# dgrzech/sobfu

Measured on AMD Instinct MI355X. Metric: solver iterations/sec on 256^3 voxel grid, higher is better.
Workload: dtype f32

## Files before the change

include/sobfu_amd/sobfu.hpp:

```cpp
#pragma once

#include <hip/hip_runtime_api.h>
#include <hip/hip_vector_types.h>

#include <chrono>
#include <cmath>
#include <cstdio>
#include <cstdlib>
#include <cstring>
#include <iostream>
#include <memory>
#include <stdexcept>
#include <algorithm>
#include <string>
#include <vector>

#include "sobfu_hip.h"

#ifndef SOBFU_AMD_HAVE_OPENCV
namespace cv {
template <class T, int N>
struct Vec {
    T val[N];
    Vec() { for (int i = 0; i < N; ++i) val[i] = T(); }
// ... 310 lines not shown
    image.create(normals.rows(), normals.cols());
    sobfuSafeCall(sobfu_hip_render_normals((const float*) normals.ptr(), (int) normals.step(), normals.rows(), normals.cols(), (uint8_t*) image.ptr(),
                                           (int) image.step(), nullptr));
}

inline void depthBilateralFilter(const Depth& in, Depth& out, int kernel_size, float sigma_spatial, float sigma_depth) {
    out.create(in.rows(), in.cols());
    sobfuSafeCall(sobfu_hip_bilateral_filter(in.ptr(), (int) in.step(), out.ptr(), (int) out.step(), in.rows(), in.cols(),
                                             kernel_size, sigma_spatial, sigma_depth, nullptr));
}
inline void depthTruncation(Depth& depth, float threshold) {
    sobfuSafeCall(sobfu_hip_truncate_depth(depth.ptr(), (int) depth.step(), depth.rows(), depth.cols(), threshold, nullptr));
}
inline void computeDists(const Depth& depth, Dists& dists, const Intr& intr) {
    dists.create(depth.rows(), depth.cols());
    sobfuSafeCall(sobfu_hip_compute_dists(depth.ptr(), (int) depth.step(), dists.ptr(), (int) dists.step(), depth.rows(),
                                          depth.cols(), intr.fx, intr.fy, intr.cx, intr.cy, nullptr));
}

inline void depthBuildPyramid(const Depth& depth, Depth& pyramid, float sigma_depth) {
    pyramid.create(depth.rows() / 2, depth.cols() / 2);
    sobfuSafeCall(sobfu_hip_depth_pyramid(depth.ptr(), (int) depth.step(), depth.rows(), depth.cols(), pyramid.ptr(), (int) pyramid.step(),
                                          sigma_depth, nullptr));
}
inline void computeNormalsAndMaskDepth(const Intr& intr, Depth& depth, Normals& normals) {
    normals.create(depth.rows(), depth.cols());
    sobfuSafeCall(sobfu_hip_compute_normals_mask_depth(depth.ptr(), (int) depth.step(), depth.rows(), depth.cols(), intr.fx, intr.fy, intr.cx, intr.cy,
                                                       (float*) normals.ptr(), (int) normals.step(), nullptr));
}
inline void computePointNormals(const Intr& intr, const Depth& depth, Cloud& points, Normals& normals) {
    points.create(depth.rows(), depth.cols());
    normals.create(depth.rows(), depth.cols());
    sobfuSafeCall(sobfu_hip_compute_point_normals(depth.ptr(), (int) depth.step(), depth.rows(), depth.cols(), intr.fx, intr.fy, intr.cx, intr.cy,
                                                  (float*) points.ptr(), (int) points.step(), (float*) normals.ptr(), (int) normals.step(), nullptr));
}
inline void resizeDepthNormals(const Depth& depth, const Normals& normals, Depth& depth_out, Normals& normals_out) {
    depth_out.create(depth.rows() / 2, depth.cols() / 2);
    normals_out.create(depth.rows() / 2, depth.cols() / 2);
    sobfuSafeCall(sobfu_hip_resize_depth_normals(depth.ptr(), (int) depth.step(), (const float*) normals.ptr(), (int) normals.step(), depth.rows(),
                                                 depth.cols(), depth_out.ptr(), (int) depth_out.step(), (float*) normals_out.ptr(),
                                                 (int) normals_out.step(), nullptr));
}
inline void resizePointsNormals(const Cloud& points, const Normals& normals, Cloud& points_out, Normals& normals_out) {
    points_out.create(points.rows() / 2, points.cols() / 2);
    normals_out.create(points.rows() / 2, points.cols() / 2);
    sobfuSafeCall(sobfu_hip_resize_points_normals((const float*) points.ptr(), (int) points.step(), (const float*) normals.ptr(), (int) normals.step(),
                                                  points.rows(), points.cols(), (float*) points_out.ptr(), (int) points_out.step(),
                                                  (float*) normals_out.ptr(), (int) normals_out.step(), nullptr));
}

struct Frame {
    bool use_points = false;
    std::vector<Depth> depth_pyr;
    std::vector<Cloud> points_pyr;
    std::vector<Normals> normals_pyr;
};

class ProjectiveICP {
public:
    enum { MAX_PYRAMID_LEVELS = 4 };
    typedef std::vector<Depth> DepthPyr;
    typedef std::vector<Cloud> PointsPyr;
    typedef std::vector<Normals> NormalsPyr;

    ProjectiveICP() : angle_thres_(20.f * 0.017453293f), dist_thres_(0.1f) {
        setIterationsNum(std::vector<int>{10, 5, 4, 0});
        workspace_.create(sobfu_hip_icp_workspace_bytes() + 16 * sizeof(float) + 4 * sizeof(int));
    }
    virtual ~ProjectiveICP() {}
    float getDistThreshold() const { return dist_thres_; }
    void setDistThreshold(float distance) { dist_thres_ = distance; }
    float getAngleThreshold() const { return angle_thres_; }
    void setAngleThreshold(float angle) { angle_thres_ = angle; }
    void setIterationsNum(const std::vector<int>& iters) {
        iters_.assign(MAX_PYRAMID_LEVELS, 0);
        for (size_t i = 0; i < iters.size() && i < (size_t) MAX_PYRAMID_LEVELS; ++i) iters_[i] = iters[i];
    }
    int getUsedLevelsNum() const {
        int i = MAX_PYRAMID_LEVELS - 1;
        for (; i >= 0 && !iters_[i]; --i) {}
        return i + 1;
    }
    virtual bool estimateTransform(Affine3f& affine, const Intr& intr, const Frame& curr, const Frame& prev) {
        if (curr.use_points) return estimateTransform(affine, intr, curr.points_pyr, curr.normals_pyr, prev.points_pyr, prev.normals_pyr);
        return estimateTransform(affine, intr, curr.depth_pyr, curr.normals_pyr, prev.depth_pyr, prev.normals_pyr);
    }
    virtual bool estimateTransform(Affine3f& affine, const Intr& intr, const DepthPyr& dcurr, const NormalsPyr ncurr, const DepthPyr dprev,
                                   const NormalsPyr nprev) {
        return run(affine, intr, 1, [&](int l) {
            return sobfu_hip_icp_level{dcurr[l].ptr(), (int) dcurr[l].step(), (const float*) ncurr[l].ptr(), (int) ncurr[l].step(), dprev[l].ptr(),
                                       (int) dprev[l].step(), (const float*) nprev[l].ptr(), (int) nprev[l].step(), nprev[l].rows(), nprev[l].cols()};
        }, std::min(std::min(dcurr.size(), ncurr.size()), std::min(dprev.size(), nprev.size())));
    }
    virtual bool estimateTransform(Affine3f& affine, const Intr& intr, const PointsPyr& vcurr, const NormalsPyr ncurr, const PointsPyr vprev,
                                   const NormalsPyr nprev) {
        return run(affine, intr, 0, [&](int l) {
            return sobfu_hip_icp_level{vcurr[l].ptr(), (int) vcurr[l].step(), (const float*) ncurr[l].ptr(), (int) ncurr[l].step(), vprev[l].ptr(),
                                       (int) vprev[l].step(), (const float*) nprev[l].ptr(), (int) nprev[l].step(), nprev[l].rows(), nprev[l].cols()};
        }, std::min(std::min(vcurr.size(), ncurr.size()), std::min(vprev.size(), nprev.size())));
    }
    int lastFailedLevel() const { return status_ ? (status_ >> 8) & 0xFF : -1; }
    int lastFailedIteration() const { return status_ ? status_ & 0xFF : -1; }

private:
    template <class F>
    bool run(Affine3f& affine, const Intr& intr, int depth_mode, F level, size_t available) {
        const int n = getUsedLevelsNum();
        affine = Affine3f::Identity();
        if (n < 1 || available < (size_t) n) error("ProjectiveICP: fewer pyramid levels than iterations need", __FILE__, __LINE__);
        sobfu_hip_icp_level lv[MAX_PYRAMID_LEVELS];
        for (int l = 0; l < n; ++l) lv[l] = level(l);
        char* ws = workspace_.ptr<char>();
        const size_t wsb = sobfu_hip_icp_workspace_bytes();
        float* d_pose = (float*) (ws + wsb);
        int* d_status = (int*) (ws + wsb + 16 * sizeof(float));
        sobfuSafeCall(sobfu_hip_icp_estimate(lv, n, iters_.data(), depth_mode, intr.fx, intr.fy, intr.cx, intr.cy, dist_thres_, angle_thres_, ws, wsb,
                                             d_pose, d_status, nullptr, nullptr));
        float P[16];
        sobfuSafeCall(hipMemcpy(P, d_pose, sizeof P, hipMemcpyDeviceToHost));
        sobfuSafeCall(hipMemcpy(&status_, d_status, sizeof status_, hipMemcpyDeviceToHost));
        if (status_ != 0) return false;
        for (int i = 0; i < 3; ++i) {
            for (int j = 0; j < 3; ++j) affine.R[3 * i + j] = P[4 * i + j];
            affine.t[i] = P[4 * i + 3];
        }
        return true;
    }
    std::vector<int> iters_;
    float angle_thres_;
    float dist_thres_;
    DeviceMemory workspace_;
    int status_ = 0;
};
}

namespace device {
typedef int3 Vec3i;
typedef float3 Vec3f;
struct Mat3f { float3 data[3]; };
struct Aff3f { Mat3f R; Vec3f t; };
struct Projector {
    float2 f, c;
    Projector() {}
    Projector(float fx, float fy, float cx, float cy) { f.x = fx; f.y = fy; c.x = cx; c.y = cy; }
};
struct TsdfVolume {
    float2* const data;
    const int3 dims;
    const float3 voxel_size;
    const float trunc_dist, eta, max_weight;
    TsdfVolume(float2* d, int3 dm, float3 vs, float trunc, float eta_, float maxw)
        : data(d), dims(dm), voxel_size(vs), trunc_dist(trunc), eta(eta_), max_weight(maxw) {}
};
inline void clear_volume(TsdfVolume& v) { sobfuSafeCall(sobfu_hip_clear_volume((float*) v.data, v.dims.x, v.dims.y, v.dims.z, nullptr)); }
inline void integrate(TsdfVolume& g, TsdfVolume& n) {
    sobfuSafeCall(sobfu_hip_integrate_fuse((float*) g.data, (const float*) n.data, g.dims.x, g.dims.y, g.dims.z, g.max_weight, nullptr));
    sobfuSafeCall(hipDeviceSynchronize());
}
inline void integrate(const cuda::Dists& dists, TsdfVolume& v, const Aff3f& a, const Projector& p) {
    float R[9] = {a.R.data[0].x, a.R.data[0].y, a.R.data[0].z, a.R.data[1].x, a.R.data[1].y, a.R.data[1].z,
                  a.R.data[2].x, a.R.data[2].y, a.R.data[2].z};
    float t[3] = {a.t.x, a.t.y, a.t.z}, vs[3] = {v.voxel_size.x, v.voxel_size.y, v.voxel_size.z};
    sobfuSafeCall(sobfu_hip_integrate_depth(dists.ptr(), (int) dists.step(), dists.rows(), dists.cols(), (float*) v.data, v.dims.x,
                                            v.dims.y, v.dims.z, vs, v.trunc_dist, v.eta, R, t, p.f.x, p.f.y, p.c.x, p.c.y, nullptr));
    sobfuSafeCall(hipDeviceSynchronize());
}
#define SOBFU_AMD_VS(v) float vs[3] = {(v).voxel_size.x, (v).voxel_size.y, (v).voxel_size.z}
inline void init_sphere(TsdfVolume& v, const float3& c, const float& r) {
    SOBFU_AMD_VS(v); float cc[3] = {c.x, c.y, c.z};
    sobfuSafeCall(sobfu_hip_init_sphere((float*) v.data, v.dims.x, v.dims.y, v.dims.z, vs, v.trunc_dist, v.eta, cc, r, nullptr));
    sobfuSafeCall(hipDeviceSynchronize());
}
inline void init_box(TsdfVolume& v, const float3& b) {
    SOBFU_AMD_VS(v); float bb[3] = {b.x, b.y, b.z};
    sobfuSafeCall(sobfu_hip_init_box((float*) v.data, v.dims.x, v.dims.y, v.dims.z, vs, v.trunc_dist, bb, nullptr));
    sobfuSafeCall(hipDeviceSynchronize());
}
inline void init_ellipsoid(TsdfVolume& v, const float3& r) {
    SOBFU_AMD_VS(v); float rr[3] = {r.x, r.y, r.z};
    sobfuSafeCall(sobfu_hip_init_ellipsoid((float*) v.data, v.dims.x, v.dims.y, v.dims.z, vs, v.trunc_dist, rr, nullptr));
    sobfuSafeCall(hipDeviceSynchronize());
}
inline void init_plane(TsdfVolume& v, const float& z) {
    SOBFU_AMD_VS(v);
    sobfuSafeCall(sobfu_hip_init_plane((float*) v.data, v.dims.x, v.dims.y, v.dims.z, vs, v.trunc_dist, z, nullptr));
    sobfuSafeCall(hipDeviceSynchronize());
}
inline void init_torus(TsdfVolume& v, const float2& t) {
    SOBFU_AMD_VS(v); float tt[2] = {t.x, t.y};
    sobfuSafeCall(sobfu_hip_init_torus((float*) v.data, v.dims.x, v.dims.y, v.dims.z, vs, v.trunc_dist, tt, nullptr));
    sobfuSafeCall(hipDeviceSynchronize());
}
#undef SOBFU_AMD_VS
}

template <class D, class S> inline D device_cast(const S& s);
template <> inline int3 device_cast<int3, cv::Vec3i>(const cv::Vec3i& v) { int3 r; r.x = v[0]; r.y = v[1]; r.z = v[2]; return r; }
template <> inline float3 device_cast<float3, cv::Vec3f>(const cv::Vec3f& v) { float3 r; r.x = v[0]; r.y = v[1]; r.z = v[2]; return r; }
template <> inline device::Aff3f device_cast<device::Aff3f, cv::Affine3f>(const cv::Affine3f& a) {
    device::Aff3f r;
    for (int i = 0; i < 3; ++i) { r.R.data[i].x = a.R[3 * i]; r.R.data[i].y = a.R[3 * i + 1]; r.R.data[i].z = a.R[3 * i + 2]; }
    r.t.x = a.t[0]; r.t.y = a.t[1]; r.t.z = a.t[2];
    return r;
}

namespace cuda {
class TsdfVolume {
public:
    explicit TsdfVolume(const Params& p)
        : trunc_dist_(p.tsdf_trunc_dist), eta_(p.eta), max_weight_(p.tsdf_max_weight), dims_(p.volume_dims), size_(p.volume_size),
          pose_(p.volume_pose), gradient_delta_factor_(p.gradient_delta_factor), raycast_step_factor_(0.f) { create(dims_); }
    virtual ~TsdfVolume() {}
    void create(const Vec3i& dims) {
        dims_ = dims;
        data_.create((size_t) dims_[0] * dims_[1] * dims_[2] * 2 * sizeof(float));
        clear();
    }
    Vec3i getDims() const { return dims_; }
    Vec3f getVoxelSize() const { return Vec3f(size_[0] / dims_[0], size_[1] / dims_[1], size_[2] / dims_[2]); }
    const CudaData data() const { return data_; }
    CudaData data() { return data_; }
    Vec3f getSize() const { return size_; }
    void setSize(const Vec3f& s) { size_ = s; }
    float getTruncDist() const { return trunc_dist_; }
    void setTruncDist(float& d) { trunc_dist_ = d; }
    float getEta() const { return eta_; }
    void setEta(float& e) { eta_ = e; }
    float getMaxWeight() const { return max_weight_; }
    void setMaxWeight(float& w) { max_weight_ = w; }
    Affine3f getPose() const { return pose_; }
    void setPose(const Affine3f& p) { pose_ = p; }
    float getGradientDeltaFactor() const { return gradient_delta_factor_; }
    void setGradientDeltaFactor(float& f) { gradient_delta_factor_ = f; }
    float getRaycastStepFactor() const { return raycast_step_factor_; }
    void setRaycastStepFactor(float& f) { raycast_step_factor_ = f; }
    virtual void clear() { device::TsdfVolume v = pod(); device::clear_volume(v); }
    void swap(CudaData& d) { data_.swap(d); }
    virtual void applyAffine(const Affine3f& a) { pose_ = a * pose_; }
    virtual void integrate(const TsdfVolume& phi_n_psi) {
        device::TsdfVolume g = pod();
        device::TsdfVolume n((float2*) phi_n_psi.data_.ptr<float2>(), g.dims, g.voxel_size, trunc_dist_, eta_, max_weight_);
        device::integrate(g, n);
    }
    virtual void integrate(const Dists& dists, const Affine3f& camera_pose, const Intr& intr) {
        Affine3f vol2cam = camera_pose.inv() * pose_;
        device::TsdfVolume v = pod();
        device::integrate(dists, v, device_cast<device::Aff3f>(vol2cam), device::Projector(intr.fx, intr.fy, intr.cx, intr.cy));
    }
    virtual void raycast(const Affine3f& camera_pose, const Intr& intr, Cloud& points, Normals& normals) {
        const Affine3f vol2cam = camera_pose.inv() * pose_;
        const Vec3f vs = getVoxelSize();
        normals.create(points.rows(), points.cols());
        sobfuSafeCall(sobfu_hip_raycast(data_.ptr<float>(), dims_[0], dims_[1], dims_[2], vs[0], vs[1], vs[2], trunc_dist_, vol2cam.R, vol2cam.t,
                                        intr.fx, intr.fy, intr.cx, intr.cy, points.rows(), points.cols(),
                                        raycast_step_factor_ > 0.f ? raycast_step_factor_ : 0.75f, (float*) points.ptr(), (int) points.step(),
                                        (float*) normals.ptr(), (int) normals.step(), nullptr));
    }
    virtual void initBox(const float3& b) { device::TsdfVolume v = pod(); device::init_box(v, b); }
    virtual void initEllipsoid(const float3& r) { device::TsdfVolume v = pod(); device::init_ellipsoid(v, r); }
    virtual void initPlane(const float& z) { device::TsdfVolume v = pod(); device::init_plane(v, z); }
    virtual void initSphere(const float3& c, const float& r) { device::TsdfVolume v = pod(); device::init_sphere(v, c, r); }
    virtual void initTorus(const float2& t) { device::TsdfVolume v = pod(); device::init_torus(v, t); }
    device::TsdfVolume pod() {
        return device::TsdfVolume(data_.ptr<float2>(), device_cast<int3>(dims_), device_cast<float3>(getVoxelSize()), trunc_dist_, eta_, max_weight_);
    }

private:
    CudaData data_;
    float trunc_dist_, eta_, max_weight_;
    Vec3i dims_;
    Vec3f size_;
    Affine3f pose_;
    float gradient_delta_factor_, raycast_step_factor_;
};

inline int colour_weight_cap(float tsdf_max_weight) { return !(tsdf_max_weight >= 1.f) ? 1 : tsdf_max_weight >= 255.f ? 255 : (int) tsdf_max_weight; }
class ColourVolume {
public:
    explicit ColourVolume(const Vec3i& dims) { create(dims); }
    void create(const Vec3i& dims) {
        dims_ = dims;
        data_.create((size_t) dims_[0] * dims_[1] * dims_[2]);
        clear();
    }
    void clear() { sobfuSafeCall(hipMemsetAsync(data_.ptr(), 0, data_.sizeBytes(), nullptr)); }
    Vec3i getDims() const { return dims_; }
    DeviceArray<RGB>& data() { return data_; }
    const DeviceArray<RGB>& data() const { return data_; }
    void integrate(const Image& image, const TsdfVolume& tsdf, const float* d_psi, const Affine3f& camera_pose, const Intr& intr) {
        const Affine3f vol2cam = camera_pose.inv() * tsdf.getPose();
        const Vec3f vs = tsdf.getVoxelSize();
        const float v[3] = {vs[0], vs[1], vs[2]};
        sobfuSafeCall(sobfu_hip_integrate_colour((const uint8_t*) image.ptr(), (int) image.step(), image.rows(), image.cols(),
                                                 tsdf.data().ptr<float>(), d_psi, (uint8_t*) data_.ptr(), dims_[0], dims_[1], dims_[2], v,
                                                 vol2cam.R, vol2cam.t, intr.fx, intr.fy, intr.cx, intr.cy, colour_weight_cap(tsdf.getMaxWeight()),
                                                 nullptr));
    }
    void apply(const float* d_psi_inv, ColourVolume& out) const {
        out.create(dims_);
        sobfuSafeCall(sobfu_hip_apply_colour((const uint8_t*) data_.ptr(), (uint8_t*) out.data_.ptr(), d_psi_inv, dims_[0], dims_[1], dims_[2], nullptr));
    }
    void sample(const Cloud& points, const Normals& normals, const Affine3f& vol2cam, const Vec3f& voxel_size, Image& out) const {
        out.create(points.rows(), points.cols());
        const float v[3] = {voxel_size[0], voxel_size[1], voxel_size[2]};
        sobfuSafeCall(sobfu_hip_sample_colour((const uint8_t*) data_.ptr(), dims_[0], dims_[1], dims_[2], v, vol2cam.R, vol2cam.t, 0,
                                              (const float*) points.ptr(), (int) points.step(), (const float*) normals.ptr(), (int) normals.step(),
                                              points.rows(), points.cols(), (uint8_t*) out.ptr(), (int) out.step(), nullptr));
    }
    void sample_vertices(const DeviceArray<Point>& vertices, const Affine3f& mc_pose, const Vec3f& voxel_size, std::vector<RGB>& out) const {
        out.clear();
        const size_t n = vertices.size();
        if (n == 0) return;
        DeviceArray<RGB> d(n);
        const float v[3] = {voxel_size[0], voxel_size[1], voxel_size[2]};
        sobfuSafeCall(sobfu_hip_sample_colour((const uint8_t*) data_.ptr(), dims_[0], dims_[1], dims_[2], v, mc_pose.R, mc_pose.t, 1,
                                              (const float*) vertices.ptr(), (int) (n * sizeof(Point)), nullptr, 0, 1, (int) n, (uint8_t*) d.ptr(),
                                              (int) (n * sizeof(RGB)), nullptr));
        d.download(out);
    }

private:
    DeviceArray<RGB> data_;
    Vec3i dims_;
};

inline void renderImage(const Cloud& points, const Normals& normals, const Image& colours, const Vec3f& light_pose, Image& image) {
    image.create(normals.rows(), normals.cols());
    sobfuSafeCall(sobfu_hip_render_colour((const float*) points.ptr(), (int) points.step(), (const float*) normals.ptr(), (int) normals.step(),
                                          (const uint8_t*) colours.ptr(), (int) colours.step(), normals.rows(), normals.cols(), light_pose[0],
                                          light_pose[1], light_pose[2], (uint8_t*) image.ptr(), (int) image.step(), nullptr));
}
}

namespace device {
typedef float4 PointType;
inline void bindTextures(const int*, const int*, const int*) {}
inline void unbindTextures() {}
inline int getOccupiedVoxels(const TsdfVolume& v, cuda::DeviceArray2D<int>& occupied_voxels, cuda::DeviceArray<unsigned char>* scratch = nullptr) {
    int n = 0;
    if (scratch && scratch->size() < sobfu_hip_mc_workspace_bytes(v.dims.x, v.dims.y, v.dims.z))
        scratch->create(sobfu_hip_mc_workspace_bytes(v.dims.x, v.dims.y, v.dims.z));
    sobfuSafeCall(sobfu_hip_mc_occupied_voxels(nullptr, (const float*) v.data, v.dims.x, v.dims.y, v.dims.z, occupied_voxels.ptr(),
                                               (int) (occupied_voxels.step() / sizeof(int)), occupied_voxels.cols(), &n,
                                               scratch ? scratch->ptr() : nullptr, scratch ? scratch->size() : 0));
    return n;
}
inline int computeOffsetsAndTotalVertices(cuda::DeviceArray2D<int>& occupied_voxels, int active_voxels, cuda::DeviceArray<unsigned char>* scratch = nullptr) {
    int total = 0;
    sobfuSafeCall(sobfu_hip_mc_offsets(nullptr, occupied_voxels.ptr(), (int) (occupied_voxels.step() / sizeof(int)), active_voxels, &total,
                                       scratch ? scratch->ptr() : nullptr, scratch ? scratch->size() : 0));
    return total;
}
inline void generateTriangles(const TsdfVolume& v, const cuda::DeviceArray2D<int>& occupied_voxels, int active_voxels, const float3& volume_size,
                              const Aff3f& pose, cuda::DeviceArray<PointType>& out_vertices, cuda::DeviceArray<PointType>& out_normals) {
    const float R[9] = {pose.R.data[0].x, pose.R.data[0].y, pose.R.data[0].z, pose.R.data[1].x, pose.R.data[1].y, pose.R.data[1].z,
                        pose.R.data[2].x, pose.R.data[2].y, pose.R.data[2].z};
    const float t[3] = {pose.t.x, pose.t.y, pose.t.z};
    sobfuSafeCall(sobfu_hip_mc_generate_triangles(nullptr, (const float*) v.data, v.dims.x, v.dims.y, v.dims.z, occupied_voxels.ptr(),
                                                  (int) (occupied_voxels.step() / sizeof(int)), active_voxels, volume_size.x, volume_size.y,
                                                  volume_size.z, R, t, (float*) out_vertices.ptr(), (float*) out_normals.ptr(),
                                                  (int) std::min(out_vertices.size(), out_normals.size())));
    sobfuSafeCall(hipDeviceSynchronize());
}
}

}

namespace sobfu_amd {
struct IndexedMesh {
    std::vector<float4> vertices, normals;
    std::vector<int> faces;
    std::vector<kfusion::RGB> colours;
    size_t triangles() const { return faces.size() / 3; }
    bool empty() const { return faces.empty(); }
};
}

namespace kfusion {
namespace cuda {
class MarchingCubes {
public:
    enum { POINTS_PER_TRIANGLE = 3, DEFAULT_TRIANGLES_BUFFER_SIZE = 2 * 1000 * 1000 * POINTS_PER_TRIANGLE };
    typedef std::shared_ptr<MarchingCubes> Ptr;
    MarchingCubes() : pose(Affine3f::Identity()) {}
    void setPose(const Affine3f& pose_) { pose = pose_; }
    Surface run(const TsdfVolume& volume, DeviceArray<Point>& vertices_buffer, DeviceArray<Normal>& normals_buffer) {
        if (vertices_buffer.empty()) vertices_buffer.create(DEFAULT_TRIANGLES_BUFFER_SIZE);
        if (normals_buffer.empty()) normals_buffer.create(DEFAULT_TRIANGLES_BUFFER_SIZE);
        occupied_voxels_buffer_.create(3, (int) (vertices_buffer.size() / 3));
        device::TsdfVolume vol = const_cast<TsdfVolume&>(volume).pod();
        const int active_voxels = device::getOccupiedVoxels(vol, occupied_voxels_buffer_, &scan_scratch_);
        std::cout << "no. of active voxels: " << active_voxels << std::endl;
        if (!active_voxels) return Surface();
        int total_vertices = device::computeOffsetsAndTotalVertices(occupied_voxels_buffer_, active_voxels, &scan_scratch_);
        const int cap = (int) (std::min(vertices_buffer.size(), normals_buffer.size()) / 3 * 3);
        if (total_vertices > cap) total_vertices = cap;
        device::generateTriangles(vol, occupied_voxels_buffer_, active_voxels, device_cast<float3>(volume.getSize()),
                                  device_cast<device::Aff3f>(pose), vertices_buffer, normals_buffer);
        Surface s;
        s.vertices = DeviceArray<Point>(vertices_buffer.ptr(), (size_t) total_vertices);
        s.normals  = DeviceArray<Normal>(normals_buffer.ptr(), (size_t) total_vertices);
        return s;
    }

    sobfu_amd::IndexedMesh run_indexed(const TsdfVolume& volume) {
        const Vec3i d = volume.getDims();
        const size_t ws = sobfu_hip_mc_indexed_workspace_bytes(d[0], d[1], d[2]);
        if (indexed_scratch_.size() < ws) indexed_scratch_.create(ws);
        const float* vol = volume.data().ptr<float>();
        int active = 0, nv = 0, nt = 0;
        sobfuSafeCall(sobfu_hip_mc_indexed_count(nullptr, vol, d[0], d[1], d[2], indexed_scratch_.ptr(), indexed_scratch_.size(), &active, &nv, &nt));
        std::cout << "no. of active voxels: " << active << std::endl;
        sobfu_amd::IndexedMesh m;
        indexed_vertices_.release();
        if (nt == 0) return m;
        indexed_vertices_.create(nv);
        indexed_normals_.create(nv);
        indexed_faces_.create(3 * (size_t) nt);
        const Vec3f sz = volume.getSize();
        sobfuSafeCall(sobfu_hip_mc_indexed_generate(nullptr, vol, d[0], d[1], d[2], sz[0], sz[1], sz[2], pose.R, pose.t, indexed_scratch_.ptr(),
                                                    indexed_scratch_.size(), (float*) indexed_vertices_.ptr(), (float*) indexed_normals_.ptr(), nv,
// ... 136 lines not shown
inline void convolution_depth(float4* dst, float4* src, int w, int h, int d) { sobfuSafeCall(sobfu_hip_convolution_depth((float*) dst, (const float*) src, conv_taps(), w, h, d, nullptr)); }
inline void calculate_potential_gradient(kfusion::device::TsdfVolume& pnp, kfusion::device::TsdfVolume& pg, TsdfGradient& g, Laplacian& L,
                                         PotentialGradient& nU, float w_reg) {
    sobfuSafeCall(sobfu_hip_potential_gradient((const float*) pnp.data, (const float*) pg.data, (const float*) g.data, (const float*) L.data,
                                               (float*) nU.data, w_reg, pnp.dims.x, pnp.dims.y, pnp.dims.z, nullptr));
}
inline void update_psi(DeformationField& psi, PotentialGradient& nUS, float4* updates, float alpha) {
    sobfuSafeCall(sobfu_hip_update_psi((float*) psi.data, (const float*) nUS.data, (float*) updates, alpha, psi.dims.x, psi.dims.y, psi.dims.z, nullptr));
}

struct Reductor {
    Reductor(int3 dims_, float vsz_, float trunc_dist_) : dims(dims_), vsz(vsz_), trunc_dist(trunc_dist_) {
        no_voxels = dims.x * dims.y * dims.z;
        sobfuSafeCall(sobfu_hip_reduce_config(no_voxels, &blocks, &threads));
        sobfuSafeCall(hipMalloc(&scratch, (size_t) blocks * 8));
        sobfuSafeCall(hipMalloc((void**) &updates, (size_t) no_voxels * sizeof(float4)));
    }
    ~Reductor() { (void) hipFree(scratch); (void) hipFree(updates); }
    Reductor(const Reductor&) = delete;
    Reductor& operator=(const Reductor&) = delete;
    float data_energy(float2* phi_global, float2* phi_n) {
        float e;
        sobfuSafeCall(sobfu_hip_data_energy((const float*) phi_global, (const float*) phi_n, no_voxels, scratch, &e, nullptr));
        return e;
    }
    float reg_energy_sobolev(Mat4f* J) {
        float e;
        sobfuSafeCall(sobfu_hip_reg_energy_sobolev((const float*) J, no_voxels, scratch, &e, nullptr));
        return e;
    }
    float2 max_update_norm() {
        float o[2];
        sobfuSafeCall(sobfu_hip_max_update_norm((const float*) updates, no_voxels, scratch, o, nullptr));
        float2 r; r.x = o[0]; r.y = o[1];
        return r;
    }
    int3 dims;
    float vsz, trunc_dist;
    int no_voxels, blocks, threads;
    float4* updates;
    void* scratch;
};
}

namespace cuda {
class VectorField {
public:
    explicit VectorField(cv::Vec3i d) : dims(d) {
        data.create((size_t) dims[0] * dims[1] * dims[2] * sizeof(float4));
        clear();
    }
    virtual ~VectorField() {}
    cv::Vec3i get_dims() const { return dims; }
    kfusion::cuda::CudaData get_data() { return data; }
    const kfusion::cuda::CudaData get_data() const { return data; }
    void set_data(kfusion::cuda::CudaData& d) { data = d; }
    void clear() { device::VectorField f(data.ptr<float4>(), kfusion::device_cast<int3>(dims)); device::clear(f); }
    void print() {
        const size_t X = (size_t) dims[0], Y = (size_t) dims[1], Z = (size_t) dims[2];
        std::vector<float4> h(X * Y * Z);
        data.download(h.data());
        std::cout << "--- FIELD ---" << std::endl;
        for (size_t i = 0; i < X; ++i)
            for (size_t j = 0; j < Y; ++j)
                for (size_t k = 0; k < Z; ++k) {
                    const float4& v = h[i + X * (j + Y * k)];
                    if (std::fabs(v.x) > 1e-5f || std::fabs(v.y) > 1e-5f || std::fabs(v.z) > 1e-5f)
                        std::cout << "(x,y,z)=(" << i << ", " << j << ", " << k << "), (u,v,w)=(" << v.x << ", " << v.y << "," << v.z << ")"
                                  << std::endl;
                }
    }
    int get_no_nans() {
        size_t n = (size_t) dims[0] * dims[1] * dims[2];
        std::unique_ptr<float4[]> h(new float4[n]);
        data.download(h.get());
        int c = 0;
        for (size_t i = 0; i < n; ++i) c += (h[i].x != h[i].x || h[i].y != h[i].y || h[i].z != h[i].z);
        return c;
    }

protected:
    kfusion::cuda::CudaData data;
    cv::Vec3i dims;
};
typedef VectorField TsdfGradient;
typedef VectorField Laplacian;
typedef VectorField PotentialGradient;

class DeformationField : public VectorField {
public:
    explicit DeformationField(cv::Vec3i d) : VectorField(d) { clear(); }
    void clear() { device::DeformationField p(data.ptr<float4>(), kfusion::device_cast<int3>(dims)); device::init_identity(p); }
    void apply(const cv::Ptr<kfusion::cuda::TsdfVolume> phi, cv::Ptr<kfusion::cuda::TsdfVolume> phi_psi) {
        kfusion::device::TsdfVolume a = phi->pod(), b = phi_psi->pod();
        device::DeformationField p(data.ptr<float4>(), a.dims);
        device::apply(a, b, p);
        kfusion::cuda::waitAllDefaultStream();
    }
    void get_inverse(DeformationField& psi_inv) {
        int3 d = kfusion::device_cast<int3>(dims);
        device::DeformationField a(data.ptr<float4>(), d), b(psi_inv.data.ptr<float4>(), d);
        device::estimate_inverse(a, b);
    }
};

class Jacobian {
public:
    explicit Jacobian(cv::Vec3i d) : dims(d) {
        data.create((size_t) dims[0] * dims[1] * dims[2] * sizeof(Mat4f));
        clear();
    }
    kfusion::cuda::CudaData get_data() { return data; }
    void clear() { device::Jacobian J(data.ptr<Mat4f>(), kfusion::device_cast<int3>(dims)); device::clear(J); }

private:
    kfusion::cuda::CudaData data;
    cv::Vec3i dims;
};

struct SpatialGradients {
    explicit SpatialGradients(cv::Vec3i d)
        : nabla_phi_n(new TsdfGradient(d)), nabla_phi_n_o_psi(new TsdfGradient(d)), J(new Jacobian(d)), J_inv(new Jacobian(d)),
          L(new Laplacian(d)), L_o_psi_inv(new Laplacian(d)), nabla_U(new PotentialGradient(d)), nabla_U_S(new PotentialGradient(d)) {}
    ~SpatialGradients() {
        delete nabla_phi_n; delete nabla_phi_n_o_psi; delete J; delete J_inv; delete L; delete L_o_psi_inv; delete nabla_U; delete nabla_U_S;
    }
    SpatialGradients(const SpatialGradients&) = delete;
    SpatialGradients& operator=(const SpatialGradients&) = delete;
    TsdfGradient *nabla_phi_n, *nabla_phi_n_o_psi;
    Jacobian *J, *J_inv;
    Laplacian *L, *L_o_psi_inv;
    PotentialGradient *nabla_U, *nabla_U_S;
};

class Solver {
public:
    explicit Solver(Params& p) : h_(nullptr) {
        sobfu_hip_solver_params sp;
        sp.verbosity = p.verbosity; sp.max_iter = p.max_iter; sp.s = p.s; sp.max_update_norm = p.max_update_norm;
        sp.lambda = p.lambda; sp.alpha = p.alpha; sp.w_reg = p.w_reg;
        sobfuSafeCall(sobfu_hip_solver_create(&h_, p.volume_dims[0], p.volume_dims[1], p.volume_dims[2], &sp));
    }
    ~Solver() { sobfu_hip_solver_destroy(h_); }
    Solver(const Solver&) = delete;
    Solver& operator=(const Solver&) = delete;
    void estimate_psi(const cv::Ptr<kfusion::cuda::TsdfVolume> phi_global, cv::Ptr<kfusion::cuda::TsdfVolume> phi_global_psi_inv,
                      const cv::Ptr<kfusion::cuda::TsdfVolume> phi_n, cv::Ptr<kfusion::cuda::TsdfVolume> phi_n_psi,
                      std::shared_ptr<DeformationField> psi, std::shared_ptr<DeformationField> psi_inv) {
        sobfuSafeCall(sobfu_hip_solver_estimate_psi(h_, phi_global->data().ptr<float>(), phi_global_psi_inv->data().ptr<float>(),
                                                    phi_n->data().ptr<float>(), phi_n_psi->data().ptr<float>(),
                                                    psi->get_data().ptr<float>(), psi_inv->get_data().ptr<float>(), &last_report,
                                                    nullptr, nullptr));
    }
    sobfu_hip_solver* handle() { return h_; }
    sobfu_hip_solver_report last_report{};

private:
    sobfu_hip_solver* h_;
};
}
}

#include <fstream>
#include <map>
#include <sstream>

namespace sobfu_amd {

inline bool read_params_ini(const std::string& path, Params& p, std::map<std::string, std::string>* raw = nullptr, std::string* why = nullptr) {
    std::ifstream f(path);
    if (!f) {
        if (why) *why = "cannot open " + path;
        return false;
    }
    std::map<std::string, std::string> kv;
    std::string line;
    while (std::getline(f, line)) {
        size_t h = line.find('#');
        if (h != std::string::npos) line.erase(h);
        size_t e = line.find('=');
        if (e == std::string::npos) continue;
        auto trim = [](std::string s) {
            size_t a = s.find_first_not_of(" \t\r\n"), b = s.find_last_not_of(" \t\r\n");
            return a == std::string::npos ? std::string() : s.substr(a, b - a + 1);
        };
        kv[trim(line.substr(0, e))] = trim(line.substr(e + 1));
    }
    auto F = [&](const char* k, float& v) { auto it = kv.find(k); if (it != kv.end()) v = std::strtof(it->second.c_str(), nullptr); };
    auto I = [&](const char* k, int& v) { auto it = kv.find(k); if (it != kv.end()) v = (int) std::strtol(it->second.c_str(), nullptr, 10); };
    I("VOL_DIMS_X", p.volume_dims[0]); I("VOL_DIMS_Y", p.volume_dims[1]); I("VOL_DIMS_Z", p.volume_dims[2]);
    F("VOL_SIZE_X", p.volume_size[0]); F("VOL_SIZE_Y", p.volume_size[1]); F("VOL_SIZE_Z", p.volume_size[2]);
    F("TSDF_MAX_WEIGHT", p.tsdf_max_weight);
    F("GRADIENT_DELTA_FACTOR", p.gradient_delta_factor);
    F("INTR_FX", p.intr.fx); F("INTR_FY", p.intr.fy); F("INTR_CX", p.intr.cx); F("INTR_CY", p.intr.cy);
    F("TRUNC_DEPTH", p.icp_truncate_depth_dist);
    F("BILATERAL_SIGMA_DEPTH", p.bilateral_sigma_depth); F("BILATERAL_SIGMA_SPATIAL", p.bilateral_sigma_spatial);
    I("BILATERAL_KERNEL_SIZE", p.bilateral_kernel_size);
    I("START_FRAME", p.start_frame); I("MAX_ITER", p.max_iter);
    F("MAX_UPDATE_NORM", p.max_update_norm);
    I("S", p.s); F("LAMBDA", p.lambda); F("ALPHA", p.alpha); F("W_REG", p.w_reg);
    {
        int track = p.track_camera ? 1 : 0;
        I("TRACK_CAMERA", track);
        p.track_camera = track != 0;
        F("ICP_DIST_THRES", p.icp_dist_thres);
        auto it = kv.find("ICP_ANGLE_THRES");
        if (it != kv.end()) p.icp_angle_thres = std::strtof(it->second.c_str(), nullptr) * 0.017453293f;
        it = kv.find("ICP_ITERS");
        if (it != kv.end()) {
            std::vector<int> iters;
            std::stringstream ss(it->second);
            std::string tok;
            while (std::getline(ss, tok, ',')) iters.push_back((int) std::strtol(tok.c_str(), nullptr, 10));
            iters.resize(4, 0);
            p.icp_iter_num = iters;
        }
    }
    float trunc_vox = 0.f, eta_vox = 0.f, tz = 0.f;
    for (const char* k : {"TSDF_TRUNC_DIST", "ETA", "VOL_POSE_T_Z"})
        if (!kv.count(k)) {
            if (why) *why = std::string("required key ") + k + " is missing from " + path;
            return false;
        }
    F("TSDF_TRUNC_DIST", trunc_vox); F("ETA", eta_vox); F("VOL_POSE_T_Z", tz);
    for (int i = 0; i < 3; ++i)
        if (p.volume_dims[i] <= 0 || !(p.volume_size[i] > 0.f)) {
            if (why) *why = "VOL_DIMS_* / VOL_SIZE_* must be positive in " + path;
            return false;
        }
    if (!(trunc_vox > 0.f)) {
        if (why) *why = "TSDF_TRUNC_DIST must be positive in " + path;
        return false;
    }
    p.tsdf_trunc_dist = trunc_vox * p.voxel_sizes()[0];
    p.eta             = eta_vox * p.voxel_sizes()[0];
    p.volume_pose     = cv::Affine3f().translate(cv::Vec3f(-p.volume_size[0] / 2.f, -p.volume_size[1] / 2.f, tz));
    if (raw) *raw = kv;
    return true;
}
}

namespace sobfu_amd {
struct MeshFit {
    size_t vertices = 0, valid = 0;
    double mean_abs = 0, rms = 0, max = 0;
};
inline void warp_mesh(IndexedMesh& m, const sobfu::cuda::DeformationField& psi, const Params& p,
                      kfusion::cuda::DeviceArray<kfusion::cuda::Point>* d_vertices = nullptr, kfusion::cuda::DeviceArray<kfusion::cuda::Normal>* d_normals = nullptr) {
    const size_t n = m.vertices.size();
    if (n == 0) return;
    kfusion::cuda::DeviceArray<kfusion::cuda::Point> dv;
    kfusion::cuda::DeviceArray<kfusion::cuda::Normal> dn;
    const bool normals = m.normals.size() == n;
    if (d_vertices && d_vertices->size() == n && (!normals || (d_normals && d_normals->size() == n))) {
        dv = *d_vertices;
        if (normals) dn = *d_normals;
    } else {
        dv.upload(m.vertices);
        if (normals) dn.upload(m.normals);
    }
    const cv::Vec3i d = psi.get_dims();
    const cv::Vec3f vs = p.voxel_sizes();
    const float v[3] = {vs[0], vs[1], vs[2]};
    sobfuSafeCall(sobfu_hip_warp_points(psi.get_data().ptr<float>(), d[0], d[1], d[2], v, p.volume_pose.R, p.volume_pose.t, 1, (const float*) dv.ptr(),
                                        normals ? (const float*) dn.ptr() : nullptr, (int) n, (float*) dv.ptr(), normals ? (float*) dn.ptr() : nullptr,
                                        nullptr));
    dv.download(m.vertices);
    if (normals) dn.download(m.normals);
}
inline MeshFit mesh_fit(const IndexedMesh& m, const kfusion::cuda::TsdfVolume& vol, const Params& p, std::vector<float>* samples = nullptr) {
    MeshFit f;
    const size_t n = f.vertices = m.vertices.size();
    std::vector<float> h;
    if (n > 0) {
        kfusion::cuda::DeviceArray<kfusion::cuda::Point> dv;
        kfusion::cuda::DeviceArray<float> out(n);
        dv.upload(m.vertices);
        const cv::Vec3i d = vol.getDims();
        const cv::Vec3f vs = vol.getVoxelSize();
        const float v[3] = {vs[0], vs[1], vs[2]};
        sobfuSafeCall(sobfu_hip_sample_tsdf(vol.data().ptr<float>(), d[0], d[1], d[2], v, p.volume_pose.R, p.volume_pose.t, 1, (const float*) dv.ptr(), (int) n,
                                            out.ptr(), nullptr));
        out.download(h);
    }
    double s1 = 0, s2 = 0;
    for (float x : h) {
        if (x != x) continue;
        const double a = std::fabs((double) x) * (double) vol.getTruncDist();
        ++f.valid, s1 += a, s2 += a * a, f.max = std::max(f.max, a);
    }
    if (f.valid) f.mean_abs = s1 / (double) f.valid, f.rms = std::sqrt(s2 / (double) f.valid);
    if (samples) samples->swap(h);
    return f;
}
}

#include "evaluate.hpp"
#include "warp_stats.hpp"

#ifndef SOBFU_AMD_NO_SOBFUSION
class SobFusion {
public:
    explicit SobFusion(const Params& p) : frame_counter_(0), params(p), camera_pose_(cv::Affine3f::Identity()) {
        dists_.create(params.rows, params.cols);
        mc = std::make_shared<kfusion::cuda::MarchingCubes>();
        mc->setPose(params.volume_pose);
        poses_.reserve(4096);
    }
    Params& getParams() { return params; }
    const std::vector<cv::Affine3f>& getPoses() const { return poses_; }
    cv::Affine3f getCameraPose() const { return camera_pose_; }
    bool operator()(const kfusion::cuda::Depth& depth, const kfusion::cuda::Image& image = kfusion::cuda::Image()) {
        const bool coloured = !image.empty();
        if (coloured && (image.rows() != depth.rows() || image.cols() != depth.cols()))
            kfusion::cuda::error("colour frame and depth frame differ in size", __FILE__, __LINE__);
        std::printf("--- FRAME NO. %d ---\n", frame_counter_);
        kfusion::cuda::depthBilateralFilter(depth, filtered_, params.bilateral_kernel_size, params.bilateral_sigma_spatial,
                                            params.bilateral_sigma_depth);
        kfusion::cuda::depthTruncation(filtered_, params.icp_truncate_depth_dist);
        kfusion::cuda::computeDists(filtered_, dists_, params.intr);
        if (params.track_camera) track();
        poses_.push_back(camera_pose_);
        return frame(image, [&](kfusion::cuda::TsdfVolume& v, bool fresh) {
            if (!fresh) v.clear();
            v.integrate(dists_, camera_pose_, params.intr);
        });
    }
    bool integrate_mesh(const sobfu_amd::IndexedMesh& mesh, const cv::Affine3f& mesh2cam = sobfu_amd::mesh_frame(), bool allow_open = false,
                        std::string* why = nullptr, int* open_rows = nullptr, int sign = sobfu_amd::kSignParity) {
        cv::Ptr<kfusion::cuda::TsdfVolume> target = frame_counter_ == 0 ? cv::Ptr<kfusion::cuda::TsdfVolume>(new kfusion::cuda::TsdfVolume(params)) : phi_n;
        int open = 0;
        if (!sobfu_amd::mesh_to_tsdf(mesh, mesh2cam, camera_pose_.inv() * params.volume_pose, *target, &open, why, 0.f, SOBFU_MESH_DISTANCE_AUTO, sign)) return false;
        if (open_rows) *open_rows = open;
        if (sign != sobfu_amd::kSignWinding && open > 0 && !allow_open) {
            if (why) *why = "the mesh is not closed: " + std::to_string(open) + " rows of the volume cross it an odd number of times";
            return false;
        }
        std::printf("--- FRAME NO. %d ---\n", frame_counter_);
        poses_.push_back(camera_pose_);
        return frame(kfusion::cuda::Image(), [](kfusion::cuda::TsdfVolume&, bool) {}, target);
    }
    std::shared_ptr<kfusion::cuda::ColourVolume> get_colour_global_psi_inv() {
        if (!colour_global) return nullptr;
        if (!colour_global_psi_inv) colour_global_psi_inv = std::make_shared<kfusion::cuda::ColourVolume>(params.volume_dims);
        colour_global->apply(psi_inv->get_data().ptr<float>(), *colour_global_psi_inv);
        return colour_global_psi_inv;
    }
    std::shared_ptr<sobfu::cuda::DeformationField> getDeformationField() { return psi; }
    sobfu_amd::TriangleMesh get_phi_global_mesh() { return get_mesh(phi_global, colour_global.get()); }
    sobfu_amd::TriangleMesh get_phi_global_psi_inv_mesh() { return get_mesh(phi_global_psi_inv, get_colour_global_psi_inv().get()); }
    sobfu_amd::TriangleMesh get_phi_n_mesh() { return get_mesh(phi_n); }
    sobfu_amd::TriangleMesh get_phi_n_psi_mesh() { return get_mesh(phi_n_psi); }
    sobfu_amd::TriangleMesh get_mesh(cv::Ptr<kfusion::cuda::TsdfVolume> vol, const kfusion::cuda::ColourVolume* colour = nullptr) {
        kfusion::cuda::DeviceArray<kfusion::cuda::Point> vertices_buffer;
        kfusion::cuda::DeviceArray<kfusion::cuda::Normal> normals_buffer;
        kfusion::cuda::Surface model = mc->run(*vol, vertices_buffer, normals_buffer);
        kfusion::cuda::waitAllDefaultStream();
        sobfu_amd::TriangleMesh m = convert_to_mesh(model.vertices);
        if (colour) colour->sample_vertices(model.vertices, params.volume_pose, vol->getVoxelSize(), m.colours);
        return m;
    }
    sobfu_amd::IndexedMesh get_phi_global_indexed_mesh() { return get_indexed_mesh(phi_global, colour_global.get()); }
    sobfu_amd::IndexedMesh get_phi_global_psi_inv_indexed_mesh() { return get_indexed_mesh(phi_global_psi_inv, get_colour_global_psi_inv().get()); }
    sobfu_amd::IndexedMesh get_phi_n_indexed_mesh() { return get_indexed_mesh(phi_n); }
    sobfu_amd::IndexedMesh get_phi_n_psi_indexed_mesh() { return get_indexed_mesh(phi_n_psi); }
    sobfu_amd::IndexedMesh get_indexed_mesh(cv::Ptr<kfusion::cuda::TsdfVolume> vol, const kfusion::cuda::ColourVolume* colour = nullptr) {
        sobfu_amd::IndexedMesh m = mc->run_indexed(*vol);
        if (colour && !m.empty()) colour->sample_vertices(mc->last_indexed_vertices(), params.volume_pose, vol->getVoxelSize(), m.colours);
        return m;
    }
    sobfu_amd::IndexedMesh get_phi_global_warped_indexed_mesh() {
        sobfu_amd::IndexedMesh m = get_indexed_mesh(phi_global, colour_global.get());
        if (!m.empty() && psi) sobfu_amd::warp_mesh(m, *psi, params, &mc->last_indexed_vertices(), &mc->last_indexed_normals());
        return m;
    }
    sobfu_amd::IndexedMesh warp_to_live(sobfu_amd::IndexedMesh m) {
        if (psi) sobfu_amd::warp_mesh(m, *psi, params);
        return m;
    }
    sobfu_amd::MeshFit fit_to_live(const sobfu_amd::IndexedMesh& m, std::vector<float>* samples = nullptr) {
        if (!phi_n) kfusion::cuda::error("fit_to_live needs a second frame", __FILE__, __LINE__);
        return sobfu_amd::mesh_fit(m, *phi_n, params, samples);
    }
    bool evaluate_canonical(const sobfu_amd::IndexedMesh& gt, float max_dist, sobfu_amd::MeshComparison& out, sobfu_amd::IndexedMesh* model = nullptr,
                            std::vector<float>* d_model = nullptr, std::string* why = nullptr, sobfu_amd::AlignRequest* align = nullptr, bool with_signs = false,
                            int sign = sobfu_amd::kSignParity, const sobfu_amd::ScoreRequest* score = nullptr, sobfu_amd::MeshScore* scored = nullptr) {
        sobfu_amd::IndexedMesh m = get_phi_global_indexed_mesh();
        const bool scoring = score && scored;
        bool ok;
        if (align) {
            sobfu_amd::IndexedMesh posed = gt;
            ok = sobfu_amd::align_meshes(m.vertices, gt, align->pose, align->info, align->iters, max_dist, align->dof, 0.f, 0.f, why);
            if (ok) {
                sobfu_amd::transform_points(posed.vertices, align->pose);
                ok = sobfu_amd::compare_meshes(m, posed, max_dist, out, d_model, nullptr, why, nullptr, with_signs, sign);
            }
            if (ok && scoring) ok = sobfu_amd::f_score(m, posed, *score, max_dist, *scored, why);
        } else {
            ok = sobfu_amd::compare_meshes(m, gt, max_dist, out, d_model, nullptr, why, nullptr, with_signs, sign);
            if (ok && scoring) ok = sobfu_amd::f_score(m, gt, *score, max_dist, *scored, why);
        }
        if (model) *model = std::move(m);
        return ok;
    }
    bool evaluate_live(const sobfu_amd::IndexedMesh& gt, float max_dist, sobfu_amd::MeshComparison& out, sobfu_amd::IndexedMesh* model = nullptr,
                       std::vector<float>* d_model = nullptr, std::string* why = nullptr, sobfu_amd::TriangleGrid* gt_grid = nullptr, bool with_signs = false,
                       int sign = sobfu_amd::kSignParity, const sobfu_amd::ScoreRequest* score = nullptr, sobfu_amd::MeshScore* scored = nullptr) {
        sobfu_amd::IndexedMesh m = get_phi_global_warped_indexed_mesh();
        bool ok = sobfu_amd::compare_meshes(m, gt, max_dist, out, d_model, nullptr, why, gt_grid, with_signs, sign);
        if (ok && score && scored) ok = sobfu_amd::f_score(m, gt, *score, max_dist, *scored, why, gt_grid);
        if (model) *model = std::move(m);
        return ok;
    }
    bool warp_stats(float band, sobfu_amd::WarpStats& out, std::vector<float>* det = nullptr, std::vector<float>* res = nullptr,
                    const std::vector<float>& edges = {0.f, 0.25f, 0.5f, 1.f, 2.f, 4.f}, float res_tol = -1.f) {
        if (!solved_) return false;
        const cv::Vec3i d = psi->get_dims();
        const cv::Vec3f vs = params.voxel_sizes();
        const int dims[3] = {d[0], d[1], d[2]};
        const float v[3] = {vs[0], vs[1], vs[2]};
        const float tol = res_tol >= 0.f ? res_tol : (float) (0.1 * (double) std::min(v[0], std::min(v[1], v[2])));
        out = sobfu_amd::warp_stats(psi->get_data().ptr<float>(), psi_inv->get_data().ptr<float>(), phi_global->data().ptr<float>(),
                                    phi_global_psi_inv->data().ptr<float>(), dims, v, band, edges, tol, det, res);
        return true;
    }
    static sobfu_amd::TriangleMesh convert_to_mesh(const kfusion::cuda::DeviceArray<kfusion::cuda::Point>& triangles) {
        sobfu_amd::TriangleMesh m;
        if (!triangles.empty()) triangles.download(m.vertices);
        return m;
    }
    std::shared_ptr<kfusion::cuda::MarchingCubes> mc;

    cv::Ptr<kfusion::cuda::TsdfVolume> phi_global, phi_global_psi_inv, phi_n, phi_n_psi;
    std::shared_ptr<sobfu::cuda::DeformationField> psi, psi_inv;
    std::shared_ptr<sobfu::cuda::Solver> solver;
    std::shared_ptr<kfusion::cuda::ColourVolume> colour_global, colour_global_psi_inv;

private:
    template <class Integrate>
    bool frame(const kfusion::cuda::Image& image, Integrate&& integrate, cv::Ptr<kfusion::cuda::TsdfVolume> ready = cv::Ptr<kfusion::cuda::TsdfVolume>()) {
        const bool coloured = !image.empty();
        if (frame_counter_ == 0) {
            phi_global = ready ? ready : cv::Ptr<kfusion::cuda::TsdfVolume>(new kfusion::cuda::TsdfVolume(params));
            integrate(*phi_global, true);
            if (coloured) integrate_colour(image, *phi_global, nullptr);
            phi_global_psi_inv = cv::Ptr<kfusion::cuda::TsdfVolume>(new kfusion::cuda::TsdfVolume(params));
            phi_n              = cv::Ptr<kfusion::cuda::TsdfVolume>(new kfusion::cuda::TsdfVolume(params));
            phi_n_psi          = cv::Ptr<kfusion::cuda::TsdfVolume>(new kfusion::cuda::TsdfVolume(params));
            psi     = std::make_shared<sobfu::cuda::DeformationField>(params.volume_dims);
            psi_inv = std::make_shared<sobfu::cuda::DeformationField>(params.volume_dims);
            solver  = std::make_shared<sobfu::cuda::Solver>(params);
            return ++frame_counter_, true;
        }
        integrate(*phi_n, false);
        if (frame_counter_ < params.start_frame) {
            if (coloured) integrate_colour(image, *phi_n, nullptr);
            phi_global->integrate(*phi_n);
            return ++frame_counter_, true;
        }
        solver->estimate_psi(phi_global, phi_global_psi_inv, phi_n, phi_n_psi, psi, psi_inv);
        solved_ = true;
        if (coloured) integrate_colour(image, *phi_n_psi, psi->get_data().ptr<float>());
        phi_global->integrate(*phi_n_psi);
        return ++frame_counter_, true;
    }
    void integrate_colour(const kfusion::cuda::Image& image, const kfusion::cuda::TsdfVolume& tsdf, const float* d_psi) {
        if (!colour_global) colour_global = std::make_shared<kfusion::cuda::ColourVolume>(params.volume_dims);
        colour_global->integrate(image, tsdf, d_psi, camera_pose_, params.intr);
    }
    void track() {
        kfusion::cuda::ProjectiveICP probe;
        probe.setIterationsNum(params.icp_iter_num);
        const int levels = std::max(1, probe.getUsedLevelsNum());
        curr_.use_points = prev_.use_points = true;
        curr_.depth_pyr.resize(levels), curr_.points_pyr.resize(levels), curr_.normals_pyr.resize(levels);
        curr_.depth_pyr[0] = filtered_;
        for (int l = 1; l < levels; ++l) kfusion::cuda::depthBuildPyramid(curr_.depth_pyr[l - 1], curr_.depth_pyr[l], params.bilateral_sigma_depth);
        for (int l = 0; l < levels; ++l) kfusion::cuda::computePointNormals(params.intr(l), curr_.depth_pyr[l], curr_.points_pyr[l], curr_.normals_pyr[l]);
        if (frame_counter_ > 0) {
            if (!icp_) icp_ = std::make_shared<kfusion::cuda::ProjectiveICP>();
            icp_->setIterationsNum(params.icp_iter_num);
            icp_->setDistThreshold(params.icp_dist_thres);
            icp_->setAngleThreshold(params.icp_angle_thres);
            cv::Affine3f aff;
            if (icp_->estimateTransform(aff, params.intr, curr_, prev_)) camera_pose_ = camera_pose_ * aff;
            else std::printf("camera tracking failed on frame %d (level %d, iteration %d): keeping the previous pose\n", frame_counter_,
                             icp_->lastFailedLevel(), icp_->lastFailedIteration());
        }
        std::swap(curr_, prev_);
    }
    int frame_counter_;
    bool solved_ = false;
    Params params;
    cv::Affine3f camera_pose_;
    std::vector<cv::Affine3f> poses_;
    kfusion::cuda::Frame curr_, prev_;
    std::shared_ptr<kfusion::cuda::ProjectiveICP> icp_;
    kfusion::cuda::Depth filtered_;
    kfusion::cuda::Dists dists_;
};
#endif
```

include/sobfu_hip.h:

```cpp
#ifndef SOBFU_HIP_H
#define SOBFU_HIP_H

#include <stddef.h>
#include <stdint.h>

#if defined(__GNUC__)
#pragma GCC visibility push(default)
#endif
#ifdef __cplusplus
extern "C" {
#endif

#define SOBFU_HIP_ABI_VERSION 3

#define SOBFU_E_BADARG (-1)
#define SOBFU_E_FILTER (-2)
#define SOBFU_E_UNSUPPORTED (-3)

int sobfu_hip_abi_version(void);
const char* sobfu_hip_error_string(int code);

int sobfu_hip_clear_volume(float* d_vol, int X, int Y, int Z, void* stream);
int sobfu_hip_integrate_depth(const float* d_dists, int dists_step_bytes, int rows, int cols, float* d_vol, int X,
                              int Y, int Z, const float voxel_size[3], float trunc_dist, float eta,
                              const float R[9], const float t[3], float fx, float fy, float cx, float cy,
                              void* stream);
int sobfu_hip_integrate_fuse(float* d_phi_global, const float* d_phi_n_psi, int X, int Y, int Z, float max_weight,
                             void* stream);
int sobfu_hip_init_sphere(float* d_vol, int X, int Y, int Z, const float voxel_size[3], float trunc_dist, float eta,
                          const float centre[3], float radius, void* stream);
int sobfu_hip_init_box(float* d_vol, int X, int Y, int Z, const float voxel_size[3], float trunc_dist,
                       const float b[3], void* stream);
int sobfu_hip_init_ellipsoid(float* d_vol, int X, int Y, int Z, const float voxel_size[3], float trunc_dist,
                             const float r[3], void* stream);
int sobfu_hip_init_plane(float* d_vol, int X, int Y, int Z, const float voxel_size[3], float trunc_dist, float z,
                         void* stream);
int sobfu_hip_init_torus(float* d_vol, int X, int Y, int Z, const float voxel_size[3], float trunc_dist,
                         const float t[2], void* stream);

int sobfu_hip_bilateral_filter(const uint16_t* d_src, int src_step_bytes, uint16_t* d_dst, int dst_step_bytes,
                               int rows, int cols, int kernel_size, float sigma_spatial, float sigma_depth,
                               void* stream);
int sobfu_hip_truncate_depth(uint16_t* d_depth, int step_bytes, int rows, int cols, float max_dist_m, void* stream);
int sobfu_hip_compute_dists(const uint16_t* d_depth, int depth_step_bytes, float* d_dists, int dists_step_bytes,
                            int rows, int cols, float fx, float fy, float cx, float cy, void* stream);

int sobfu_hip_clear_field(float* d_field, int X, int Y, int Z, void* stream);
int sobfu_hip_init_identity(float* d_psi, int X, int Y, int Z, void* stream);
int sobfu_hip_apply(const float* d_phi, float* d_phi_warped, const float* d_psi, int X, int Y, int Z, void* stream);
int sobfu_hip_estimate_inverse(const float* d_psi, float* d_psi_inv, int X, int Y, int Z, int n_sweeps,
                               void* stream);
int sobfu_hip_inverse_and_warp(const float* d_psi, float* d_psi_inv, const float* d_phi, float* d_phi_warped, int X, int Y, int Z,
                               int n_sweeps, void* stream);
int sobfu_hip_tsdf_gradient(const float* d_vol, float* d_grad, int X, int Y, int Z, void* stream);
int sobfu_hip_laplacian(const float* d_psi, float* d_L, int X, int Y, int Z, void* stream);
int sobfu_hip_jacobian(const float* d_psi, float* d_J, int X, int Y, int Z, int mode, void* stream);
int sobfu_hip_clear_jacobian(float* d_J, int X, int Y, int Z, void* stream);

int sobfu_hip_sobolev_filter(int s, float lambda, float* out);
int sobfu_hip_potential_gradient(const float* d_phi_n_psi, const float* d_phi_global, const float* d_grad,
                                 const float* d_L, float* d_nabla_U, float w_reg, int X, int Y, int Z, void* stream);
int sobfu_hip_convolution_rows(float* d_dst, const float* d_src, const float taps[7], int w, int h, int d,
                               void* stream);
int sobfu_hip_convolution_columns(float* d_dst, const float* d_src, const float taps[7], int w, int h, int d,
                                  void* stream);
int sobfu_hip_convolution_depth(float* d_dst, const float* d_src, const float taps[7], int w, int h, int d,
                                void* stream);
int sobfu_hip_update_psi(float* d_psi, const float* d_nabla_U_S, float* d_updates, float alpha, int X, int Y, int Z,
                         void* stream);

int sobfu_hip_reduce_config(int n, int* blocks, int* threads);
int sobfu_hip_data_energy(const float* d_phi_global, const float* d_phi_n, int n, void* d_scratch, float* out,
                          void* stream);
int sobfu_hip_reg_energy_sobolev(const float* d_J, int n, void* d_scratch, float* out, void* stream);
int sobfu_hip_max_update_norm(const float* d_updates, int n, void* d_scratch, float out[2], void* stream);
int sobfu_hip_reg_energy_sobolev_from_psi(const float* d_psi, int X, int Y, int Z, void* d_scratch, float* out,
                                          void* stream);

int sobfu_hip_fused_potential_gradient(const float* d_phi_n_psi, const float* d_phi_global, const float* d_psi,
                                       float* d_nabla_U, float w_reg, int X, int Y, int Z, void* stream);
int sobfu_hip_fused_smooth_update_apply(const float* d_nabla_U, float* d_psi, const float* d_phi_n,
                                        float* d_phi_n_psi, float* d_updates, uint32_t* d_max_sq_slots,
                                        const float taps[7], float alpha, int X, int Y, int Z, void* stream);

int sobfu_hip_pack_vec3(const float* d_src4, float* d_dst3, size_t n, void* stream);
int sobfu_hip_unpack_vec3(const float* d_src3, float* d_dst4, size_t n, void* stream);
int sobfu_hip_extract_tsdf(const float* d_src2, float* d_dst1, size_t n, void* stream);

int sobfu_hip_tile3_init_identity(float* d_psi, int Lx, int Ly, int Lz, int xb, int yb, int zb, void* stream);
int sobfu_hip_tile3_apply(const float* d_phi, int Xg, int Yg, int Zg, float* d_phi_warped, const float* d_psi, int Lx, int Ly, int Lz,
                          void* stream);
int sobfu_hip_tile3_estimate_inverse(const float* d_psi, int Xg, int Yg, int Zg, float* d_psi_inv, int Lx, int Ly, int Lz, int xb, int yb,
                                     int zb, int n_sweeps, void* stream);
int sobfu_hip_tile3_estimate_inverse_window(const float* d_psi_win, const int win[6], int Xg, int Yg, int Zg, float* d_psi_inv, int Lx, int Ly, int Lz,
                                            int xb, int yb, int zb, const int box[6], int n_sweeps, int* d_violation, void* stream);
int sobfu_hip_tile3_apply_window(const float* d_phi_win, const int win[6], int Xg, int Yg, int Zg, float* d_phi_warped, const float* d_psi, int Lx,
                                 int Ly, int Lz, const int box[6], int* d_violation, void* stream);
int sobfu_hip_tile3_max_displacement(const float* d_psi, int Lx, int Ly, int Lz, int xb, int yb, int zb, const int box[6], uint32_t* d_max_bits,
                                     void* stream);
int sobfu_hip_tile3_integrate_depth(const float* d_dists, int dists_step_bytes, int rows, int cols, float* d_vol_local, int Lx, int Ly,
                                    int Lz, int xb, int yb, int zb, const float voxel_size[3], float trunc_dist, float eta,
                                    const float R[9], const float t[3], float fx, float fy, float cx, float cy, void* stream);
int sobfu_hip_tile3_potential_gradient(const float* d_phi_n_psi, const float* d_phi_global, const float* d_psi, float* d_nabla_U,
                                       float w_reg, int Lx, int Ly, int Lz, const int box[6], int thin,
                                       const uint32_t* d_prev_slots, float max_update_norm, int compact, void* stream);
int sobfu_hip_tile3_smooth_update_apply(const float* d_nabla_U, float* d_psi, const float* d_phi_n, float* d_phi_n_psi, float* d_updates,
                                        uint32_t* d_max_sq_slots, const float taps[7], float alpha, int Lx, int Ly, int Lz, int Xg,
                                        int Yg, int Zg, const int own[6], const int box[6], int thin,
                                        const uint32_t* d_prev_slots, float max_update_norm, int compact, void* stream);
int sobfu_hip_tile3_apply_tsdf_only(const float* d_phi1, int Xg, int Yg, int Zg, float* d_out1, const float* d_psi3, int Lx, int Ly, int Lz,
                                    void* stream);
int sobfu_hip_tile3_pack(const float* d_field3, int Lx, int Ly, int Lz, float* d_buf, const int* boxes, int n_boxes, void* stream);
int sobfu_hip_tile3_unpack(float* d_field3, int Lx, int Ly, int Lz, const float* d_buf, const int* boxes, int n_boxes, void* stream);

typedef struct sobfu_hip_solver sobfu_hip_solver;

typedef struct {
    int verbosity;
    int max_iter;
    int s;
    float max_update_norm;
    float lambda;
    float alpha;
    float w_reg;
} sobfu_hip_solver_params;

typedef struct {
    int iterations;
    int converged;
    float last_max_update_norm;
    float last_max_update_index;
    float last_e_data, last_e_reg;
} sobfu_hip_solver_report;

int sobfu_hip_solver_create(sobfu_hip_solver** out, int X, int Y, int Z, const sobfu_hip_solver_params* params);
int sobfu_hip_solver_destroy(sobfu_hip_solver* s);
int sobfu_hip_solver_set_params(sobfu_hip_solver* s, const sobfu_hip_solver_params* params);
size_t sobfu_hip_solver_workspace_bytes(const sobfu_hip_solver* s);
int sobfu_hip_solver_estimate_psi(sobfu_hip_solver* s, const float* d_phi_global, float* d_phi_global_psi_inv,
                                  const float* d_phi_n, float* d_phi_n_psi, float* d_psi, float* d_psi_inv,
                                  sobfu_hip_solver_report* report, float* per_iter_max_norm, void* stream);
int sobfu_hip_solver_iterate(sobfu_hip_solver* s, const float* d_phi_global, const float* d_phi_n,
                             float* d_phi_n_psi, float* d_psi, int n_iters, sobfu_hip_solver_report* report,
                             float* per_iter_max_norm, void* stream);
int sobfu_hip_solver_begin(sobfu_hip_solver* s, const float* d_phi_global, const float* d_phi_n, float* d_phi_n_psi,
                           float* d_psi, int max_iters, void* stream);
int sobfu_hip_solver_step(sobfu_hip_solver* s, int n_iters, void* stream);
int sobfu_hip_solver_end(sobfu_hip_solver* s, sobfu_hip_solver_report* report, float* per_iter_max_norm, void* stream);
float* sobfu_hip_solver_updates(sobfu_hip_solver* s);
int sobfu_hip_solver_keep_updates(sobfu_hip_solver* s, int keep);
int sobfu_hip_solver_set_compact(sobfu_hip_solver* s, int enable);
int sobfu_hip_solver_set_profiling(sobfu_hip_solver* s, int stride);
int sobfu_hip_solver_get_profile(sobfu_hip_solver* s, float* ms_pass_a, float* ms_pass_b, int* launches, int reset);
typedef void (*sobfu_hip_log_fn)(const char* line, void* user);
int sobfu_hip_solver_set_logger(sobfu_hip_solver* s, sobfu_hip_log_fn fn, void* user);

size_t sobfu_hip_mc_workspace_bytes(int X, int Y, int Z);
int sobfu_hip_mc_occupied_voxels(void* stream, const float* d_vol, int X, int Y, int Z, int* d_occupied, int stride, int max_size,
                                 int* h_count, void* d_workspace, size_t workspace_bytes);
int sobfu_hip_mc_offsets(void* stream, int* d_occupied, int stride, int count, int* h_total_vertices, void* d_workspace,
                         size_t workspace_bytes);
int sobfu_hip_mc_generate_triangles(void* stream, const float* d_vol, int X, int Y, int Z, const int* d_occupied, int stride, int count,
                                    float size_x, float size_y, float size_z, const float R[9], const float t[3], float* d_vertices,
                                    float* d_normals, int max_vertices);
size_t sobfu_hip_mc_indexed_workspace_bytes(int X, int Y, int Z);
int sobfu_hip_mc_indexed_count(void* stream, const float* d_vol, int X, int Y, int Z, void* d_workspace, size_t workspace_bytes,
                               int* h_active_cells, int* h_vertices, int* h_triangles);
int sobfu_hip_mc_indexed_generate(void* stream, const float* d_vol, int X, int Y, int Z, float size_x, float size_y, float size_z,
                                  const float R[9], const float t[3], void* d_workspace, size_t workspace_bytes, float* d_vertices,
                                  float* d_normals, int max_vertices, int* d_faces, int max_triangles);

int sobfu_hip_raycast(const float* d_vol, int X, int Y, int Z, float vsx, float vsy, float vsz, float trunc, const float R[9],
                      const float t[3], float fx, float fy, float cx, float cy, int rows, int cols, float step_factor, float* d_points,
                      int points_step, float* d_normals, int normals_step, void* stream);
int sobfu_hip_render_image(const float* d_points, int points_step, const float* d_normals, int normals_step, int rows, int cols,
                           float lx, float ly, float lz, uint8_t* d_image, int image_step, void* stream);
int sobfu_hip_render_normals(const float* d_normals, int normals_step, int rows, int cols, uint8_t* d_image, int image_step,
                             void* stream);

int sobfu_hip_integrate_colour(const uint8_t* d_image, int image_step, int rows, int cols, const float* d_tsdf, const float* d_psi,
                               uint8_t* d_colour, int X, int Y, int Z, const float voxel_size[3], const float R[9], const float t[3],
                               float fx, float fy, float cx, float cy, int cap, void* stream);
int sobfu_hip_apply_colour(const uint8_t* d_colour, uint8_t* d_colour_warped, const float* d_psi_inv, int X, int Y, int Z, void* stream);
int sobfu_hip_sample_colour(const uint8_t* d_colour, int X, int Y, int Z, const float voxel_size[3], const float R[9], const float t[3],
                            int mc_vertices, const float* d_points, int points_step, const float* d_normals, int normals_step, int rows,
                            int cols, uint8_t* d_out, int out_step, void* stream);
int sobfu_hip_render_colour(const float* d_points, int points_step, const float* d_normals, int normals_step, const uint8_t* d_colour_image,
                            int colour_step, int rows, int cols, float lx, float ly, float lz, uint8_t* d_image, int image_step,
                            void* stream);

int sobfu_hip_warp_points(const float* d_psi, int X, int Y, int Z, const float voxel_size[3], const float R[9], const float t[3],
                          int mc_vertices, const float* d_points, const float* d_normals, int n, float* d_points_out, float* d_normals_out,
                          void* stream);
int sobfu_hip_sample_tsdf(const float* d_vol, int X, int Y, int Z, const float voxel_size[3], const float R[9], const float t[3],
                          int mc_vertices, const float* d_points, int n, float* d_out, void* stream);

int sobfu_hip_depth_pyramid(const uint16_t* d_src, int src_step, int rows, int cols, uint16_t* d_dst, int dst_step, float sigma_depth,
                            void* stream);
int sobfu_hip_compute_point_normals(const uint16_t* d_depth, int depth_step, int rows, int cols, float fx, float fy, float cx, float cy,
                                    float* d_points, int points_step, float* d_normals, int normals_step, void* stream);
int sobfu_hip_compute_normals_mask_depth(uint16_t* d_depth, int depth_step, int rows, int cols, float fx, float fy, float cx, float cy,
                                         float* d_normals, int normals_step, void* stream);
int sobfu_hip_resize_depth_normals(const uint16_t* d_depth, int depth_step, const float* d_normals, int normals_step, int rows, int cols,
                                   uint16_t* d_depth_out, int depth_out_step, float* d_normals_out, int normals_out_step, void* stream);
int sobfu_hip_resize_points_normals(const float* d_points, int points_step, const float* d_normals, int normals_step, int rows, int cols,
                                    float* d_points_out, int points_out_step, float* d_normals_out, int normals_out_step, void* stream);
typedef struct {
    const void* curr;
    int curr_step;
    const float* ncurr;
    int ncurr_step;
    const void* prev;
    int prev_step;
    const float* nprev;
    int nprev_step;
    int rows, cols;
} sobfu_hip_icp_level;
size_t sobfu_hip_icp_workspace_bytes(void);
int sobfu_hip_icp_step(const sobfu_hip_icp_level* level, int level_index, int depth_mode, float fx, float fy, float cx, float cy,
                       float dist_thres, float angle_thres, const float* d_aff, void* d_workspace, size_t workspace_bytes,
                       double* d_sums, uint8_t* d_codes, int codes_step, void* stream);
int sobfu_hip_icp_estimate(const sobfu_hip_icp_level* levels, int n_levels, const int iters[4], int depth_mode, float fx, float fy, float cx,
                           float cy, float dist_thres, float angle_thres, void* d_workspace, size_t workspace_bytes, float* d_pose,
                           int* d_status, float* d_trace, void* stream);

#define SOBFU_E_RCCL (-4)
typedef struct sobfu_hip_tiled sobfu_hip_tiled;
int sobfu_hip_tiled_load_rccl(const char* librccl_path);
int sobfu_hip_tiled_unique_id(char out[128]);
int sobfu_hip_tiled_create(sobfu_hip_tiled** out, int X, int Y, int Z, int world, int rank, const char unique_id[128],
                           const sobfu_hip_solver_params* params);
int sobfu_hip_tiled_destroy(sobfu_hip_tiled* t);
int sobfu_hip_tiled_create3(sobfu_hip_tiled** out, int X, int Y, int Z, int Px, int Py, int Pz, int rank, const char unique_id[128],
                            const sobfu_hip_solver_params* params);
int sobfu_hip_tiled_layout3(const sobfu_hip_tiled* t, int out[24]);
int sobfu_hip_tiled_layout(const sobfu_hip_tiled* t, int* z0, int* z1, int* lo, int* hi, int* Lz, int* zbase);
int sobfu_hip_tiled_iterate(sobfu_hip_tiled* t, const float* d_phi_global_local, const float* d_phi_n_full,
                            float* d_phi_n_psi_local, float* d_psi_local, int n_iters, sobfu_hip_solver_report* report,
                            float* per_iter_max_norm, void* stream);
int sobfu_hip_tiled_begin(sobfu_hip_tiled* t, const float* d_phi_global_local, const float* d_phi_n_full, float* d_phi_n_psi_local,
                          float* d_psi_local, int max_iters, void* stream);
int sobfu_hip_tiled_step(sobfu_hip_tiled* t, int n_iters, void* stream);
int sobfu_hip_tiled_end(sobfu_hip_tiled* t, sobfu_hip_solver_report* report, float* per_iter_max_norm, void* stream);
int sobfu_hip_tiled_add_reduce_comm(sobfu_hip_tiled* t, const char unique_id[128]);
int sobfu_hip_tiled_set_schedule(sobfu_hip_tiled* t, int schedule);
double sobfu_hip_tiled_last_enqueue_us(const sobfu_hip_tiled* t);
typedef struct {
    int peer;
    size_t send_off, recv_off, count;
} sobfu_hip_tiled_msg;
int sobfu_hip_tiled_messages(const sobfu_hip_tiled* t, sobfu_hip_tiled_msg* msgs, int* send_boxes, int* recv_boxes, int max_msgs);
int sobfu_hip_tiled_messages_inplace(const sobfu_hip_tiled* t, sobfu_hip_tiled_msg* msgs, int max_msgs, int* n_packed);
int sobfu_hip_tiled_set_profiling(sobfu_hip_tiled* t, int stride, int max_samples);
int sobfu_hip_tiled_get_profile(sobfu_hip_tiled* t, float ms[3], int* samples, int reset);
typedef int (*sobfu_hip_tiled_exchange_fn)(void* ctx, int rank, const float* d_send, float* d_recv, const sobfu_hip_tiled_msg* msgs,
                                           int n_msgs, void* stream);
typedef int (*sobfu_hip_tiled_allreduce_fn)(void* ctx, int rank, uint32_t* d_buf, size_t n, void* stream);
int sobfu_hip_tiled_set_transport(sobfu_hip_tiled* t, sobfu_hip_tiled_exchange_fn exchange, sobfu_hip_tiled_allreduce_fn allreduce_max,
                                  void* ctx);
#define SOBFU_E_TIMEOUT (-5)
typedef struct {
    void* arena;
    size_t nabla_u_off[2];
    size_t rows_off;
    void* flags;
} sobfu_hip_tiled_exports;
int sobfu_hip_tiled_exports_get(const sobfu_hip_tiled* t, sobfu_hip_tiled_exports* out);
int sobfu_hip_tiled_connect(sobfu_hip_tiled* t, int n_peers, const int* peer_ranks, const sobfu_hip_tiled_exports* peers);
int sobfu_hip_ipc_export(const void* d_ptr, char handle[64]);
int sobfu_hip_ipc_open(const char handle[64], void** d_ptr);
int sobfu_hip_ipc_close(void* d_ptr);
int sobfu_hip_tiled_status(sobfu_hip_tiled* t, int* missing_peer);
int sobfu_hip_tiled_max_iterations(const sobfu_hip_tiled* t);
int sobfu_hip_p2p_info(int device, int peer_device, int out[4]);
int sobfu_hip_tiled_wait_stats(sobfu_hip_tiled* t, double* wait_us, int* waits, int reset);
int sobfu_hip_tiled_pingpong(sobfu_hip_tiled* t, int rank_a, int rank_b, int reps, void* stream);
int sobfu_hip_tiled_probe_push(sobfu_hip_tiled* t, int reps, void* stream);
int sobfu_hip_tiled_set_wait(sobfu_hip_tiled* t, int wait);
int sobfu_hip_tiled_step_phase(sobfu_hip_tiled* t, int phase, void* stream);
int sobfu_hip_tiled_exchange(sobfu_hip_tiled* t, float* d_field3, int planes, void* stream);
int sobfu_hip_tiled_self_sendrecv(sobfu_hip_tiled* t, const float* d_src, float* d_dst, size_t n, void* stream);
int sobfu_hip_tiled_allreduce_max_u32(sobfu_hip_tiled* t, uint32_t* d_buf, size_t n, void* stream);

int sobfu_hip_mesh_grid_plan(const float bbox[6], int n_triangles, float cell, float origin[3], float* h, int dims[3]);
size_t sobfu_hip_mesh_grid_workspace_bytes(const int dims[3], int max_refs);
int sobfu_hip_mesh_grid_build(const float* d_vertices, int n_vertices, const int* d_faces, int n_triangles, const float origin[3], float h,
                              const int dims[3], void* d_workspace, size_t workspace_bytes, int max_refs, int* h_refs, void* stream);
#define SOBFU_MESH_DISTANCE_AUTO 0
#define SOBFU_MESH_DISTANCE_GRID 1
#define SOBFU_MESH_DISTANCE_BRUTE 2
int sobfu_hip_mesh_distance(void* d_workspace, size_t workspace_bytes, const float* d_vertices, int n_vertices, const int* d_faces,
                            int n_triangles, const float origin[3], float h, const int dims[3], const float* d_points, int n, float max_dist,
                            int mode, int ring_cap, float* d_dist, int* d_tri, float* d_closest, int* d_unresolved, void* stream);
int sobfu_hip_mesh_distance_unresolved(const void* d_workspace, int* h_count, void* stream);

size_t sobfu_hip_mesh_align_workspace_bytes(int n);
int sobfu_hip_mesh_align_step(void* d_grid_workspace, size_t grid_workspace_bytes, const float* d_vertices, int n_vertices, const int* d_faces,
                              int n_triangles, const float origin[3], float h, const int dims[3], const float* d_points, int n, float max_dist, int mode,
                              int ring_cap, const float* d_pose, void* d_workspace, size_t workspace_bytes, double* d_sums, void* stream);
int sobfu_hip_mesh_align_estimate(void* d_grid_workspace, size_t grid_workspace_bytes, const float* d_vertices, int n_vertices, const int* d_faces,
                                  int n_triangles, const float origin[3], float h, const int dims[3], const float* d_points, int n, float max_dist,
                                  int mode, int ring_cap, int iters, int dof, float eps_rot, float eps_trans, void* d_workspace, size_t workspace_bytes,
                                  float* d_pose, int* d_status, float* d_trace, void* stream);

// ... 99 lines not shown
```

sobfu_amd/csrc/solver_capi.hip:

```cpp
#include <algorithm>
#include <cmath>
#include <cstdio>
#include <cstdlib>
#include <cstring>
#include <string>
#include <vector>

#include "sobfu_device.hpp"
#include "sobfu_hip.h"
#include "sobfu_host.hpp"
#include "sobfu_launch.hpp"


namespace {

using sobfu_hip::DevicePtr;
using sobfu_hip::EventPtr;
using sobfu_hip::kSlots;
using sobfu_hip::slots_to_norm;
constexpr int kCheckEvery = 32;
constexpr int kMaxRunAhead = 96;

}

struct sobfu_hip_solver {
    int X = 0, Y = 0, Z = 0;
    size_t N = 0;
    sobfu_hip_solver_params p{};
    float taps[7]{};
    DevicePtr<float> nabla_U;
    DevicePtr<float> updates;
    DevicePtr<float> c_psi;
    DevicePtr<float> c_f;
    DevicePtr<float> c_g;
    DevicePtr<float> c_n;
    bool compact = true;
    DevicePtr<uint32_t> slots;
    sobfu_hip::PinnedPtr<uint32_t> h_rows;
    int h_rows_iters   = 0;
    EventPtr ev_chk;
    DevicePtr<void> red_scratch;
    int slots_iters    = 0;
    bool keep_updates  = false;
    sobfu_hip_log_fn log_fn = nullptr;
    void* log_user          = nullptr;
    bool log_set            = false;
    size_t bytes            = 0;
    int prof_stride = 0;
    std::vector<EventPtr> events;
    double ms_a = 0, ms_b = 0;
    int prof_launches = 0, prof_pending = 0;
    struct Session {
        bool active = false, compact = false;
        const float *pg = nullptr, *pn = nullptr;
        float *pnp = nullptr, *psi = nullptr;
        const float *it_pnp = nullptr, *it_pg = nullptr, *it_pn = nullptr;
        float *it_psi = nullptr, *it_out = nullptr, *upd = nullptr;
        int cap = 0;
        int launched = 0;
        int checked = 0, fl_to = 0;
        bool in_flight = false;
        int done = 0;
        bool converged = false;
        float last_norm = 0.f;
        bool inline_log = false;
        bool warp = false;
    } q;

    void log(const std::string& line) const {
        if (log_set) {
            if (log_fn) log_fn(line.c_str(), log_user);
        } else {
            std::printf("%s\n", line.c_str());
        }
    }
};

namespace {

std::string fmt_g(float v) {
    char b[64];
    std::snprintf(b, sizeof b, "%g", (double) v);
    return b;
}

int ensure_slots(sobfu_hip_solver* s, int iters) {
    if (iters <= s->slots_iters) return 0;
    if (s->slots) s->bytes -= (size_t) (s->slots_iters + 1) * kSlots * 4;
    s->slots_iters = 0;
    SOBFU_HIP_TRY(sobfu_hip::device_alloc(s->slots, (size_t) (iters + 1) * kSlots * 4));
    s->slots_iters = iters;
    s->bytes += (size_t) (iters + 1) * kSlots * 4;
    return 0;
}

int ensure_poll(sobfu_hip_solver* s, int iters) {
    if (!s->ev_chk) SOBFU_HIP_TRY(sobfu_hip::event_create(s->ev_chk, hipEventDisableTiming));
    if (iters <= s->h_rows_iters) return 0;
    s->h_rows.reset();
    s->h_rows_iters = 0;
    void* h = nullptr;
    SOBFU_HIP_TRY(hipHostMalloc(&h, (size_t) iters * kSlots * 4, hipHostMallocDefault));
    s->h_rows.reset((uint32_t*) h);
    s->h_rows_iters = iters;
    return 0;
}

int ensure_compact(sobfu_hip_solver* s) {
    if (s->c_psi) return 0;
    SOBFU_HIP_TRY(sobfu_hip::device_alloc(s->c_psi, s->N * 12));
    SOBFU_HIP_TRY(sobfu_hip::device_alloc(s->c_f, s->N * 4));
    SOBFU_HIP_TRY(sobfu_hip::device_alloc(s->c_g, s->N * 4));
    SOBFU_HIP_TRY(sobfu_hip::device_alloc(s->c_n, s->N * 4));
    s->bytes += s->N * 24;
    return 0;
}

int ensure_updates(sobfu_hip_solver* s) {
    if (s->updates) return 0;
    SOBFU_HIP_TRY(sobfu_hip::device_alloc(s->updates, s->N * 16));
    s->bytes += s->N * 16;
    return 0;
}

int set_params(sobfu_hip_solver* s, const sobfu_hip_solver_params* p) {
    SOBFU_CHECK_ARGS(p && p->max_iter >= 0);
    if (p->s < 7 || p->s > 16) return p->s < 7 ? SOBFU_E_UNSUPPORTED : SOBFU_E_FILTER;
    float h[16];
    SOBFU_TRY(sobfu_hip_sobolev_filter(p->s, p->lambda, h));
    for (int i = 0; i < 7; ++i) s->taps[i] = h[i];
    s->p = *p;
    return 0;
}

int ensure_events(sobfu_hip_solver* s, size_t n) {
    while (s->events.size() < n) {
        EventPtr e;
        SOBFU_HIP_TRY(sobfu_hip::event_create(e, hipEventDefault));
        s->events.push_back(std::move(e));
    }
    return 0;
}

int session_begin_impl(sobfu_hip_solver* s, const float* pg, const float* pn, float* pnp, float* psi, int cap, hipStream_t st) {
    sobfu_hip_solver::Session& q = s->q;
    const int X = s->X, Y = s->Y, Z = s->Z;
    q = sobfu_hip_solver::Session{};
    q.pg = pg; q.pn = pn; q.pnp = pnp; q.psi = psi;
    q.cap = cap;
    q.compact = s->compact && cap > 0;
    q.last_norm = NAN;
    if (!q.compact) SOBFU_TRY(sobfu_hip_apply(pn, pnp, psi, X, Y, Z, st));
    if (cap <= 0) return 0;
    SOBFU_TRY(ensure_slots(s, cap));
    SOBFU_HIP_TRY(hipMemsetAsync(s->slots.get(), 0, (size_t) (cap + 1) * kSlots * 4, st));
    if (s->keep_updates) {
        SOBFU_TRY(ensure_updates(s));
        q.upd = s->updates.get();
    }
    q.it_pnp = pnp; q.it_pg = pg; q.it_pn = pn; q.it_psi = psi; q.it_out = pnp;
    if (q.compact) {
        SOBFU_TRY(ensure_compact(s));
        SOBFU_TRY(sobfu_hip::launch_compact_enter(psi, pg, pn, s->c_psi.get(), s->c_g.get(), s->c_n.get(), s->c_f.get(), X, Y, Z, st));
        q.it_pnp = s->c_f.get(); q.it_pg = s->c_g.get(); q.it_pn = s->c_n.get(); q.it_psi = s->c_psi.get(); q.it_out = s->c_f.get();
        q.warp = s->p.verbosity == 0 && !q.upd && sobfu_hip::loop_warps_in_pass_a(X, Y, Z);
    }
    if (s->p.max_update_norm >= 0.f) SOBFU_TRY(ensure_poll(s, cap));
    if (s->prof_stride > 0) SOBFU_TRY(ensure_events(s, (size_t) 3 * (cap / s->prof_stride + 1)));
    return 0;
}
int session_begin(sobfu_hip_solver* s, const float* pg, const float* pn, float* pnp, float* psi, int cap, hipStream_t st) {
    if (s->q.active) return SOBFU_E_BADARG;
    const int rc = session_begin_impl(s, pg, pn, pnp, psi, cap, st);
    s->q.active = rc == 0;
    return rc;
}

void session_examine(sobfu_hip_solver* s, int upto, float* per_iter) {
    sobfu_hip_solver::Session& q = s->q;
    for (int k = q.checked; k < upto && !q.converged; ++k) {
        const float v = slots_to_norm(s->h_rows.get() + (size_t) k * kSlots);
        if (per_iter) per_iter[k] = v;
        q.last_norm = v;
        q.done = k + 1;
        if (v <= s->p.max_update_norm) q.converged = true;
    }
    q.checked = upto;
}

int session_enqueue(sobfu_hip_solver* s, int n, bool poll, float* per_iter, hipStream_t st) {
    sobfu_hip_solver::Session& q = s->q;
    if (!q.active || n < 0 || q.launched + n > q.cap) return SOBFU_E_BADARG;
    const int X = s->X, Y = s->Y, Z = s->Z;
    const sobfu_hip_solver_params& p = s->p;
    const bool can_converge = p.max_update_norm >= 0.f;
    const int last = q.launched + n;
    sobfu_hip::PassALaunch A;
    sobfu_hip::set_whole_grid(A, X, Y, Z);
    A.pnp = q.warp ? q.it_pn : q.it_pnp; A.pg = q.it_pg; A.psi = q.it_psi; A.nU = s->nabla_U.get(); A.w_reg = p.w_reg;
    A.max_update_norm = p.max_update_norm;
    A.compact = q.compact;
    A.warp    = q.warp;
    sobfu_hip::PassBLaunch B;
    sobfu_hip::set_whole_grid(B, X, Y, Z);
    B.nU = s->nabla_U.get(); B.psi = q.it_psi; B.phi_n = q.it_pn; B.pnp = q.it_out; B.updates = q.upd; B.taps = s->taps; B.alpha = p.alpha;
    B.max_update_norm = p.max_update_norm;
    B.compact = q.compact;
    B.warp    = q.warp;
    for (int it = q.launched + 1; it <= last && !q.converged; ++it) {
        const uint32_t* prev = (it > 1) ? s->slots.get() + (size_t) (it - 1) * kSlots : nullptr;
        uint32_t* cur        = s->slots.get() + (size_t) it * kSlots;
        const bool ev = s->prof_stride > 0 && (it % s->prof_stride == 0) && (size_t) 3 * (s->prof_pending + 1) <= s->events.size();
        const int e0  = 3 * s->prof_pending;
        if (ev) SOBFU_HIP_TRY(hipEventRecord(s->events[e0].get(), st));
        A.prev_slots = B.prev_slots = prev;
        B.slots = cur;
        SOBFU_TRY(sobfu_hip::launch_pass_a(A, st));
        if (ev) SOBFU_HIP_TRY(hipEventRecord(s->events[e0 + 1].get(), st));
        SOBFU_TRY(sobfu_hip::launch_pass_b(B, st));
        if (ev) {
            SOBFU_HIP_TRY(hipEventRecord(s->events[e0 + 2].get(), st));
            s->prof_pending += 1;
        }
        q.launched = it;
        if (can_converge && poll) {
            if (!q.in_flight && (it % kCheckEvery == 0 || it == last)) {
                SOBFU_HIP_TRY(hipMemcpyAsync(s->h_rows.get() + (size_t) q.checked * kSlots, s->slots.get() + (size_t) (q.checked + 1) * kSlots,
                                             (size_t) (it - q.checked) * kSlots * 4, hipMemcpyDeviceToHost, st));
                SOBFU_HIP_TRY(hipEventRecord(s->ev_chk.get(), st));
                q.in_flight = true;
                q.fl_to     = it;
            }
            if (q.in_flight) {
                const bool must_wait = it - q.checked >= kMaxRunAhead;
                hipError_t e = must_wait ? hipEventSynchronize(s->ev_chk.get()) : hipEventQuery(s->ev_chk.get());
                if (e == hipSuccess) {
                    session_examine(s, q.fl_to, per_iter);
                    q.in_flight = false;
                } else if (e != hipErrorNotReady) {
                    return (int) e;
                }
            }
        }
    }
    return 0;
}

int session_drain(sobfu_hip_solver* s, float* per_iter, hipStream_t st) {
    sobfu_hip_solver::Session& q = s->q;
    if (q.launched == 0) return 0;
    if (s->p.max_update_norm >= 0.f) {
        if (q.in_flight) {
            SOBFU_HIP_TRY(hipEventSynchronize(s->ev_chk.get()));
            session_examine(s, q.fl_to, per_iter);
            q.in_flight = false;
        }
        if (!q.converged && q.checked < q.launched) {
            SOBFU_HIP_TRY(hipMemcpyAsync(s->h_rows.get() + (size_t) q.checked * kSlots, s->slots.get() + (size_t) (q.checked + 1) * kSlots,
                                         (size_t) (q.launched - q.checked) * kSlots * 4, hipMemcpyDeviceToHost, st));
            SOBFU_HIP_TRY(hipStreamSynchronize(st));
            session_examine(s, q.launched, per_iter);
        }
    } else {
        std::vector<uint32_t> hs((size_t) q.launched * kSlots);
        SOBFU_HIP_TRY(hipMemcpyAsync(hs.data(), s->slots.get() + kSlots, hs.size() * 4, hipMemcpyDeviceToHost, st));
        SOBFU_HIP_TRY(hipStreamSynchronize(st));
        for (int k = 0; k < q.launched; ++k) {
            const float v = slots_to_norm(hs.data() + (size_t) k * kSlots);
            if (per_iter) per_iter[k] = v;
            q.last_norm = v;
        }
        q.done = q.launched;
    }
    return 0;
}

int session_end(sobfu_hip_solver* s, sobfu_hip_solver_report* rep, float* per_iter, hipStream_t st) {
    sobfu_hip_solver::Session& q = s->q;
    if (!q.active) return SOBFU_E_BADARG;
    sobfu_hip_solver_report r{};
    r.last_max_update_norm = NAN;
    r.last_max_update_index = NAN;
    r.last_e_data = r.last_e_reg = NAN;
    SOBFU_TRY(session_drain(s, per_iter, st));
    if (q.compact) SOBFU_TRY(sobfu_hip::launch_compact_leave(s->c_psi.get(), q.pn, q.psi, q.pnp, s->X, s->Y, s->Z, st));
    for (int it = 1; it <= q.done && !q.inline_log; ++it)
        if (it == 1 || it % 50 == 0) s->log("iter. no. " + std::to_string(it));
    if (q.converged) s->log("SOLVER CONVERGED AFTER " + std::to_string(q.done) + " ITERATIONS");
    else if (q.cap > 0 && q.done == q.cap) s->log("SOLVER REACHED MAX. NO. OF ITERATIONS WITHOUT CONVERGING");
    r.iterations = q.done;
    r.converged  = q.converged ? 1 : 0;
    r.last_max_update_norm = q.last_norm;
    q.active = false;
    SOBFU_HIP_TRY(hipStreamSynchronize(st));
    if (rep) *rep = r;
    return 0;
}

int run_verbose(sobfu_hip_solver* s, const float* pg, const float* pn, float* pnp, float* psi, int max_iter,
                sobfu_hip_solver_report* rep, float* per_iter, hipStream_t st) {
    const int X = s->X, Y = s->Y, Z = s->Z;
    const sobfu_hip_solver_params& p = s->p;
    auto reports = [&](int it) { return p.verbosity == 2 || (p.verbosity == 1 && (it == 1 || it % 50 == 0 || it == max_iter)); };
    SOBFU_TRY(ensure_updates(s));
    SOBFU_TRY(session_begin(s, pg, pn, pnp, psi, max_iter, st));
    sobfu_hip_solver::Session& q = s->q;
    q.upd = s->updates.get();
    q.inline_log = p.verbosity <= 2;
    float e_data = NAN, e_reg = NAN, arg = NAN;
    auto fail = [&](int rc) {
        q.active = false;
        return rc;
    };
#define SOBFU_VTRY(expr)                    \
    do {                                    \
        const int rc_ = (int) (expr);       \
        if (rc_ != 0) return fail(rc_);     \
    } while (0)
    sobfu_hip::PassALaunch A;
    sobfu_hip::set_whole_grid(A, X, Y, Z);
    A.pnp = q.it_pnp; A.pg = q.it_pg; A.psi = q.it_psi; A.nU = s->nabla_U.get(); A.w_reg = p.w_reg;
    A.compact = q.compact;
    sobfu_hip::PassBLaunch B;
    sobfu_hip::set_whole_grid(B, X, Y, Z);
    B.nU = s->nabla_U.get(); B.psi = q.it_psi; B.phi_n = q.it_pn; B.pnp = q.it_out; B.updates = s->updates.get(); B.taps = s->taps; B.alpha = p.alpha;
    B.compact = q.compact;
    for (int it = 1; it <= max_iter && !q.converged;) {
        if (!reports(it)) {
            int to = it;
            while (to + 1 <= max_iter && !reports(to + 1)) ++to;
            SOBFU_VTRY(session_enqueue(s, to - it + 1, true, per_iter, st));
            if (p.max_update_norm >= 0.f) SOBFU_VTRY(session_drain(s, per_iter, st));
            it = to + 1;
            continue;
        }
        if (it == 1 || it % 50 == 0) s->log("iter. no. " + std::to_string(it));
        if (q.compact) {
            SOBFU_VTRY(sobfu_hip::data_energy_tsdf(q.it_pg, q.it_pnp, (int) s->N, s->red_scratch.get(), &e_data, st));
            SOBFU_VTRY(sobfu_hip::reg_energy_from_psi3(q.it_psi, X, Y, Z, s->red_scratch.get(), &e_reg, st));
        } else {
            SOBFU_VTRY(sobfu_hip_data_energy(pg, pnp, (int) s->N, s->red_scratch.get(), &e_data, st));
            SOBFU_VTRY(sobfu_hip_reg_energy_sobolev_from_psi(psi, X, Y, Z, s->red_scratch.get(), &e_reg, st));
        }
        const float e = e_data + p.w_reg * e_reg;
        s->log("data energy + w_reg * reg energy = " + fmt_g(e_data) + " + " + fmt_g(p.w_reg) + " * " + fmt_g(e_reg) + " = " + fmt_g(e));
        uint32_t* cur = s->slots.get() + (size_t) it * kSlots;
        B.slots = cur;
        SOBFU_VTRY(sobfu_hip::launch_pass_a(A, st));
        SOBFU_VTRY(sobfu_hip::launch_pass_b(B, st));
        float mx[2];
        SOBFU_VTRY(sobfu_hip_max_update_norm(s->updates.get(), (int) s->N, s->red_scratch.get(), mx, st));
        if (per_iter) per_iter[it - 1] = mx[0];
        arg = mx[1];
        q.launched = q.checked = q.done = it;
        q.last_norm = mx[0];
        {
            int ix = (int) (mx[1] / (float) (X * Y));
            int iy = (int) ((mx[1] - (float) (ix * X * Y)) / (float) X);
            int iz = (int) (mx[1] - (float) (X * (iy + Y * ix)));
            s->log("max. update norm " + fmt_g(mx[0]) + " at voxel (" + std::to_string(iz) + ", " + std::to_string(iy) + ", " + std::to_string(ix) + ")");
        }
        if (mx[0] <= p.max_update_norm) q.converged = true;
        ++it;
    }
#undef SOBFU_VTRY
    const bool last_reported = q.done > 0 && reports(q.done);
    sobfu_hip_solver_report r{};
    SOBFU_TRY(session_end(s, &r, per_iter, st));
    r.last_e_data = e_data;
    r.last_e_reg  = e_reg;
    r.last_max_update_index = last_reported ? arg : NAN;
    if (rep) *rep = r;
    return 0;
}

int run_loop(sobfu_hip_solver* s, const float* pg, const float* pn, float* pnp, float* psi, int max_iter,
             sobfu_hip_solver_report* rep, float* per_iter, hipStream_t st) {
    if (s->q.active) return SOBFU_E_BADARG;
    if (s->p.verbosity > 0 && max_iter > 0) return run_verbose(s, pg, pn, pnp, psi, max_iter, rep, per_iter, st);
    SOBFU_TRY(session_begin(s, pg, pn, pnp, psi, max_iter, st));
    int rc = session_enqueue(s, max_iter, true, per_iter, st);
    if (rc != 0) {
        s->q.active = false;
        return rc;
    }
    return session_end(s, rep, per_iter, st);
}

}

extern "C" {

int sobfu_hip_abi_version(void) { return SOBFU_HIP_ABI_VERSION; }

const char* sobfu_hip_error_string(int code) {
    switch (code) {
        case 0: return "success";
        case SOBFU_E_BADARG: return "sobfu_hip: bad argument";
        case SOBFU_E_FILTER: return "sobfu_hip: (s, lambda) not in the Sobolev filter table";
        case SOBFU_E_UNSUPPORTED: return "sobfu_hip: unsupported configuration";
        case SOBFU_E_RCCL: return "sobfu_hip: RCCL not loaded or an RCCL call failed (see stderr)";
        case SOBFU_E_TIMEOUT: return "sobfu_hip: a peer rank did not answer within the deadline (see stderr); the tiled handle is dead";
        default: return code > 0 ? hipGetErrorString((hipError_t) code) : "sobfu_hip: unknown error";
    }
}

int sobfu_hip_sobolev_filter(int s, float lambda, float* h) {
    SOBFU_CHECK_ARGS(h);
    bool ok = false;
    if (s == 3 && lambda == 0.1f) { h[0] = 0.06537f; h[1] = 0.99572f; h[2] = h[0]; ok = true; }
    if (s == 7) {
        if (lambda == 0.05f) { h[0] = 0.00006f; h[1] = 0.00015f; h[2] = 0.03917f; h[3] = 0.99846f; ok = true; }
        if (lambda == 0.1f) { h[0] = 0.00030f; h[1] = 0.00441f; h[2] = 0.06571f; h[3] = 0.99565f; ok = true; }
        if (lambda == 0.2f) { h[0] = 0.00120f; h[1] = 0.01094f; h[2] = 0.10204f; h[3] = 0.98941f; ok = true; }
        if (lambda == 0.4f) { h[0] = 0.00169f; h[1] = 0.01312f; h[2] = 0.10927f; h[3] = 0.98781f; ok = true; }
        if (ok) { h[4] = h[2]; h[5] = h[1]; h[6] = h[0]; }
    }
    if (s == 9) {
        if (lambda == 0.05f) { h[0] = 0.000003f; h[1] = 0.00006f; h[2] = 0.00155f; h[3] = 0.03917f; h[4] = 0.99846f; ok = true; }
        if (lambda == 0.1f) { h[0] = 0.00002f; h[1] = 0.00030f; h[2] = 0.00441f; h[3] = 0.06571f; h[4] = 0.99565f; ok = true; }
        if (ok) { h[5] = h[3]; h[6] = h[2]; h[7] = h[1]; h[8] = h[0]; }
    }
    if (s == 11 && lambda == 0.1f) {
        h[0] = 0.0000015f; h[1] = 0.00002f; h[2] = 0.00030f; h[3] = 0.00441f; h[4] = 0.06571f; h[5] = 0.99565f;
        h[6] = h[4]; h[7] = h[3]; h[8] = h[2]; h[9] = h[1]; h[10] = h[0];
        ok = true;
    }
    if (!ok) return SOBFU_E_FILTER;
    volatile float sum = 0.f;
    for (int i = 0; i < s; ++i) sum = sum + h[i];
    for (int i = 0; i < s; ++i) h[i] = h[i] / sum;
    return 0;
}

int sobfu_hip_solver_create(sobfu_hip_solver** out, int X, int Y, int Z, const sobfu_hip_solver_params* params) {
    SOBFU_CHECK_ARGS(out && params && X > 1 && Y > 1 && Z > 1);
    if ((size_t) X * Y * Z > (size_t) 0x7fffffff) return SOBFU_E_UNSUPPORTED;
    std::unique_ptr<sobfu_hip_solver> s(new sobfu_hip_solver());
    s->X = X; s->Y = Y; s->Z = Z;
    s->N = (size_t) X * Y * Z;
    if (const char* e = getenv("SOBFU_COMPACT")) s->compact = atoi(e) != 0;
    SOBFU_TRY(set_params(s.get(), params));
    SOBFU_HIP_TRY(sobfu_hip::device_alloc(s->nabla_U, s->N * 16));
    SOBFU_HIP_TRY(sobfu_hip::device_alloc(s->red_scratch, 65536 * 8));
    s->bytes = s->N * 16 + 65536 * 8;
    SOBFU_TRY(ensure_slots(s.get(), params->max_iter > 0 ? params->max_iter : 1));
    if (s->compact) SOBFU_TRY(ensure_compact(s.get()));
    if (params->verbosity > 0) SOBFU_TRY(ensure_updates(s.get()));
    *out = s.release();
    return 0;
}

int sobfu_hip_solver_destroy(sobfu_hip_solver* s) {
    if (s) delete s;
    return 0;
}

int sobfu_hip_solver_set_params(sobfu_hip_solver* s, const sobfu_hip_solver_params* params) {
    SOBFU_CHECK_ARGS(s);
    return set_params(s, params);
}

size_t sobfu_hip_solver_workspace_bytes(const sobfu_hip_solver* s) { return s ? s->bytes : 0; }

float* sobfu_hip_solver_updates(sobfu_hip_solver* s) {
    if (!s) return nullptr;
    if (ensure_updates(s) != 0) return nullptr;
    return s->updates.get();
}

int sobfu_hip_solver_keep_updates(sobfu_hip_solver* s, int keep) {
    SOBFU_CHECK_ARGS(s);
    s->keep_updates = keep != 0;
    return 0;
}

int sobfu_hip_solver_set_logger(sobfu_hip_solver* s, sobfu_hip_log_fn fn, void* user) {
    SOBFU_CHECK_ARGS(s);
    s->log_fn   = fn;
    s->log_user = user;
    s->log_set  = true;
    return 0;
}

int sobfu_hip_solver_set_compact(sobfu_hip_solver* s, int enable) {
    SOBFU_CHECK_ARGS(s);
    s->compact = enable != 0;
    return 0;
}

int sobfu_hip_solver_set_profiling(sobfu_hip_solver* s, int stride) {
    SOBFU_CHECK_ARGS(s && stride >= 0);
    s->prof_stride = stride;
    const int cap = s->q.active ? s->q.cap : (s->p.max_iter > 0 ? s->p.max_iter : 1);
    if (stride > 0) SOBFU_TRY(ensure_events(s, (size_t) 3 * (cap / stride + 1)));
    return 0;
}

int sobfu_hip_solver_get_profile(sobfu_hip_solver* s, float* ms_pass_a, float* ms_pass_b, int* launches, int reset) {
    SOBFU_CHECK_ARGS(s);
    for (int it = 1; it <= s->prof_pending; ++it) {
        float a = 0, b = 0;
        SOBFU_HIP_TRY(hipEventElapsedTime(&a, s->events[3 * (it - 1)].get(), s->events[3 * (it - 1) + 1].get()));
        SOBFU_HIP_TRY(hipEventElapsedTime(&b, s->events[3 * (it - 1) + 1].get(), s->events[3 * (it - 1) + 2].get()));
        s->ms_a += a;
        s->ms_b += b;
        s->prof_launches += 1;
    }
    s->prof_pending = 0;
    if (ms_pass_a) *ms_pass_a = (float) s->ms_a;
    if (ms_pass_b) *ms_pass_b = (float) s->ms_b;
    if (launches) *launches = s->prof_launches;
    if (reset) {
        s->ms_a = s->ms_b = 0;
        s->prof_launches = 0;
    }
    return 0;
}

int sobfu_hip_solver_iterate(sobfu_hip_solver* s, const float* d_phi_global, const float* d_phi_n, float* d_phi_n_psi,
                             float* d_psi, int n_iters, sobfu_hip_solver_report* report, float* per_iter_max_norm,
                             void* stream) {
    SOBFU_CHECK_ARGS(s && d_phi_global && d_phi_n && d_phi_n_psi && d_psi && n_iters >= 0);
    SOBFU_TRY(run_loop(s, d_phi_global, d_phi_n, d_phi_n_psi, d_psi, n_iters, report, per_iter_max_norm, (hipStream_t) stream));
    return (int) hipStreamSynchronize((hipStream_t) stream);
}

int sobfu_hip_solver_begin(sobfu_hip_solver* s, const float* d_phi_global, const float* d_phi_n, float* d_phi_n_psi, float* d_psi,
                           int max_iters, void* stream) {
    SOBFU_CHECK_ARGS(s && d_phi_global && d_phi_n && d_phi_n_psi && d_psi && max_iters >= 0);
    if (s->p.verbosity > 0) return SOBFU_E_UNSUPPORTED;
    return session_begin(s, d_phi_global, d_phi_n, d_phi_n_psi, d_psi, max_iters, (hipStream_t) stream);
}

int sobfu_hip_solver_step(sobfu_hip_solver* s, int n_iters, void* stream) {
    SOBFU_CHECK_ARGS(s && n_iters >= 0);
    return session_enqueue(s, n_iters, false, nullptr, (hipStream_t) stream);
}

int sobfu_hip_solver_end(sobfu_hip_solver* s, sobfu_hip_solver_report* report, float* per_iter_max_norm, void* stream) {
    SOBFU_CHECK_ARGS(s);
    return session_end(s, report, per_iter_max_norm, (hipStream_t) stream);
}

int sobfu_hip_solver_estimate_psi(sobfu_hip_solver* s, const float* d_phi_global, float* d_phi_global_psi_inv,
                                  const float* d_phi_n, float* d_phi_n_psi, float* d_psi, float* d_psi_inv,
                                  sobfu_hip_solver_report* report, float* per_iter_max_norm, void* stream) {
    SOBFU_CHECK_ARGS(s && d_phi_global && d_phi_global_psi_inv && d_phi_n && d_phi_n_psi && d_psi && d_psi_inv);
    hipStream_t st = (hipStream_t) stream;
    SOBFU_TRY(run_loop(s, d_phi_global, d_phi_n, d_phi_n_psi, d_psi, s->p.max_iter, report, per_iter_max_norm, st));
    SOBFU_TRY(sobfu_hip_inverse_and_warp(d_psi, d_psi_inv, d_phi_global, d_phi_global_psi_inv, s->X, s->Y, s->Z, 48, st));
    return (int) hipStreamSynchronize(st);
}

}
```

sobfu_amd/csrc/tsdf_kernels.hip:

```cpp
#include "sobfu_frame.hpp"
#include "sobfu_hip.h"
#include "sobfu_host.hpp"

using namespace sobfu_hip;

namespace {

constexpr int kZC = 16;

struct IntegrateArgs {
    const float* dists;
    int step, rows, cols;
    float2* vol;
    Dims d;
    float vsx, vsy, vsz, trunc, eta;
    float R[9], t[3];
    float fx, fy, cx, cy;
    int zbase;
    int xbase, ybase;
};

__global__ void __launch_bounds__(256) integrate_depth_kernel(IntegrateArgs a) {
    int x = blockIdx.x * kBX + threadIdx.x, y = blockIdx.y * kBY + threadIdx.y;
    if (x >= a.d.x || y >= a.d.y) return;
    int z0 = blockIdx.z * kZC;
    float vcx = (x + a.xbase) * a.vsx + a.vsx / 2.f, vcy = (y + a.ybase) * a.vsy + a.vsy / 2.f, vcz = a.vsz / 2.f;
    float camx = dot3(a.R + 0, vcx, vcy, vcz) + a.t[0];
    float camy = dot3(a.R + 3, vcx, vcy, vcz) + a.t[1];
    float camz = dot3(a.R + 6, vcx, vcy, vcz) + a.t[2];
    const float sx = a.R[2] * a.vsz, sy = a.R[5] * a.vsz, sz = a.R[8] * a.vsz;
    for (int i = 0; i < z0 + a.zbase; ++i) camx += sx, camy += sy, camz += sz;
    int z1 = min(z0 + kZC, a.d.z);
    for (int z = z0; z < z1; ++z, camx += sx, camy += sy, camz += sz) {
        float coox = __builtin_fmaf(a.fx, camx / camz, a.cx), cooy = __builtin_fmaf(a.fy, camy / camz, a.cy);
        if (coox < 0 || cooy < 0 || coox >= (float) a.cols || cooy >= (float) a.rows) continue;
        if (!(camz > 0)) continue;
        if (!(coox == coox) || !(cooy == cooy)) continue;
        int px = (int) floorf(coox), py = (int) floorf(cooy);
        float Dp = row_ptr(a.dists, a.step, py)[px];
        if (Dp <= 0.f) continue;
        float psdf   = Dp - camz;
        float weight = (psdf > -a.eta) ? 1.f : 0.f;
        a.vol[vidx(a.d, x, y, z)] = pack_tsdf(psdf, a.trunc, weight);
    }
}

__global__ void __launch_bounds__(256) integrate_fuse_kernel(float2* __restrict__ g, const float2* __restrict__ n,
                                                             size_t N, float max_weight) {
    size_t i = ((size_t) blockIdx.x * blockDim.x + threadIdx.x) * 2;
    if (i >= N) return;
    auto one = [&](float2 t, float2 p, bool& w) -> float2 {
        w = !(t.y == 0.f || (t.y == 1.f && (t.x == 0.f || t.x == -1.f)));
        return make_float2(__builtin_fmaf(p.y, p.x, t.x) / (p.y + 1.f), fminf(p.y + 1.f, max_weight));
    };
    if (i + 1 < N) {
        float4 t = *(const float4*) (n + i), p = *(const float4*) (g + i);
        bool w0, w1;
        float2 o0 = one(make_float2(t.x, t.y), make_float2(p.x, p.y), w0);
        float2 o1 = one(make_float2(t.z, t.w), make_float2(p.z, p.w), w1);
        if (w0 && w1) *(float4*) (g + i) = make_float4(o0.x, o0.y, o1.x, o1.y);
        else if (w0) g[i] = o0;
        else if (w1) g[i + 1] = o1;
    } else {
        bool w0;
        float2 o0 = one(n[i], g[i], w0);
        if (w0) g[i] = o0;
    }
}

enum Prim { SPHERE, BOX, ELLIPSOID, PLANE, TORUS };
struct PrimArgs {
    float2* vol;
    Dims d;
    float vsx, vsy, vsz, trunc, eta;
    float p[3];
    float r;
};

SOBFU_DEV float norm3_fma(float x, float y, float z) {
    float a[3] = {x, y, z};
    return __builtin_sqrtf(dot3(a, x, y, z));
}

template <int P>
__global__ void __launch_bounds__(256) init_prim_kernel(PrimArgs a) {
    int x = blockIdx.x * kBX + threadIdx.x, y = blockIdx.y * kBY + threadIdx.y;
    if (x >= a.d.x || y >= a.d.y) return;
    int z0 = blockIdx.z * kZC;
    float vx = x * a.vsx + a.vsx / 2.f, vy = y * a.vsy + a.vsy / 2.f, vz = a.vsz / 2.f;
    if (P == BOX || P == ELLIPSOID || P == TORUS) {
        vx = vx - a.d.x / 2.f * a.vsx;
        vy = vy - a.d.y / 2.f * a.vsy;
        vz = vz - a.d.z / 2.f * a.vsz;
    }
    for (int i = 0; i < z0; ++i) vz += a.vsz;
    int z1 = min(z0 + kZC, a.d.z);
    for (int z = z0; z < z1; ++z, vz += a.vsz) {
        float sdf, w = 1.f;
        if (P == SPHERE) {
            float dx = vx - a.p[0], dy = vy - a.p[1], dz = vz - a.p[2];
            sdf = __builtin_sqrtf(dx * dx + dy * dy + dz * dz) - a.r;
            w   = (sdf > -a.eta) ? 1.f : 0.f;
        } else if (P == BOX) {
            float dx = fabsf(vx) - a.p[0], dy = fabsf(vy) - a.p[1], dz = fabsf(vz) - a.p[2];
            sdf = fminf(fmaxf(dx, fmaxf(dy, dz)), 0.f) + norm3_fma(fmaxf(dx, 0.f), fmaxf(dy, 0.f), fmaxf(dz, 0.f));
        } else if (P == ELLIPSOID) {
            float k0 = norm3_fma(vx / a.p[0], vy / a.p[1], vz / a.p[2]);
            float k1 = norm3_fma(vx / (a.p[0] * a.p[0]), vy / (a.p[1] * a.p[1]), vz / (a.p[2] * a.p[2]));
            sdf      = k0 * (k0 - 1.f) / k1;
        } else if (P == PLANE) {
            sdf = vz - a.p[0];
        } else {
            float qx = __builtin_sqrtf(vx * vx + vz * vz) - a.p[0];
            sdf      = __builtin_sqrtf(qx * qx + vy * vy) - a.p[1];
        }
        a.vol[vidx(a.d, x, y, z)] = pack_tsdf(sdf, a.trunc, w);
    }
}

__global__ void __launch_bounds__(256) bilateral_kernel(const uint16_t* src, int sstep, uint16_t* dst, int dstep,
                                                        int rows, int cols, int ksz, float sss, float sds) {
    int x = blockIdx.x * blockDim.x + threadIdx.x, y = blockIdx.y * blockDim.y + threadIdx.y;
    if (x >= cols || y >= rows) return;
    int value = row_ptr(src, sstep, y)[x];
    int tx = min(x - ksz / 2 + ksz, cols - 1), ty = min(y - ksz / 2 + ksz, rows - 1);
    float sum1 = 0, sum2 = 0;
    for (int cy = max(y - ksz / 2, 0); cy < ty; ++cy)
        for (int cx = max(x - ksz / 2, 0); cx < tx; ++cx) {
            int depth    = row_ptr(src, sstep, cy)[cx];
            float space2 = (float) ((x - cx) * (x - cx) + (y - cy) * (y - cy));
            float color2 = (float) (int) ((unsigned) (value - depth) * (unsigned) (value - depth));
            float weight = expf(-(space2 * sss + color2 * sds));
            sum1 += depth * weight;
            sum2 += weight;
        }
    float q = sum1 / sum2;
    int r   = (q == q) ? (int) rintf(q) : 0;
    row_ptr(dst, dstep, y)[x] = (uint16_t) r;
}

__global__ void truncate_depth_kernel(uint16_t* depth, int step, int rows, int cols, uint16_t max_mm) {
    int x = blockIdx.x * blockDim.x + threadIdx.x, y = blockIdx.y * blockDim.y + threadIdx.y;
    if (x >= cols || y >= rows) return;
    uint16_t* p = row_ptr(depth, step, y) + x;
    if (*p > max_mm) *p = 0;
}

__global__ void compute_dists_kernel(const uint16_t* depth, int dstep, float* dists, int sstep, int rows, int cols,
                                     float fix, float fiy, float cx, float cy) {
    int x = blockIdx.x * blockDim.x + threadIdx.x, y = blockIdx.y * blockDim.y + threadIdx.y;
    if (x >= cols || y >= rows) return;
    float xl = (x - cx) * fix, yl = (y - cy) * fiy;
    float lambda = __builtin_sqrtf(xl * xl + yl * yl + 1);
    int dv       = row_ptr(depth, dstep, y)[x];
    row_ptr(dists, sstep, y)[x] = dv * lambda * 0.001f;
}

inline dim3 chunk_grid(int X, int Y, int Z) { return dim3((X + kBX - 1) / kBX, (Y + kBY - 1) / kBY, (Z + kZC - 1) / kZC); }

template <int P>
int launch_prim(float* d_vol, int X, int Y, int Z, const float vs[3], float trunc, float eta, const float* p, int np,
                float r, void* stream) {
    SOBFU_CHECK_ARGS(d_vol && vs && X > 0 && Y > 0 && Z > 0);
    PrimArgs a{(float2*) d_vol, {X, Y, Z}, vs[0], vs[1], vs[2], trunc, eta, {0, 0, 0}, r};
    for (int i = 0; i < np; ++i) a.p[i] = p[i];
    hipLaunchKernelGGL(init_prim_kernel<P>, chunk_grid(X, Y, Z), voxel_block(), 0, (hipStream_t) stream, a);
    return (int) hipGetLastError();
}

}

extern "C" {

int sobfu_hip_clear_volume(float* d_vol, int X, int Y, int Z, void* stream) {
    SOBFU_CHECK_ARGS(d_vol && X > 0 && Y > 0 && Z > 0);
    return (int) hipMemsetAsync(d_vol, 0, sizeof(float2) * (size_t) X * Y * Z, (hipStream_t) stream);
}

int sobfu_hip_integrate_depth(const float* d_dists, int step, int rows, int cols, float* d_vol, int X, int Y, int Z,
                              const float vs[3], float trunc, float eta, const float R[9], const float t[3], float fx,
                              float fy, float cx, float cy, void* stream) {
    SOBFU_CHECK_ARGS(d_dists && d_vol && vs && R && t && X > 0 && Y > 0 && Z > 0 && rows > 0 && cols > 0 && step >= cols * 4);
    IntegrateArgs a{d_dists, step, rows, cols, (float2*) d_vol, {X, Y, Z}, vs[0], vs[1], vs[2], trunc, eta, {}, {}, fx, fy, cx, cy, 0, 0, 0};
    fill_pose(R, t, a.R, nullptr, a.t);
    hipLaunchKernelGGL(integrate_depth_kernel, chunk_grid(X, Y, Z), voxel_block(), 0, (hipStream_t) stream, a);
    return (int) hipGetLastError();
}

int sobfu_hip_tile3_integrate_depth(const float* d_dists, int step, int rows, int cols, float* d_vol_local, int Lx, int Ly, int Lz, int xb,
                                    int yb, int zb, const float vs[3], float trunc, float eta, const float R[9], const float t[3], float fx,
                                    float fy, float cx, float cy, void* stream) {
    SOBFU_CHECK_ARGS(d_dists && d_vol_local && vs && R && t && Lx > 0 && Ly > 0 && Lz > 0 && xb >= 0 && yb >= 0 && zb >= 0 && rows > 0 &&
                     cols > 0 && step >= cols * 4);
    IntegrateArgs a{d_dists, step, rows, cols, (float2*) d_vol_local, {Lx, Ly, Lz}, vs[0], vs[1], vs[2], trunc, eta, {}, {}, fx, fy, cx, cy, zb, xb, yb};
    fill_pose(R, t, a.R, nullptr, a.t);
    hipLaunchKernelGGL(integrate_depth_kernel, chunk_grid(Lx, Ly, Lz), voxel_block(), 0, (hipStream_t) stream, a);
    return (int) hipGetLastError();
}

int sobfu_hip_integrate_fuse(float* d_phi_global, const float* d_phi_n_psi, int X, int Y, int Z, float max_weight,
                             void* stream) {
    SOBFU_CHECK_ARGS(d_phi_global && d_phi_n_psi && X > 0 && Y > 0 && Z > 0);
    size_t N = (size_t) X * Y * Z, pairs = (N + 1) / 2;
    hipLaunchKernelGGL(integrate_fuse_kernel, dim3((unsigned) ((pairs + 255) / 256)), dim3(256), 0, (hipStream_t) stream,
                       (float2*) d_phi_global, (const float2*) d_phi_n_psi, N, max_weight);
    return (int) hipGetLastError();
}

int sobfu_hip_init_sphere(float* d_vol, int X, int Y, int Z, const float vs[3], float trunc, float eta,
                          const float c[3], float radius, void* stream) {
    SOBFU_CHECK_ARGS(c);
    return launch_prim<SPHERE>(d_vol, X, Y, Z, vs, trunc, eta, c, 3, radius, stream);
}
int sobfu_hip_init_box(float* d_vol, int X, int Y, int Z, const float vs[3], float trunc, const float b[3], void* stream) {
    SOBFU_CHECK_ARGS(b);
    return launch_prim<BOX>(d_vol, X, Y, Z, vs, trunc, 0.f, b, 3, 0.f, stream);
}
int sobfu_hip_init_ellipsoid(float* d_vol, int X, int Y, int Z, const float vs[3], float trunc, const float r[3], void* stream) {
    SOBFU_CHECK_ARGS(r);
    return launch_prim<ELLIPSOID>(d_vol, X, Y, Z, vs, trunc, 0.f, r, 3, 0.f, stream);
}
int sobfu_hip_init_plane(float* d_vol, int X, int Y, int Z, const float vs[3], float trunc, float z, void* stream) {
    return launch_prim<PLANE>(d_vol, X, Y, Z, vs, trunc, 0.f, &z, 1, 0.f, stream);
}
int sobfu_hip_init_torus(float* d_vol, int X, int Y, int Z, const float vs[3], float trunc, const float t[2], void* stream) {
    SOBFU_CHECK_ARGS(t);
    return launch_prim<TORUS>(d_vol, X, Y, Z, vs, trunc, 0.f, t, 2, 0.f, stream);
}

int sobfu_hip_bilateral_filter(const uint16_t* d_src, int sstep, uint16_t* d_dst, int dstep, int rows, int cols, int ksz,
                               float sigma_spatial, float sigma_depth, void* stream) {
    SOBFU_CHECK_ARGS(d_src && d_dst && rows > 0 && cols > 0 && ksz > 0);
    sigma_depth *= 1000;
    hipLaunchKernelGGL(bilateral_kernel, image_grid(rows, cols), dim3(64, 4), 0, (hipStream_t) stream, d_src, sstep, d_dst,
                       dstep, rows, cols, ksz, 0.5f / (sigma_spatial * sigma_spatial), 0.5f / (sigma_depth * sigma_depth));
    return (int) hipGetLastError();
}

int sobfu_hip_truncate_depth(uint16_t* d_depth, int step, int rows, int cols, float max_dist_m, void* stream) {
    SOBFU_CHECK_ARGS(d_depth && rows > 0 && cols > 0);
    hipLaunchKernelGGL(truncate_depth_kernel, image_grid(rows, cols), dim3(64, 4), 0, (hipStream_t) stream, d_depth, step, rows,
                       cols, (uint16_t) (max_dist_m * 1000.f));
    return (int) hipGetLastError();
}

int sobfu_hip_compute_dists(const uint16_t* d_depth, int dstep, float* d_dists, int sstep, int rows, int cols, float fx,
                            float fy, float cx, float cy, void* stream) {
    SOBFU_CHECK_ARGS(d_depth && d_dists && rows > 0 && cols > 0);
    hipLaunchKernelGGL(compute_dists_kernel, image_grid(rows, cols), dim3(64, 4), 0, (hipStream_t) stream, d_depth, dstep,
                       d_dists, sstep, rows, cols, 1.f / fx, 1.f / fy, cx, cy);
    return (int) hipGetLastError();
}

}
```

sobfu_amd/fusion.py:

```python
from __future__ import annotations

import numpy as np

MESH_FRAME = (np.diag([1.0, -1.0, -1.0]).astype(np.float32), np.zeros(3, np.float32))


def affine_mul(a, b):
    a, b = np.asarray(a, np.float32), np.asarray(b, np.float32)
    r = np.eye(4, dtype=np.float32)
    for i in range(3):
        for j in range(3):
            acc = np.float32(0)
            for k in range(3):
                acc = np.float32(acc + a[i, k] * b[k, j])
            r[i, j] = acc
        r[i, 3] = np.float32(np.float32(np.float32(a[i, 0] * b[0, 3]) + np.float32(a[i, 1] * b[1, 3])) + np.float32(a[i, 2] * b[2, 3])) + a[i, 3]
    return r


def affine_inv(a):
    a = np.asarray(a, np.float32)
    r = np.eye(4, dtype=np.float32)
    r[:3, :3] = a[:3, :3].T
    for i in range(3):
        r[i, 3] = -(np.float32(np.float32(r[i, 0] * a[0, 3]) + np.float32(r[i, 1] * a[1, 3])) + np.float32(r[i, 2] * a[2, 3]))
    return r


def transform_points(points, pose):
    p, m = np.asarray(points, np.float32), np.asarray(pose, np.float32).reshape(4, 4)
    out = np.ones((len(p), 4), np.float32)
    for i in range(3):
        out[:, i] = ((m[i, 0] * p[:, 0] + m[i, 1] * p[:, 1]) + m[i, 2] * p[:, 2]) + m[i, 3]
    return out


class SobFusion:

    def __init__(self, params, max_iter=None):
        from . import ops

        self.ops, self.P = ops, params
        self.max_iter = int(params["max_iter"] if max_iter is None else max_iter)
        self.frame = 0
        self.phi_global = self.phi_global_psi_inv = self.phi_n = self.phi_n_psi = self.psi = self.psi_inv = self.solver = None
        self.last_report = None
        self.colour_global = None
        self.image_shape = None
        self.track = bool(params.get("track_camera", False))
        self.pose = np.eye(4, dtype=np.float32)
        self.poses = []
        self.icp = None
        self._prev = None

    def vol2cam(self):
        P = self.P
        if not self.track:
            return P["R"], P["t"]
        vp = np.eye(4, dtype=np.float32)
        vp[:3, :3], vp[:3, 3] = P["R"], P["t"]
        m = affine_mul(affine_inv(self.pose), vp)
        return m[:3, :3], m[:3, 3]

    def _track(self, d):
        ops, P = self.ops, self.P
        if self.icp is None:
            self.icp = ops.ICP(P["icp_dist_thres"], P["icp_angle_thres"], P["icp_iter_num"])
        levels = max(1, self.icp.used_levels())
        depth = [d]
        for _ in range(1, levels):
            depth.append(ops.depth_pyramid(depth[-1], P["bilateral"][2]))
        curr = [ops.point_normals(x, tuple(float(np.float32(np.float32(v) / np.float32(1 << l))) for v in P["intr"])) for l, x in enumerate(depth)]
        prev, self._prev = self._prev, curr
        if prev is None:
            return
        ok, aff = self.icp.estimate(P["intr"], [c[0] for c in curr], [c[1] for c in curr], [p[0] for p in prev], [p[1] for p in prev])
        if ok:
            self.pose = affine_mul(self.pose, aff)
        else:
            level, it = self.icp.failure()
            print(f"camera tracking failed on frame {self.frame} (level {level}, iteration {it}): keeping the previous pose")

    def __call__(self, depth_u16, colour=None):
        ops, P = self.ops, self.P
        if colour is not None and tuple(colour.shape) != tuple(depth_u16.shape) + (4,):
            raise ValueError(f"colour frame {tuple(colour.shape)} does not match the depth frame {tuple(depth_u16.shape)}")
        self.image_shape = tuple(depth_u16.shape)
        vs = tuple(float(v) for v in P["vs"])
        ks, ss, sd = P["bilateral"]
        d = ops.bilateral_filter(depth_u16, ks, ss, sd)
        ops.truncate_depth(d, P["trunc_depth"])
        dists = ops.compute_dists(d, P["intr"])
        if self.track:
            self._track(d)
        self.poses.append(self.pose.copy())
        R, t = self.vol2cam()

        def integrate(vol, fresh):
            if not fresh:
                ops.clear_volume(vol)
            ops.integrate_depth(dists, vol, vs, P["trunc"], P["eta"], R, t, P["intr"])

        return self._frame(integrate, colour)

    def integrate_mesh(self, vertices, faces, pose=MESH_FRAME, allow_open=False, sign="parity"):
        from .mesh_voxelise import mesh_to_tsdf

        ops, P = self.ops, self.P
        R, t = self.vol2cam()
        target = ops.new_volume(P["dims"]) if self.frame == 0 else self.phi_n
        _, open_rows = mesh_to_tsdf(vertices, faces, dict(P, R=R, t=t), pose=pose, out=target, sign=sign)
        if sign != "winding" and int(open_rows) > 0 and not allow_open:
            raise ValueError(f"the mesh is not closed: {int(open_rows)} rows of the volume cross it an odd number of times")
        self.poses.append(self.pose.copy())

        def integrate(vol, fresh):
            if vol is not target:
                vol.copy_(target)

        return self._frame(integrate, None)

    def _frame(self, integrate, colour):
        ops, P = self.ops, self.P
        dims = P["dims"]
        if self.frame == 0:
            self.phi_global = ops.new_volume(dims)
            integrate(self.phi_global, True)
            self._colour(colour, self.phi_global, None)
            self.phi_global_psi_inv, self.phi_n, self.phi_n_psi = ops.new_volume(dims), ops.new_volume(dims), ops.new_volume(dims)
            self.psi, self.psi_inv = ops.new_field(dims), ops.new_field(dims)
            ops.init_identity(self.psi)
            ops.init_identity(self.psi_inv)
            self.solver = ops.Solver(dims, max_iter=self.max_iter, alpha=P["alpha"], w_reg=P["w_reg"], s=P["s"], lam=P["lam"],
                                     max_update_norm=P["max_update_norm"])
            self.frame += 1
            return None
        integrate(self.phi_n, False)
        if self.frame < P["start_frame"]:
            self._colour(colour, self.phi_n, None)
            ops.integrate_fuse(self.phi_global, self.phi_n, P["max_weight"])
        else:
            self.last_report = self.solver.estimate_psi(self.phi_global, self.phi_global_psi_inv, self.phi_n, self.phi_n_psi, self.psi,
                                                        self.psi_inv)
            self._colour(colour, self.phi_n_psi, self.psi)
            ops.integrate_fuse(self.phi_global, self.phi_n_psi, P["max_weight"])
        self.frame += 1
        return self.last_report

    def _colour(self, colour, tsdf, psi):
        if colour is None:
            return
        P = self.P
        if self.colour_global is None:
            self.colour_global = self.ops.new_colour_volume(P["dims"])
        R, t = self.vol2cam()
        self.ops.integrate_colour(colour, tsdf, psi, self.colour_global, P["vs"], R, t, P["intr"],
                                  self.ops.colour_weight_cap(P["max_weight"]))

    def warp_stats(self, band=1.0, **kw):
        if self.last_report is None:
            return None
        return self.ops.warp_stats(self.psi, self.psi_inv, mask=self.phi_global, mask_inv=self.phi_global_psi_inv,
                                   voxel_size=tuple(float(v) for v in self.P["vs"]), band=band, **kw)

    def colour_global_psi_inv(self):
        import torch

        if self.colour_global is None:
            return None
        return self.ops.apply_colour(self.colour_global, torch.empty_like(self.colour_global), self.psi_inv)

    def render(self, which="phi_global", light=(0.0, 0.0, 0.0), colour=True):
        if which not in ("phi_global", "phi_global_psi_inv", "phi_n", "phi_n_psi"):
            raise ValueError(f"unknown volume {which!r}")
        vol = getattr(self, which)
        if vol is None:
            raise RuntimeError(f"{which} does not exist before the first frame")
        P, (rows, cols) = self.P, self.image_shape
        R, t = self.vol2cam()
        pts, nrm = self.ops.raycast(vol, P["vs"], P["trunc"], R, t, P["intr"], rows=rows, cols=cols)
        if colour and self.colour_global is not None and which in ("phi_global", "phi_global_psi_inv"):
            col = self.colour_global if which == "phi_global" else self.colour_global_psi_inv()
            return self.ops.render_colour(pts, nrm, self.ops.sample_colour(col, P["vs"], R, t, pts, nrm), light)
        return self.ops.render_image(pts, nrm, light)

    def render_model_depth(self, sensor=None, seed=0):
        if self.phi_global is None or self.image_shape is None:
            raise RuntimeError("there is no model and no depth camera before the first depth frame")
        P, (rows, cols) = self.P, self.image_shape
        R, t = self.vol2cam()
        pts, nrm = self.ops.raycast(self.phi_global, P["vs"], P["trunc"], R, t, P["intr"], rows=rows, cols=cols)
        return self.ops.depth_sensor(pts, nrm, self.ops.SensorModel.ideal() if sensor is None else sensor, seed, self.frame)

    def warp_to_live(self, vertices, normals=None):
        if self.last_report is None:
            return vertices if normals is None else (vertices, normals)
        P = self.P
        return self.ops.warp_points(self.psi, P["vs"], P["R"], P["t"], vertices, normals, mc_vertices=True)

    def fit(self, vertices):
        if self.phi_n is None:
            raise RuntimeError("phi_n does not exist before the second frame")
        P = self.P
        d = self.ops.sample_tsdf(self.phi_n, P["vs"], P["R"], P["t"], vertices, mc_vertices=True).cpu().numpy().astype(np.float64)
        d = np.abs(d[~np.isnan(d)]) * float(P["trunc"])
        if d.size == 0:
            return dict(valid=0, mean_abs=0.0, rms=0.0, max=0.0)
        return dict(valid=int(d.size), mean_abs=float(d.mean()), rms=float(np.sqrt((d * d).mean())), max=float(d.max()))

    def evaluate(self, gt_vertices, gt_faces, which="canonical", max_dist=None, pose=None, return_meshes=False, align=False, align_dof=6,
                 align_iters=30, signed=False, f_score=None):
        import torch

        from . import evaluate as E

        if which not in ("canonical", "live"):
            raise ValueError(f"which is 'canonical' or 'live', not {which!r}")
        if self.phi_global is None:
            raise RuntimeError("phi_global does not exist before the first frame")
        P = self.P
        v, _, f = self.ops.marching_cubes_indexed(self.phi_global, P["size"], P["R"], P["t"])
        if which == "live":
            v = self.warp_to_live(v)
        gv = E.device_tensor(gt_vertices, torch.float32)
        info = None
        if align:
            if which != "canonical":
                raise ValueError("align refines the pose of the canonical evaluation only")
            pose, info = E.align_meshes(v, gv, gt_faces, pose, iters=align_iters, max_dist=max_dist, dof=align_dof)
        if pose is not None:
            gv = E.device_tensor(transform_points(gv.cpu().numpy(), pose), torch.float32)
        r = E.compare_meshes(v, f, gv, gt_faces, max_dist, signed=signed)
        if align:
            r["pose"], r["align"] = pose, info
        if f_score is not None:
            r["f_score"] = E.f_score(v, f, gv, gt_faces, **f_score)
        return (r, v, f, gv) if return_meshes else r

    def close(self):
        if self.solver is not None:
            self.solver.close()
            self.solver = None
```

sobfu_amd/ops.py:

```python
from __future__ import annotations

import ctypes as C
import dataclasses

import numpy as np
import torch

from . import _lib
from ._lib import SolverParams, SolverReport, check

_F3 = C.c_float * 3
_F2 = C.c_float * 2
_F7 = C.c_float * 7
_F9 = C.c_float * 9


def _require_gpu():
    if not torch.cuda.is_available():
        raise RuntimeError("sobfu_amd needs a HIP device (MI355X); there is no CPU fallback")


def _ptr(t: torch.Tensor, dtype=torch.float32):
    if not (t.is_cuda and t.is_contiguous() and t.dtype == dtype):
        raise ValueError(f"expected a contiguous {dtype} tensor on the GPU, got {t.dtype} {t.device} contiguous={t.is_contiguous()}")
    return C.c_void_p(t.data_ptr())


def _stream():
    return C.c_void_p(torch.cuda.current_stream().cuda_stream)


def _xyz(t: torch.Tensor):
    Z, Y, X = t.shape[:3]
    return C.c_int(X), C.c_int(Y), C.c_int(Z)


def _f(x):
    return C.c_float(float(x))


def _pose(R, t):
    return (_F9(*[float(v) for v in np.asarray(R, np.float32).reshape(9)]), _F3(*[float(v) for v in np.asarray(t, np.float32).reshape(3)]))


def _vs3(voxel_size):
    return _F3(*[float(v) for v in voxel_size])


def new_volume(dims, device="cuda"):
    X, Y, Z = dims
    return torch.zeros((Z, Y, X, 2), dtype=torch.float32, device=device)


def new_field(dims, device="cuda"):
    X, Y, Z = dims
    return torch.zeros((Z, Y, X, 4), dtype=torch.float32, device=device)


def new_jacobian(dims, device="cuda"):
    X, Y, Z = dims
    return torch.zeros((Z, Y, X, 4, 4), dtype=torch.float32, device=device)


def clear_volume(vol):
    check(_lib.lib().sobfu_hip_clear_volume(_ptr(vol), *_xyz(vol), _stream()), "clear_volume")


def integrate_depth(dists, vol, voxel_size, trunc, eta, R, t, intr):
    Rm, tv = _pose(R, t)
    assert dists.is_cuda and dists.dtype == torch.float32 and dists.stride(1) == 1
    check(_lib.lib().sobfu_hip_integrate_depth(C.c_void_p(dists.data_ptr()), C.c_int(dists.stride(0) * 4),
                                               C.c_int(dists.shape[0]), C.c_int(dists.shape[1]), _ptr(vol), *_xyz(vol),
                                               _vs3(voxel_size), _f(trunc), _f(eta), Rm, tv, _f(intr[0]), _f(intr[1]), _f(intr[2]), _f(intr[3]),
                                               _stream()), "integrate_depth")


def tile3_integrate_depth(dists, vol_local, base, voxel_size, trunc, eta, R, t, intr):
    Rm, tv = _pose(R, t)
    assert dists.is_cuda and dists.dtype == torch.float32 and dists.stride(1) == 1
    check(_lib.lib().sobfu_hip_tile3_integrate_depth(C.c_void_p(dists.data_ptr()), C.c_int(dists.stride(0) * 4), C.c_int(dists.shape[0]),
                                                     C.c_int(dists.shape[1]), _ptr(vol_local), *_xyz(vol_local), *[C.c_int(int(b)) for b in base],
                                                     _vs3(voxel_size), _f(trunc), _f(eta), Rm, tv, _f(intr[0]),
                                                     _f(intr[1]), _f(intr[2]), _f(intr[3]), _stream()), "tile3_integrate_depth")


def integrate_fuse(phi_global, phi_n_psi, max_weight):
    check(_lib.lib().sobfu_hip_integrate_fuse(_ptr(phi_global), _ptr(phi_n_psi), *_xyz(phi_global), _f(max_weight),
                                              _stream()), "integrate_fuse")


def init_sphere(vol, voxel_size, trunc, eta, centre, radius):
    check(_lib.lib().sobfu_hip_init_sphere(_ptr(vol), *_xyz(vol), _vs3(voxel_size), _f(trunc),
                                           _f(eta), _F3(*[float(np.float32(v)) for v in centre]), _f(np.float32(radius)),
                                           _stream()), "init_sphere")


def init_box(vol, voxel_size, trunc, b):
    check(_lib.lib().sobfu_hip_init_box(_ptr(vol), *_xyz(vol), _vs3(voxel_size), _f(trunc),
                                        _F3(*[float(v) for v in b]), _stream()), "init_box")


def init_ellipsoid(vol, voxel_size, trunc, r):
    check(_lib.lib().sobfu_hip_init_ellipsoid(_ptr(vol), *_xyz(vol), _vs3(voxel_size), _f(trunc),
                                              _F3(*[float(v) for v in r]), _stream()), "init_ellipsoid")


def init_plane(vol, voxel_size, trunc, z):
    check(_lib.lib().sobfu_hip_init_plane(_ptr(vol), *_xyz(vol), _vs3(voxel_size), _f(trunc), _f(z),
                                          _stream()), "init_plane")


def init_torus(vol, voxel_size, trunc, t):
    check(_lib.lib().sobfu_hip_init_torus(_ptr(vol), *_xyz(vol), _vs3(voxel_size), _f(trunc),
                                          _F2(*[float(v) for v in t]), _stream()), "init_torus")


def _u16(t):
    if not (t.is_cuda and t.is_contiguous() and t.dtype in (torch.int16, torch.uint16)):
        raise ValueError("depth images must be contiguous 16-bit tensors on the GPU")
    return C.c_void_p(t.data_ptr())


def bilateral_filter(src, ksz, sigma_spatial, sigma_depth):
    dst = torch.empty_like(src)
    rows, cols = src.shape
    check(_lib.lib().sobfu_hip_bilateral_filter(_u16(src), C.c_int(cols * 2), _u16(dst), C.c_int(cols * 2), C.c_int(rows),
                                                C.c_int(cols), C.c_int(ksz), _f(sigma_spatial), _f(sigma_depth), _stream()),
          "bilateral_filter")
    return dst


def truncate_depth(depth, max_dist_m):
    rows, cols = depth.shape
    check(_lib.lib().sobfu_hip_truncate_depth(_u16(depth), C.c_int(cols * 2), C.c_int(rows), C.c_int(cols), _f(max_dist_m),
                                              _stream()), "truncate_depth")


def compute_dists(depth, intr):
    rows, cols = depth.shape
    dists = torch.empty((rows, cols), dtype=torch.float32, device=depth.device)
    check(_lib.lib().sobfu_hip_compute_dists(_u16(depth), C.c_int(cols * 2), _ptr(dists), C.c_int(cols * 4), C.c_int(rows),
                                             C.c_int(cols), _f(intr[0]), _f(intr[1]), _f(intr[2]), _f(intr[3]), _stream()),
          "compute_dists")
    return dists


def clear_field(f):
    check(_lib.lib().sobfu_hip_clear_field(_ptr(f), *_xyz(f), _stream()), "clear_field")


def init_identity(psi):
    check(_lib.lib().sobfu_hip_init_identity(_ptr(psi), *_xyz(psi), _stream()), "init_identity")


def apply(phi, phi_warped, psi):
    check(_lib.lib().sobfu_hip_apply(_ptr(phi), _ptr(phi_warped), _ptr(psi), *_xyz(phi), _stream()), "apply")


def estimate_inverse(psi, psi_inv, n_sweeps=48):
    check(_lib.lib().sobfu_hip_estimate_inverse(_ptr(psi), _ptr(psi_inv), *_xyz(psi), C.c_int(n_sweeps), _stream()),
          "estimate_inverse")


def tsdf_gradient(vol, grad):
    check(_lib.lib().sobfu_hip_tsdf_gradient(_ptr(vol), _ptr(grad), *_xyz(vol), _stream()), "tsdf_gradient")


def laplacian(psi, L):
    check(_lib.lib().sobfu_hip_laplacian(_ptr(psi), _ptr(L), *_xyz(psi), _stream()), "laplacian")


def jacobian(psi, J, mode):
    check(_lib.lib().sobfu_hip_jacobian(_ptr(psi), _ptr(J), *_xyz(psi), C.c_int(mode), _stream()), "jacobian")


def sobolev_filter(s, lam):
    out = (C.c_float * 16)()
    check(_lib.lib().sobfu_hip_sobolev_filter(C.c_int(s), _f(np.float32(lam)), out), "sobolev_filter")
    return np.array(out[:s], np.float32)


def _taps(S):
    S = np.asarray(S, np.float32)
    assert S.size >= 7
    return _F7(*[float(v) for v in S[:7]])


def potential_gradient(phi_n_psi, phi_global, grad, L, nabla_U, w_reg):
    check(_lib.lib().sobfu_hip_potential_gradient(_ptr(phi_n_psi), _ptr(phi_global), _ptr(grad), _ptr(L), _ptr(nabla_U),
                                                  _f(w_reg), *_xyz(phi_n_psi), _stream()), "potential_gradient")


def convolution_rows(dst, src, S):
    check(_lib.lib().sobfu_hip_convolution_rows(_ptr(dst), _ptr(src), _taps(S), *_xyz(src), _stream()), "convolution_rows")


def convolution_columns(dst, src, S):
    check(_lib.lib().sobfu_hip_convolution_columns(_ptr(dst), _ptr(src), _taps(S), *_xyz(src), _stream()), "convolution_columns")


def convolution_depth(dst, src, S):
    check(_lib.lib().sobfu_hip_convolution_depth(_ptr(dst), _ptr(src), _taps(S), *_xyz(src), _stream()), "convolution_depth")


def update_psi(psi, nabla_U_S, updates, alpha):
    check(_lib.lib().sobfu_hip_update_psi(_ptr(psi), _ptr(nabla_U_S), _ptr(updates), _f(alpha), *_xyz(psi), _stream()),
          "update_psi")


def reduce_config(n):
    b, t = C.c_int(), C.c_int()
    check(_lib.lib().sobfu_hip_reduce_config(C.c_int(n), C.byref(b), C.byref(t)), "reduce_config")
    return b.value, t.value


def _scratch(dev):
    return torch.empty(65536 * 2, dtype=torch.float32, device=dev)


def data_energy(phi_global, phi_n):
    out, sc = C.c_float(), _scratch(phi_global.device)
    check(_lib.lib().sobfu_hip_data_energy(_ptr(phi_global), _ptr(phi_n), C.c_int(phi_global.numel() // 2), _ptr(sc),
                                           C.byref(out), _stream()), "data_energy")
    return out.value


def reg_energy_sobolev(J):
    out, sc = C.c_float(), _scratch(J.device)
    check(_lib.lib().sobfu_hip_reg_energy_sobolev(_ptr(J), C.c_int(J.numel() // 16), _ptr(sc), C.byref(out), _stream()),
          "reg_energy_sobolev")
    return out.value


def reg_energy_sobolev_from_psi(psi):
    out, sc = C.c_float(), _scratch(psi.device)
    check(_lib.lib().sobfu_hip_reg_energy_sobolev_from_psi(_ptr(psi), *_xyz(psi), _ptr(sc), C.byref(out), _stream()),
          "reg_energy_sobolev_from_psi")
    return out.value


def max_update_norm(updates):
    out, sc = _F2(), _scratch(updates.device)
    check(_lib.lib().sobfu_hip_max_update_norm(_ptr(updates), C.c_int(updates.numel() // 4), _ptr(sc), out, _stream()),
          "max_update_norm")
    return out[0], out[1]


def fused_potential_gradient(phi_n_psi, phi_global, psi, nabla_U, w_reg):
    check(_lib.lib().sobfu_hip_fused_potential_gradient(_ptr(phi_n_psi), _ptr(phi_global), _ptr(psi), _ptr(nabla_U),
                                                        _f(w_reg), *_xyz(psi), _stream()), "fused_potential_gradient")


def fused_smooth_update_apply(nabla_U, psi, phi_n, phi_n_psi, S, alpha, updates=None, slots=None):
    if slots is None:
        slots = torch.zeros(256, dtype=torch.int32, device=psi.device)
    up = _ptr(updates) if updates is not None else None
    check(_lib.lib().sobfu_hip_fused_smooth_update_apply(_ptr(nabla_U), _ptr(psi), _ptr(phi_n), _ptr(phi_n_psi), up,
                                                         _ptr(slots, torch.int32), _taps(S), _f(alpha), *_xyz(psi),
                                                         _stream()), "fused_smooth_update_apply")
    m = np.float32(slots.max().cpu().numpy().view(np.float32))
    r = np.sqrt(m, dtype=np.float32)
    if r > 0 and np.float64(r) * np.float64(r) > np.float64(m):
        r = np.nextafter(r, np.float32(-np.inf), dtype=np.float32)
    return float(r)


class Solver:

    def __init__(self, dims, *, max_iter, alpha, w_reg, s=7, lam=0.1, max_update_norm=-1.0, verbosity=0, quiet=True):
        _require_gpu()
        self.dims = tuple(int(d) for d in dims)
        self.params = SolverParams(verbosity, max_iter, s, max_update_norm, np.float32(lam), alpha, w_reg)
        self._h = C.c_void_p()
        check(_lib.lib().sobfu_hip_solver_create(C.byref(self._h), *[C.c_int(d) for d in self.dims],
                                                 C.byref(self.params)), "solver_create")
        self.log_lines = []
        self._cb = _lib.LOG_FN(self._on_log)
        self._quiet = quiet
        check(_lib.lib().sobfu_hip_solver_set_logger(self._h, self._cb, None), "solver_set_logger")

    def _on_log(self, line, _user):
        self.log_lines.append(line.decode())
        if not self._quiet:
            print(line.decode())

    def close(self):
        if getattr(self, "_h", None):
            _lib.lib().sobfu_hip_solver_destroy(self._h)
            self._h = None

    __del__ = close

    def workspace_bytes(self):
        return int(_lib.lib().sobfu_hip_solver_workspace_bytes(self._h))

    def set_compact(self, enable=True):
        check(_lib.lib().sobfu_hip_solver_set_compact(self._h, C.c_int(1 if enable else 0)), "set_compact")

    def set_profiling(self, stride=1):
        check(_lib.lib().sobfu_hip_solver_set_profiling(self._h, C.c_int(int(stride))), "set_profiling")

    def get_profile(self, reset=True):
        a, b, n = C.c_float(), C.c_float(), C.c_int()
        check(_lib.lib().sobfu_hip_solver_get_profile(self._h, C.byref(a), C.byref(b), C.byref(n), C.c_int(1 if reset else 0)),
              "get_profile")
        return a.value, b.value, n.value

    def keep_updates(self, keep=True):
        check(_lib.lib().sobfu_hip_solver_keep_updates(self._h, C.c_int(1 if keep else 0)), "keep_updates")

    def updates(self):
        p = _lib.lib().sobfu_hip_solver_updates(self._h)
        if not p:
            raise _lib.HipError("solver_updates: allocation failed")
        X, Y, Z = self.dims

        class _Raw:
            __cuda_array_interface__ = {"shape": (Z, Y, X, 4), "typestr": "<f4", "data": (int(p), False), "version": 2}

        return torch.as_tensor(_Raw(), device="cuda")

    def estimate_psi(self, phi_global, phi_global_psi_inv, phi_n, phi_n_psi, psi, psi_inv):
        rep = SolverReport()
        hist = (C.c_float * max(1, self.params.max_iter))()
        check(_lib.lib().sobfu_hip_solver_estimate_psi(self._h, _ptr(phi_global), _ptr(phi_global_psi_inv), _ptr(phi_n),
                                                       _ptr(phi_n_psi), _ptr(psi), _ptr(psi_inv), C.byref(rep), hist,
                                                       _stream()), "solver_estimate_psi")
        return rep, np.array(hist[:rep.iterations], np.float32)

    def begin(self, phi_global, phi_n, phi_n_psi, psi, max_iters):
        self._session = (phi_global, phi_n, phi_n_psi, psi, int(max_iters))
        check(_lib.lib().sobfu_hip_solver_begin(self._h, _ptr(phi_global), _ptr(phi_n), _ptr(phi_n_psi), _ptr(psi), C.c_int(int(max_iters)),
                                                _stream()), "solver_begin")

    def step(self, n_iters):
        check(_lib.lib().sobfu_hip_solver_step(self._h, C.c_int(int(n_iters)), _stream()), "solver_step")

    def end(self):
        rep = SolverReport()
        hist = (C.c_float * max(1, self._session[4] if getattr(self, "_session", None) else 1))()
        check(_lib.lib().sobfu_hip_solver_end(self._h, C.byref(rep), hist, _stream()), "solver_end")
        self._session = None
        return rep, np.array(hist[:rep.iterations], np.float32)

    def iterate(self, phi_global, phi_n, phi_n_psi, psi, n_iters):
        rep = SolverReport()
        hist = (C.c_float * max(1, n_iters))()
        check(_lib.lib().sobfu_hip_solver_iterate(self._h, _ptr(phi_global), _ptr(phi_n), _ptr(phi_n_psi), _ptr(psi),
                                                  C.c_int(n_iters), C.byref(rep), hist, _stream()), "solver_iterate")
        return rep, np.array(hist[:rep.iterations], np.float32)


def mc_workspace(vol):
    _lib.lib().sobfu_hip_mc_workspace_bytes.restype = C.c_size_t
    n = int(_lib.lib().sobfu_hip_mc_workspace_bytes(*_xyz(vol)))
    return torch.empty(n, dtype=torch.uint8, device=vol.device)


def _ws(workspace):
    if workspace is None:
        return None, C.c_size_t(0)
    return _ptr(workspace, torch.uint8), C.c_size_t(workspace.numel())


def mc_occupied_voxels(vol, max_size, workspace=None):
    occ = torch.zeros((3, int(max_size)), dtype=torch.int32, device=vol.device)
    n = C.c_int(0)
    check(_lib.lib().sobfu_hip_mc_occupied_voxels(_stream(), _ptr(vol), *_xyz(vol), _ptr(occ, torch.int32), C.c_int(occ.shape[1]),
                                                  C.c_int(int(max_size)), C.byref(n), *_ws(workspace)), "mc_occupied_voxels")
    return occ, n.value


def mc_offsets(occ, count, workspace=None):
    total = C.c_int(0)
    check(_lib.lib().sobfu_hip_mc_offsets(_stream(), _ptr(occ, torch.int32), C.c_int(occ.shape[1]), C.c_int(int(count)), C.byref(total),
                                          *_ws(workspace)), "mc_offsets")
    return total.value


def mc_generate_triangles(vol, occ, count, volume_size, R, t, vertices, normals):
    Rm, tv = _pose(R, t)
    assert vertices.shape == normals.shape and vertices.shape[1] == 4
    check(_lib.lib().sobfu_hip_mc_generate_triangles(_stream(), _ptr(vol), *_xyz(vol), _ptr(occ, torch.int32), C.c_int(occ.shape[1]),
                                                     C.c_int(int(count)), _f(volume_size[0]), _f(volume_size[1]), _f(volume_size[2]), Rm, tv,
                                                     _ptr(vertices), _ptr(normals), C.c_int(vertices.shape[0])), "mc_generate_triangles")


def marching_cubes(vol, volume_size, R=np.eye(3), t=(0, 0, 0), max_voxels=2_000_000, max_vertices=None, workspace=None, colour=None):
    max_vertices = max_vertices or 3 * max_voxels
    occ, count = mc_occupied_voxels(vol, max_voxels, workspace)
    if count == 0:
        e = torch.zeros((0, 4), dtype=torch.float32, device=vol.device)
        if colour is not None:
            return e, e.clone(), torch.zeros((0, 4), dtype=torch.uint8, device=vol.device)
        return e, e.clone()
    total = min(mc_offsets(occ, count, workspace), max_vertices // 3 * 3)
    v = torch.zeros((max_vertices, 4), dtype=torch.float32, device=vol.device)
    n = torch.zeros_like(v)
    mc_generate_triangles(vol, occ, count, volume_size, R, t, v, n)
    if colour is not None:
        Z, Y, X = vol.shape[:3]
        vs = [float(np.float32(volume_size[i]) / np.float32(d)) for i, d in enumerate((X, Y, Z))]
        return v[:total], n[:total], sample_colour(colour, vs, R, t, v[:total], mc_vertices=True)
    return v[:total], n[:total]


def mc_indexed_workspace(vol):
    _lib.lib().sobfu_hip_mc_indexed_workspace_bytes.restype = C.c_size_t
    n = int(_lib.lib().sobfu_hip_mc_indexed_workspace_bytes(*_xyz(vol)))
    return torch.empty(n, dtype=torch.uint8, device=vol.device)


def marching_cubes_indexed(vol, volume_size, R=np.eye(3), t=(0, 0, 0), workspace=None, colour=None):
    L = _lib.lib()
    if workspace is None:
        workspace = mc_indexed_workspace(vol)
    Rm, tv = _pose(R, t)
    active, nv, nt = C.c_int(0), C.c_int(0), C.c_int(0)
    ws = _ws(workspace)
    check(L.sobfu_hip_mc_indexed_count(_stream(), _ptr(vol), *_xyz(vol), *ws, C.byref(active), C.byref(nv), C.byref(nt)), "mc_indexed_count")
    v = torch.zeros((nv.value, 4), dtype=torch.float32, device=vol.device)
    n = torch.zeros_like(v)
    f = torch.zeros((nt.value, 3), dtype=torch.int32, device=vol.device)
    if nt.value > 0:
        check(L.sobfu_hip_mc_indexed_generate(_stream(), _ptr(vol), *_xyz(vol), _f(volume_size[0]), _f(volume_size[1]), _f(volume_size[2]), Rm, tv,
                                              *ws, _ptr(v), _ptr(n), C.c_int(nv.value), _ptr(f, torch.int32), C.c_int(nt.value)),
              "mc_indexed_generate")
    if colour is not None:
        Z, Y, X = vol.shape[:3]
        vs = [float(np.float32(volume_size[i]) / np.float32(d)) for i, d in enumerate((X, Y, Z))]
        return v, n, f, sample_colour(colour, vs, R, t, v, mc_vertices=True)
    return v, n, f


def _image_ptr(t, dtype, channels):
    if not (t.is_cuda and t.dtype == dtype and t.dim() == 3 and t.shape[2] == channels and t.stride(2) == 1 and t.stride(1) == channels):
        raise ValueError(f"expected a (rows, cols, {channels}) {dtype} image on the GPU with contiguous rows, got {t.dtype} {tuple(t.shape)}")
    return C.c_void_p(t.data_ptr()), C.c_int(t.stride(0) * t.element_size())


def raycast(vol, voxel_size, trunc, R, t, intr, rows=480, cols=640, step_factor=0.75, points=None, normals=None):
    Rm, tv = _pose(R, t)
    if points is None:
        points = torch.empty((rows, cols, 4), dtype=torch.float32, device=vol.device)
    if normals is None:
        normals = torch.empty((rows, cols, 4), dtype=torch.float32, device=vol.device)
    vs = [float(np.float32(v)) for v in voxel_size]
    check(_lib.lib().sobfu_hip_raycast(_ptr(vol), *_xyz(vol), _f(vs[0]), _f(vs[1]), _f(vs[2]), _f(trunc), Rm, tv, _f(intr[0]), _f(intr[1]),
                                       _f(intr[2]), _f(intr[3]), C.c_int(int(rows)), C.c_int(int(cols)), _f(step_factor),
                                       *_image_ptr(points, torch.float32, 4), *_image_ptr(normals, torch.float32, 4), _stream()), "raycast")
# ... 765 lines not shown
```

Measured before the change: 4441.

## Keep solver compact channels resident and have integration kernels write them directly

Adds a resident mode in which the solver's compact TSDF channels for phi_global and phi_n are exposed, and the clear, integrate and fuse kernels write these channels alongside the volume. The solver's enter step can then skip repacking channels already marked current, and skip repacking psi when it is unchanged from the last solve. The compact_leave call is moved ahead of the drain, and an optional inverse-and-warp tail is added to session_end. The aim is to remove per-frame full-volume packing passes at the start of each solve, at the cost of extra stores during integration and more state to keep consistent.

```diff
diff --git a/include/sobfu_amd/sobfu.hpp b/include/sobfu_amd/sobfu.hpp
--- a/include/sobfu_amd/sobfu.hpp
+++ b/include/sobfu_amd/sobfu.hpp
@@ -486,17 +486,20 @@
     TsdfVolume(float2* d, int3 dm, float3 vs, float trunc, float eta_, float maxw)
         : data(d), dims(dm), voxel_size(vs), trunc_dist(trunc), eta(eta_), max_weight(maxw) {}
 };
-inline void clear_volume(TsdfVolume& v) { sobfuSafeCall(sobfu_hip_clear_volume((float*) v.data, v.dims.x, v.dims.y, v.dims.z, nullptr)); }
-inline void integrate(TsdfVolume& g, TsdfVolume& n) {
-    sobfuSafeCall(sobfu_hip_integrate_fuse((float*) g.data, (const float*) n.data, g.dims.x, g.dims.y, g.dims.z, g.max_weight, nullptr));
+inline void clear_volume(TsdfVolume& v, float* channel = nullptr) {
+    if (channel) sobfuSafeCall(sobfu_hip_clear_volume_ch((float*) v.data, channel, v.dims.x, v.dims.y, v.dims.z, nullptr));
+    else sobfuSafeCall(sobfu_hip_clear_volume((float*) v.data, v.dims.x, v.dims.y, v.dims.z, nullptr));
+}
+inline void integrate(TsdfVolume& g, TsdfVolume& n, float* channel = nullptr) {
+    sobfuSafeCall(sobfu_hip_integrate_fuse_ch((float*) g.data, channel, (const float*) n.data, g.dims.x, g.dims.y, g.dims.z, g.max_weight, nullptr));
     sobfuSafeCall(hipDeviceSynchronize());
 }
-inline void integrate(const cuda::Dists& dists, TsdfVolume& v, const Aff3f& a, const Projector& p) {
+inline void integrate(const cuda::Dists& dists, TsdfVolume& v, const Aff3f& a, const Projector& p, float* channel = nullptr) {
     float R[9] = {a.R.data[0].x, a.R.data[0].y, a.R.data[0].z, a.R.data[1].x, a.R.data[1].y, a.R.data[1].z,
                   a.R.data[2].x, a.R.data[2].y, a.R.data[2].z};
     float t[3] = {a.t.x, a.t.y, a.t.z}, vs[3] = {v.voxel_size.x, v.voxel_size.y, v.voxel_size.z};
-    sobfuSafeCall(sobfu_hip_integrate_depth(dists.ptr(), (int) dists.step(), dists.rows(), dists.cols(), (float*) v.data, v.dims.x,
-                                            v.dims.y, v.dims.z, vs, v.trunc_dist, v.eta, R, t, p.f.x, p.f.y, p.c.x, p.c.y, nullptr));
+    sobfuSafeCall(sobfu_hip_integrate_depth_ch(dists.ptr(), (int) dists.step(), dists.rows(), dists.cols(), (float*) v.data, channel, v.dims.x,
+                                               v.dims.y, v.dims.z, vs, v.trunc_dist, v.eta, R, t, p.f.x, p.f.y, p.c.x, p.c.y, nullptr));
     sobfuSafeCall(hipDeviceSynchronize());
 }
 #define SOBFU_AMD_VS(v) float vs[3] = {(v).voxel_size.x, (v).voxel_size.y, (v).voxel_size.z}
@@ -568,18 +571,20 @@
     void setGradientDeltaFactor(float& f) { gradient_delta_factor_ = f; }
     float getRaycastStepFactor() const { return raycast_step_factor_; }
     void setRaycastStepFactor(float& f) { raycast_step_factor_ = f; }
-    virtual void clear() { device::TsdfVolume v = pod(); device::clear_volume(v); }
+    void setChannel(float* c) { channel_ = c; }
+    float* getChannel() const { return channel_; }
+    virtual void clear() { device::TsdfVolume v = pod(); device::clear_volume(v, channel_); }
     void swap(CudaData& d) { data_.swap(d); }
     virtual void applyAffine(const Affine3f& a) { pose_ = a * pose_; }
     virtual void integrate(const TsdfVolume& phi_n_psi) {
         device::TsdfVolume g = pod();
         device::TsdfVolume n((float2*) phi_n_psi.data_.ptr<float2>(), g.dims, g.voxel_size, trunc_dist_, eta_, max_weight_);
-        device::integrate(g, n);
+        device::integrate(g, n, channel_);
     }
     virtual void integrate(const Dists& dists, const Affine3f& camera_pose, const Intr& intr) {
         Affine3f vol2cam = camera_pose.inv() * pose_;
         device::TsdfVolume v = pod();
-        device::integrate(dists, v, device_cast<device::Aff3f>(vol2cam), device::Projector(intr.fx, intr.fy, intr.cx, intr.cy));
+        device::integrate(dists, v, device_cast<device::Aff3f>(vol2cam), device::Projector(intr.fx, intr.fy, intr.cx, intr.cy), channel_);
     }
     virtual void raycast(const Affine3f& camera_pose, const Intr& intr, Cloud& points, Normals& normals) {
         const Affine3f vol2cam = camera_pose.inv() * pose_;
@@ -601,6 +606,7 @@
 
 private:
     CudaData data_;
+    float* channel_ = nullptr;
     float trunc_dist_, eta_, max_weight_;
     Vec3i dims_;
     Vec3f size_;
@@ -1043,6 +1049,10 @@
                                                     psi->get_data().ptr<float>(), psi_inv->get_data().ptr<float>(), &last_report,
                                                     nullptr, nullptr));
     }
+    void set_resident(bool on) { sobfuSafeCall(sobfu_hip_solver_set_resident(h_, on ? 1 : 0)); }
+    void invalidate() { sobfuSafeCall(sobfu_hip_solver_invalidate(h_)); }
+    void channels(float** c_phi_global, float** c_phi_n) { sobfuSafeCall(sobfu_hip_solver_channels(h_, c_phi_global, c_phi_n)); }
+    void channels_current(const float* d_phi_global, const float* d_phi_n) { sobfuSafeCall(sobfu_hip_solver_channels_current(h_, d_phi_global, d_phi_n)); }
     sobfu_hip_solver* handle() { return h_; }
     sobfu_hip_solver_report last_report{};
 
@@ -1213,8 +1223,9 @@
         if (params.track_camera) track();
         poses_.push_back(camera_pose_);
         return frame(image, [&](kfusion::cuda::TsdfVolume& v, bool fresh) {
-            if (!fresh) v.clear();
+            if (!fresh || v.getChannel()) v.clear();
             v.integrate(dists_, camera_pose_, params.intr);
+            return v.getChannel() != nullptr;
         });
     }
     bool integrate_mesh(const sobfu_amd::IndexedMesh& mesh, const cv::Affine3f& mesh2cam = sobfu_amd::mesh_frame(), bool allow_open = false,
@@ -1229,7 +1240,7 @@
         }
         std::printf("--- FRAME NO. %d ---\n", frame_counter_);
         poses_.push_back(camera_pose_);
-        return frame(kfusion::cuda::Image(), [](kfusion::cuda::TsdfVolume&, bool) {}, target);
+        return frame(kfusion::cuda::Image(), [](kfusion::cuda::TsdfVolume&, bool) { return false; }, target);
     }
     std::shared_ptr<kfusion::cuda::ColourVolume> get_colour_global_psi_inv() {
         if (!colour_global) return nullptr;
@@ -1341,15 +1352,23 @@
             psi     = std::make_shared<sobfu::cuda::DeformationField>(params.volume_dims);
             psi_inv = std::make_shared<sobfu::cuda::DeformationField>(params.volume_dims);
             solver  = std::make_shared<sobfu::cuda::Solver>(params);
+            solver->set_resident(true);
+            float *c_g = nullptr, *c_n = nullptr;
+            solver->channels(&c_g, &c_n);
+            phi_global->setChannel(c_g);
+            phi_n->setChannel(c_n);
+            g_current_ = false;
             return ++frame_counter_, true;
         }
-        integrate(*phi_n, false);
+        const bool n_current = integrate(*phi_n, false);
         if (frame_counter_ < params.start_frame) {
             if (coloured) integrate_colour(image, *phi_n, nullptr);
             phi_global->integrate(*phi_n);
             return ++frame_counter_, true;
         }
+        solver->channels_current(g_current_ ? phi_global->data().ptr<float>() : nullptr, n_current ? phi_n->data().ptr<float>() : nullptr);
         solver->estimate_psi(phi_global, phi_global_psi_inv, phi_n, phi_n_psi, psi, psi_inv);
+        g_current_ = phi_global->getChannel() != nullptr;
         solved_ = true;
         if (coloured) integrate_colour(image, *phi_n_psi, psi->get_data().ptr<float>());
         phi_global->integrate(*phi_n_psi);
@@ -1382,6 +1401,7 @@
     }
     int frame_counter_;
     bool solved_ = false;
+    bool g_current_ = false;
     Params params;
     cv::Affine3f camera_pose_;
     std::vector<cv::Affine3f> poses_;
diff --git a/include/sobfu_hip.h b/include/sobfu_hip.h
--- a/include/sobfu_hip.h
+++ b/include/sobfu_hip.h
@@ -27,6 +27,12 @@
                               void* stream);
 int sobfu_hip_integrate_fuse(float* d_phi_global, const float* d_phi_n_psi, int X, int Y, int Z, float max_weight,
                              void* stream);
+int sobfu_hip_clear_volume_ch(float* d_vol, float* d_ch, int X, int Y, int Z, void* stream);
+int sobfu_hip_integrate_depth_ch(const float* d_dists, int dists_step_bytes, int rows, int cols, float* d_vol, float* d_ch, int X,
+                                 int Y, int Z, const float voxel_size[3], float trunc_dist, float eta, const float R[9],
+                                 const float t[3], float fx, float fy, float cx, float cy, void* stream);
+int sobfu_hip_integrate_fuse_ch(float* d_phi_global, float* d_ch, const float* d_phi_n_psi, int X, int Y, int Z, float max_weight,
+                                void* stream);
 int sobfu_hip_init_sphere(float* d_vol, int X, int Y, int Z, const float voxel_size[3], float trunc_dist, float eta,
                           const float centre[3], float radius, void* stream);
 int sobfu_hip_init_box(float* d_vol, int X, int Y, int Z, const float voxel_size[3], float trunc_dist,
@@ -150,6 +156,10 @@
 float* sobfu_hip_solver_updates(sobfu_hip_solver* s);
 int sobfu_hip_solver_keep_updates(sobfu_hip_solver* s, int keep);
 int sobfu_hip_solver_set_compact(sobfu_hip_solver* s, int enable);
+int sobfu_hip_solver_set_resident(sobfu_hip_solver* s, int enable);
+int sobfu_hip_solver_invalidate(sobfu_hip_solver* s);
+int sobfu_hip_solver_channels(sobfu_hip_solver* s, float** c_phi_global, float** c_phi_n);
+int sobfu_hip_solver_channels_current(sobfu_hip_solver* s, const float* d_phi_global, const float* d_phi_n);
 int sobfu_hip_solver_set_profiling(sobfu_hip_solver* s, int stride);
 int sobfu_hip_solver_get_profile(sobfu_hip_solver* s, float* ms_pass_a, float* ms_pass_b, int* launches, int reset);
 typedef void (*sobfu_hip_log_fn)(const char* line, void* user);
diff --git a/sobfu_amd/csrc/solver_capi.hip b/sobfu_amd/csrc/solver_capi.hip
--- a/sobfu_amd/csrc/solver_capi.hip
+++ b/sobfu_amd/csrc/solver_capi.hip
@@ -20,6 +20,45 @@
 using sobfu_hip::slots_to_norm;
 constexpr int kCheckEvery = 32;
 constexpr int kMaxRunAhead = 96;
+
+typedef float v3f __attribute__((ext_vector_type(3)));
+typedef v3f __attribute__((aligned(4))) v3f_u;
+template <bool PSI, bool F>
+__global__ void __launch_bounds__(256) partial_enter_kernel(const float4* __restrict__ psi4, const float2* __restrict__ pg2,
+                                                            const float2* __restrict__ pn2, float* __restrict__ c_psi, float* __restrict__ c_g,
+                                                            float* __restrict__ c_n, float* __restrict__ c_f, sobfu_hip::Dims d) {
+    using namespace sobfu_hip;
+    const int x = blockIdx.x * kBX + threadIdx.x, y = blockIdx.y * kBY + threadIdx.y, z = blockIdx.z;
+    if (x >= d.x || y >= d.y) return;
+    const size_t i = vidx(d, x, y, z);
+    v3f p = {0.f, 0.f, 0.f};
+    if (PSI) {
+        const float4 q = psi4[i];
+        p = v3f{q.x, q.y, q.z};
+        *(v3f_u*) (c_psi + 3 * i) = p;
+    } else if (F) {
+        p = *(const v3f_u*) (c_psi + 3 * i);
+    }
+    if (c_g) c_g[i] = pg2[i].x;
+    if (c_n) c_n[i] = pn2[i].x;
+    if (F) c_f[i] = interp_tsdf(pn2, d, p.x, p.y, p.z).x;
+}
+
+int launch_enter(const float* psi4, const float* pg2, const float* pn2, float* c_psi, float* c_g, float* c_n, float* c_f, int X, int Y, int Z,
+                 bool pack_psi, hipStream_t stream) {
+    using namespace sobfu_hip;
+    if (pack_psi && c_g && c_n && c_f) return launch_compact_enter(psi4, pg2, pn2, c_psi, c_g, c_n, c_f, X, Y, Z, stream);
+    if (!pack_psi && !c_g && !c_n && !c_f) return 0;
+#define SOBFU_ENTER(PSI, F)                                                                                                      \
+    hipLaunchKernelGGL((partial_enter_kernel<PSI, F>), voxel_grid(X, Y, Z), voxel_block(), 0, stream, (const float4*) psi4, \
+                       (const float2*) pg2, (const float2*) pn2, c_psi, c_g, c_n, c_f, Dims{X, Y, Z})
+    if (pack_psi && c_f) SOBFU_ENTER(true, true);
+    else if (pack_psi) SOBFU_ENTER(true, false);
+    else if (c_f) SOBFU_ENTER(false, true);
+    else SOBFU_ENTER(false, false);
+#undef SOBFU_ENTER
+    return (int) hipGetLastError();
+}
 
 }
 
@@ -35,6 +74,9 @@
     DevicePtr<float> c_g;
     DevicePtr<float> c_n;
     bool compact = true;
+    bool resident        = false;
+    const float* res_psi = nullptr;
+    const float *cur_g = nullptr, *cur_n = nullptr;
     DevicePtr<uint32_t> slots;
     sobfu_hip::PinnedPtr<uint32_t> h_rows;
     int h_rows_iters   = 0;
@@ -152,6 +194,8 @@
     q.last_norm = NAN;
     if (!q.compact) SOBFU_TRY(sobfu_hip_apply(pn, pnp, psi, X, Y, Z, st));
     if (cap <= 0) return 0;
+    const bool psi_resident = q.compact && s->resident && s->res_psi == psi;
+    s->res_psi = nullptr;
     SOBFU_TRY(ensure_slots(s, cap));
     SOBFU_HIP_TRY(hipMemsetAsync(s->slots.get(), 0, (size_t) (cap + 1) * kSlots * 4, st));
     if (s->keep_updates) {
@@ -161,9 +205,11 @@
     q.it_pnp = pnp; q.it_pg = pg; q.it_pn = pn; q.it_psi = psi; q.it_out = pnp;
     if (q.compact) {
         SOBFU_TRY(ensure_compact(s));
-        SOBFU_TRY(sobfu_hip::launch_compact_enter(psi, pg, pn, s->c_psi.get(), s->c_g.get(), s->c_n.get(), s->c_f.get(), X, Y, Z, st));
+        q.warp = s->p.verbosity == 0 && !q.upd && sobfu_hip::loop_warps_in_pass_a(X, Y, Z);
+        const bool g_current = s->resident && s->cur_g == pg, n_current = s->resident && s->cur_n == pn;
+        SOBFU_TRY(launch_enter(psi, pg, pn, s->c_psi.get(), g_current ? nullptr : s->c_g.get(), n_current ? nullptr : s->c_n.get(),
+                               q.warp ? nullptr : s->c_f.get(), X, Y, Z, !psi_resident, st));
         q.it_pnp = s->c_f.get(); q.it_pg = s->c_g.get(); q.it_pn = s->c_n.get(); q.it_psi = s->c_psi.get(); q.it_out = s->c_f.get();
-        q.warp = s->p.verbosity == 0 && !q.upd && sobfu_hip::loop_warps_in_pass_a(X, Y, Z);
     }
     if (s->p.max_update_norm >= 0.f) SOBFU_TRY(ensure_poll(s, cap));
     if (s->prof_stride > 0) SOBFU_TRY(ensure_events(s, (size_t) 3 * (cap / s->prof_stride + 1)));
@@ -275,15 +321,26 @@
     return 0;
 }
 
-int session_end(sobfu_hip_solver* s, sobfu_hip_solver_report* rep, float* per_iter, hipStream_t st) {
+struct SolveTail {
+    float *psi_inv, *pg_psi_inv;
+};
+
+int session_end(sobfu_hip_solver* s, sobfu_hip_solver_report* rep, float* per_iter, hipStream_t st, const SolveTail* tail = nullptr) {
     sobfu_hip_solver::Session& q = s->q;
     if (!q.active) return SOBFU_E_BADARG;
     sobfu_hip_solver_report r{};
     r.last_max_update_norm = NAN;
     r.last_max_update_index = NAN;
     r.last_e_data = r.last_e_reg = NAN;
+    if (q.compact) SOBFU_TRY(sobfu_hip::launch_compact_leave(s->c_psi.get(), q.pn, q.psi, q.pnp, s->X, s->Y, s->Z, st));
+    if (tail) {
+        const int rc = sobfu_hip_inverse_and_warp(q.psi, tail->psi_inv, q.pg, tail->pg_psi_inv, s->X, s->Y, s->Z, 48, st);
+        if (rc != 0) {
+            q.active = false;
+            return rc;
+        }
+    }
     SOBFU_TRY(session_drain(s, per_iter, st));
-    if (q.compact) SOBFU_TRY(sobfu_hip::launch_compact_leave(s->c_psi.get(), q.pn, q.psi, q.pnp, s->X, s->Y, s->Z, st));
     for (int it = 1; it <= q.done && !q.inline_log; ++it)
         if (it == 1 || it % 50 == 0) s->log("iter. no. " + std::to_string(it));
     if (q.converged) s->log("SOLVER CONVERGED AFTER " + std::to_string(q.done) + " ITERATIONS");
@@ -293,12 +350,13 @@
     r.last_max_update_norm = q.last_norm;
     q.active = false;
     SOBFU_HIP_TRY(hipStreamSynchronize(st));
+    if (q.compact && s->resident) s->res_psi = q.psi;
     if (rep) *rep = r;
     return 0;
 }
 
 int run_verbose(sobfu_hip_solver* s, const float* pg, const float* pn, float* pnp, float* psi, int max_iter,
-                sobfu_hip_solver_report* rep, float* per_iter, hipStream_t st) {
+                sobfu_hip_solver_report* rep, float* per_iter, hipStream_t st, const SolveTail* tail) {
     const int X = s->X, Y = s->Y, Z = s->Z;
     const sobfu_hip_solver_params& p = s->p;
     auto reports = [&](int it) { return p.verbosity == 2 || (p.verbosity == 1 && (it == 1 || it % 50 == 0 || it == max_iter)); };
@@ -366,7 +424,7 @@
 #undef SOBFU_VTRY
     const bool last_reported = q.done > 0 && reports(q.done);
     sobfu_hip_solver_report r{};
-    SOBFU_TRY(session_end(s, &r, per_iter, st));
+    SOBFU_TRY(session_end(s, &r, per_iter, st, tail));
     r.last_e_data = e_data;
     r.last_e_reg  = e_reg;
     r.last_max_update_index = last_reported ? arg : NAN;
@@ -375,16 +433,16 @@
 }
 
 int run_loop(sobfu_hip_solver* s, const float* pg, const float* pn, float* pnp, float* psi, int max_iter,
-             sobfu_hip_solver_report* rep, float* per_iter, hipStream_t st) {
+             sobfu_hip_solver_report* rep, float* per_iter, hipStream_t st, const SolveTail* tail = nullptr) {
     if (s->q.active) return SOBFU_E_BADARG;
-    if (s->p.verbosity > 0 && max_iter > 0) return run_verbose(s, pg, pn, pnp, psi, max_iter, rep, per_iter, st);
+    if (s->p.verbosity > 0 && max_iter > 0) return run_verbose(s, pg, pn, pnp, psi, max_iter, rep, per_iter, st, tail);
     SOBFU_TRY(session_begin(s, pg, pn, pnp, psi, max_iter, st));
     int rc = session_enqueue(s, max_iter, true, per_iter, st);
     if (rc != 0) {
         s->q.active = false;
         return rc;
     }
-    return session_end(s, rep, per_iter, st);
+    return session_end(s, rep, per_iter, st, tail);
 }
 
 }
@@ -486,6 +544,38 @@
 int sobfu_hip_solver_set_compact(sobfu_hip_solver* s, int enable) {
     SOBFU_CHECK_ARGS(s);
     s->compact = enable != 0;
+    if (!s->compact) s->res_psi = nullptr;
+    return 0;
+}
+
+int sobfu_hip_solver_set_resident(sobfu_hip_solver* s, int enable) {
+    SOBFU_CHECK_ARGS(s && !s->q.active);
+    const char* e = getenv("SOBFU_RESIDENT");
+    s->resident   = enable != 0 && !(e && atoi(e) == 0);
+    s->res_psi = s->cur_g = s->cur_n = nullptr;
+    return 0;
+}
+
+int sobfu_hip_solver_invalidate(sobfu_hip_solver* s) {
+    SOBFU_CHECK_ARGS(s && !s->q.active);
+    s->res_psi = s->cur_g = s->cur_n = nullptr;
+    return 0;
+}
+
+int sobfu_hip_solver_channels(sobfu_hip_solver* s, float** c_phi_global, float** c_phi_n) {
+    SOBFU_CHECK_ARGS(s && c_phi_global && c_phi_n);
+    *c_phi_global = *c_phi_n = nullptr;
+    if (!s->resident || !s->compact) return 0;
+    SOBFU_TRY(ensure_compact(s));
+    *c_phi_global = s->c_g.get();
+    *c_phi_n      = s->c_n.get();
+    return 0;
+}
+
+int sobfu_hip_solver_channels_current(sobfu_hip_solver* s, const float* d_phi_global, const float* d_phi_n) {
+    SOBFU_CHECK_ARGS(s && !s->q.active);
+    s->cur_g = s->resident ? d_phi_global : nullptr;
+    s->cur_n = s->resident ? d_phi_n : nullptr;
     return 0;
 }
 
@@ -546,11 +636,11 @@
 int sobfu_hip_solver_estimate_psi(sobfu_hip_solver* s, const float* d_phi_global, float* d_phi_global_psi_inv,
                                   const float* d_phi_n, float* d_phi_n_psi, float* d_psi, float* d_psi_inv,
                                   sobfu_hip_solver_report* report, float* per_iter_max_norm, void* stream) {
-    SOBFU_CHECK_ARGS(s && d_phi_global && d_phi_global_psi_inv && d_phi_n && d_phi_n_psi && d_psi && d_psi_inv);
+    SOBFU_CHECK_ARGS(s && d_phi_global && d_phi_global_psi_inv && d_phi_n && d_phi_n_psi && d_psi && d_psi_inv && d_psi != d_psi_inv &&
+                     d_phi_global != d_phi_global_psi_inv);
     hipStream_t st = (hipStream_t) stream;
-    SOBFU_TRY(run_loop(s, d_phi_global, d_phi_n, d_phi_n_psi, d_psi, s->p.max_iter, report, per_iter_max_norm, st));
-    SOBFU_TRY(sobfu_hip_inverse_and_warp(d_psi, d_psi_inv, d_phi_global, d_phi_global_psi_inv, s->X, s->Y, s->Z, 48, st));
-    return (int) hipStreamSynchronize(st);
-}
-
-}
+    const SolveTail tail{d_psi_inv, d_phi_global_psi_inv};
+    return run_loop(s, d_phi_global, d_phi_n, d_phi_n_psi, d_psi, s->p.max_iter, report, per_iter_max_norm, st, &tail);
+}
+
+}
diff --git a/sobfu_amd/csrc/tsdf_kernels.hip b/sobfu_amd/csrc/tsdf_kernels.hip
--- a/sobfu_amd/csrc/tsdf_kernels.hip
+++ b/sobfu_amd/csrc/tsdf_kernels.hip
@@ -18,8 +18,10 @@
     float fx, fy, cx, cy;
     int zbase;
     int xbase, ybase;
+    float* ch;
 };
 
+template <bool CH>
 __global__ void __launch_bounds__(256) integrate_depth_kernel(IntegrateArgs a) {
     int x = blockIdx.x * kBX + threadIdx.x, y = blockIdx.y * kBY + threadIdx.y;
     if (x >= a.d.x || y >= a.d.y) return;
@@ -41,12 +43,15 @@
         if (Dp <= 0.f) continue;
         float psdf   = Dp - camz;
         float weight = (psdf > -a.eta) ? 1.f : 0.f;
-        a.vol[vidx(a.d, x, y, z)] = pack_tsdf(psdf, a.trunc, weight);
-    }
-}
-
+        const float2 v = pack_tsdf(psdf, a.trunc, weight);
+        a.vol[vidx(a.d, x, y, z)] = v;
+        if (CH) a.ch[vidx(a.d, x, y, z)] = v.x;
+    }
+}
+
+template <bool CH>
 __global__ void __launch_bounds__(256) integrate_fuse_kernel(float2* __restrict__ g, const float2* __restrict__ n,
-                                                             size_t N, float max_weight) {
+                                                             size_t N, float max_weight, float* __restrict__ ch) {
     size_t i = ((size_t) blockIdx.x * blockDim.x + threadIdx.x) * 2;
     if (i >= N) return;
     auto one = [&](float2 t, float2 p, bool& w) -> float2 {
@@ -61,10 +66,16 @@
         if (w0 && w1) *(float4*) (g + i) = make_float4(o0.x, o0.y, o1.x, o1.y);
         else if (w0) g[i] = o0;
         else if (w1) g[i + 1] = o1;
+        if (CH) {
+            if (w0 && w1) *(float2*) (ch + i) = make_float2(o0.x, o1.x);
+            else if (w0) ch[i] = o0.x;
+            else if (w1) ch[i + 1] = o1.x;
+        }
     } else {
         bool w0;
         float2 o0 = one(n[i], g[i], w0);
         if (w0) g[i] = o0;
+        if (CH && w0) ch[i] = o0.x;
     }
 }
 
@@ -177,14 +188,27 @@
     return (int) hipMemsetAsync(d_vol, 0, sizeof(float2) * (size_t) X * Y * Z, (hipStream_t) stream);
 }
 
+int sobfu_hip_clear_volume_ch(float* d_vol, float* d_ch, int X, int Y, int Z, void* stream) {
+    SOBFU_CHECK_ARGS(d_vol && d_ch && X > 0 && Y > 0 && Z > 0);
+    SOBFU_HIP_TRY(hipMemsetAsync(d_vol, 0, sizeof(float2) * (size_t) X * Y * Z, (hipStream_t) stream));
+    return (int) hipMemsetAsync(d_ch, 0, sizeof(float) * (size_t) X * Y * Z, (hipStream_t) stream);
+}
+
+int sobfu_hip_integrate_depth_ch(const float* d_dists, int step, int rows, int cols, float* d_vol, float* d_ch, int X, int Y, int Z,
+                                 const float vs[3], float trunc, float eta, const float R[9], const float t[3], float fx, float fy, float cx,
+                                 float cy, void* stream) {
+    SOBFU_CHECK_ARGS(d_dists && d_vol && vs && R && t && X > 0 && Y > 0 && Z > 0 && rows > 0 && cols > 0 && step >= cols * 4 && d_ch != d_vol);
+    IntegrateArgs a{d_dists, step, rows, cols, (float2*) d_vol, {X, Y, Z}, vs[0], vs[1], vs[2], trunc, eta, {}, {}, fx, fy, cx, cy, 0, 0, 0, d_ch};
+    fill_pose(R, t, a.R, nullptr, a.t);
+    if (d_ch) hipLaunchKernelGGL(integrate_depth_kernel<true>, chunk_grid(X, Y, Z), voxel_block(), 0, (hipStream_t) stream, a);
+    else hipLaunchKernelGGL(integrate_depth_kernel<false>, chunk_grid(X, Y, Z), voxel_block(), 0, (hipStream_t) stream, a);
+    return (int) hipGetLastError();
+}
+
 int sobfu_hip_integrate_depth(const float* d_dists, int step, int rows, int cols, float* d_vol, int X, int Y, int Z,
                               const float vs[3], float trunc, float eta, const float R[9], const float t[3], float fx,
                               float fy, float cx, float cy, void* stream) {
-    SOBFU_CHECK_ARGS(d_dists && d_vol && vs && R && t && X > 0 && Y > 0 && Z > 0 && rows > 0 && cols > 0 && step >= cols * 4);
-    IntegrateArgs a{d_dists, step, rows, cols, (float2*) d_vol, {X, Y, Z}, vs[0], vs[1], vs[2], trunc, eta, {}, {}, fx, fy, cx, cy, 0, 0, 0};
-    fill_pose(R, t, a.R, nullptr, a.t);
-    hipLaunchKernelGGL(integrate_depth_kernel, chunk_grid(X, Y, Z), voxel_block(), 0, (hipStream_t) stream, a);
-    return (int) hipGetLastError();
+    return sobfu_hip_integrate_depth_ch(d_dists, step, rows, cols, d_vol, nullptr, X, Y, Z, vs, trunc, eta, R, t, fx, fy, cx, cy, stream);
 }
 
 int sobfu_hip_tile3_integrate_depth(const float* d_dists, int step, int rows, int cols, float* d_vol_local, int Lx, int Ly, int Lz, int xb,
@@ -192,19 +216,28 @@
                                     float fy, float cx, float cy, void* stream) {
     SOBFU_CHECK_ARGS(d_dists && d_vol_local && vs && R && t && Lx > 0 && Ly > 0 && Lz > 0 && xb >= 0 && yb >= 0 && zb >= 0 && rows > 0 &&
                      cols > 0 && step >= cols * 4);
-    IntegrateArgs a{d_dists, step, rows, cols, (float2*) d_vol_local, {Lx, Ly, Lz}, vs[0], vs[1], vs[2], trunc, eta, {}, {}, fx, fy, cx, cy, zb, xb, yb};
+    IntegrateArgs a{d_dists, step, rows, cols, (float2*) d_vol_local, {Lx, Ly, Lz}, vs[0], vs[1], vs[2], trunc, eta, {}, {}, fx, fy, cx, cy, zb, xb, yb, nullptr};
     fill_pose(R, t, a.R, nullptr, a.t);
-    hipLaunchKernelGGL(integrate_depth_kernel, chunk_grid(Lx, Ly, Lz), voxel_block(), 0, (hipStream_t) stream, a);
+    hipLaunchKernelGGL(integrate_depth_kernel<false>, chunk_grid(Lx, Ly, Lz), voxel_block(), 0, (hipStream_t) stream, a);
+    return (int) hipGetLastError();
+}
+
+int sobfu_hip_integrate_fuse_ch(float* d_phi_global, float* d_ch, const float* d_phi_n_psi, int X, int Y, int Z, float max_weight,
+                                void* stream) {
+    SOBFU_CHECK_ARGS(d_phi_global && d_phi_n_psi && X > 0 && Y > 0 && Z > 0 && d_ch != d_phi_global && d_ch != d_phi_n_psi &&
+                     ((uintptr_t) d_ch & 7u) == 0);
+    size_t N = (size_t) X * Y * Z, pairs = (N + 1) / 2;
+    const dim3 grid((unsigned) ((pairs + 255) / 256));
+    if (d_ch) hipLaunchKernelGGL(integrate_fuse_kernel<true>, grid, dim3(256), 0, (hipStream_t) stream, (float2*) d_phi_global,
+                                 (const float2*) d_phi_n_psi, N, max_weight, d_ch);
+    else hipLaunchKernelGGL(integrate_fuse_kernel<false>, grid, dim3(256), 0, (hipStream_t) stream, (float2*) d_phi_global,
+                            (const float2*) d_phi_n_psi, N, max_weight, (float*) nullptr);
     return (int) hipGetLastError();
 }
 
 int sobfu_hip_integrate_fuse(float* d_phi_global, const float* d_phi_n_psi, int X, int Y, int Z, float max_weight,
                              void* stream) {
-    SOBFU_CHECK_ARGS(d_phi_global && d_phi_n_psi && X > 0 && Y > 0 && Z > 0);
-    size_t N = (size_t) X * Y * Z, pairs = (N + 1) / 2;
-    hipLaunchKernelGGL(integrate_fuse_kernel, dim3((unsigned) ((pairs + 255) / 256)), dim3(256), 0, (hipStream_t) stream,
-                       (float2*) d_phi_global, (const float2*) d_phi_n_psi, N, max_weight);
-    return (int) hipGetLastError();
+    return sobfu_hip_integrate_fuse_ch(d_phi_global, nullptr, d_phi_n_psi, X, Y, Z, max_weight, stream);
 }
 
 int sobfu_hip_init_sphere(float* d_vol, int X, int Y, int Z, const float vs[3], float trunc, float eta,
diff --git a/sobfu_amd/fusion.py b/sobfu_amd/fusion.py
--- a/sobfu_amd/fusion.py
+++ b/sobfu_amd/fusion.py
@@ -45,6 +45,8 @@
         self.frame = 0
         self.phi_global = self.phi_global_psi_inv = self.phi_n = self.phi_n_psi = self.psi = self.psi_inv = self.solver = None
         self.last_report = None
+        self._c_g = self._c_n = None
+        self._g_current = self._n_current = False
         self.colour_global = None
         self.image_shape = None
         self.track = bool(params.get("track_camera", False))
@@ -96,10 +98,11 @@
         self.poses.append(self.pose.copy())
         R, t = self.vol2cam()
 
-        def integrate(vol, fresh):
-            if not fresh:
-                ops.clear_volume(vol)
-            ops.integrate_depth(dists, vol, vs, P["trunc"], P["eta"], R, t, P["intr"])
+        def integrate(vol, fresh, channel):
+            if not fresh or channel is not None:
+                ops.clear_volume(vol, channel)
+            ops.integrate_depth(dists, vol, vs, P["trunc"], P["eta"], R, t, P["intr"], channel)
+            return channel is not None
 
         return self._frame(integrate, colour)
 
@@ -114,9 +117,10 @@
             raise ValueError(f"the mesh is not closed: {int(open_rows)} rows of the volume cross it an odd number of times")
         self.poses.append(self.pose.copy())
 
-        def integrate(vol, fresh):
+        def integrate(vol, fresh, channel):
             if vol is not target:
                 vol.copy_(target)
+            return False
 
         return self._frame(integrate, None)
 
@@ -125,7 +129,7 @@
         dims = P["dims"]
         if self.frame == 0:
             self.phi_global = ops.new_volume(dims)
-            integrate(self.phi_global, True)
+            integrate(self.phi_global, True, None)
             self._colour(colour, self.phi_global, None)
             self.phi_global_psi_inv, self.phi_n, self.phi_n_psi = ops.new_volume(dims), ops.new_volume(dims), ops.new_volume(dims)
             self.psi, self.psi_inv = ops.new_field(dims), ops.new_field(dims)
@@ -133,17 +137,22 @@
             ops.init_identity(self.psi_inv)
             self.solver = ops.Solver(dims, max_iter=self.max_iter, alpha=P["alpha"], w_reg=P["w_reg"], s=P["s"], lam=P["lam"],
                                      max_update_norm=P["max_update_norm"])
+            self.solver.set_resident(True)
+            self._c_g, self._c_n = self.solver.channels()
+            self._g_current = self._n_current = False
             self.frame += 1
             return None
-        integrate(self.phi_n, False)
+        self._n_current = bool(integrate(self.phi_n, False, self._c_n))
         if self.frame < P["start_frame"]:
             self._colour(colour, self.phi_n, None)
-            ops.integrate_fuse(self.phi_global, self.phi_n, P["max_weight"])
+            ops.integrate_fuse(self.phi_global, self.phi_n, P["max_weight"], self._c_g)
         else:
+            self.solver.channels_current(self.phi_global if self._g_current else None, self.phi_n if self._n_current else None)
             self.last_report = self.solver.estimate_psi(self.phi_global, self.phi_global_psi_inv, self.phi_n, self.phi_n_psi, self.psi,
                                                         self.psi_inv)
+            self._g_current = self._c_g is not None
             self._colour(colour, self.phi_n_psi, self.psi)
-            ops.integrate_fuse(self.phi_global, self.phi_n_psi, P["max_weight"])
+            ops.integrate_fuse(self.phi_global, self.phi_n_psi, P["max_weight"], self._c_g)
         self.frame += 1
         return self.last_report
 
diff --git a/sobfu_amd/ops.py b/sobfu_amd/ops.py
--- a/sobfu_amd/ops.py
+++ b/sobfu_amd/ops.py
@@ -62,17 +62,28 @@
     return torch.zeros((Z, Y, X, 4, 4), dtype=torch.float32, device=device)
 
 
-def clear_volume(vol):
-    check(_lib.lib().sobfu_hip_clear_volume(_ptr(vol), *_xyz(vol), _stream()), "clear_volume")
-
-
-def integrate_depth(dists, vol, voxel_size, trunc, eta, R, t, intr):
+def _channel(ch, vol):
+    if ch is None:
+        return None
+    if tuple(ch.shape) != tuple(vol.shape[:3]):
+        raise ValueError(f"channel {tuple(ch.shape)} does not match the volume {tuple(vol.shape)}")
+    return _ptr(ch)
+
+
+def clear_volume(vol, channel=None):
+    if channel is None:
+        check(_lib.lib().sobfu_hip_clear_volume(_ptr(vol), *_xyz(vol), _stream()), "clear_volume")
+    else:
+        check(_lib.lib().sobfu_hip_clear_volume_ch(_ptr(vol), _channel(channel, vol), *_xyz(vol), _stream()), "clear_volume_ch")
+
+
+def integrate_depth(dists, vol, voxel_size, trunc, eta, R, t, intr, channel=None):
     Rm, tv = _pose(R, t)
     assert dists.is_cuda and dists.dtype == torch.float32 and dists.stride(1) == 1
-    check(_lib.lib().sobfu_hip_integrate_depth(C.c_void_p(dists.data_ptr()), C.c_int(dists.stride(0) * 4),
-                                               C.c_int(dists.shape[0]), C.c_int(dists.shape[1]), _ptr(vol), *_xyz(vol),
-                                               _vs3(voxel_size), _f(trunc), _f(eta), Rm, tv, _f(intr[0]), _f(intr[1]), _f(intr[2]), _f(intr[3]),
-                                               _stream()), "integrate_depth")
+    check(_lib.lib().sobfu_hip_integrate_depth_ch(C.c_void_p(dists.data_ptr()), C.c_int(dists.stride(0) * 4),
+                                                  C.c_int(dists.shape[0]), C.c_int(dists.shape[1]), _ptr(vol), _channel(channel, vol), *_xyz(vol),
+                                                  _vs3(voxel_size), _f(trunc), _f(eta), Rm, tv, _f(intr[0]), _f(intr[1]), _f(intr[2]), _f(intr[3]),
+                                                  _stream()), "integrate_depth")
 
 
 def tile3_integrate_depth(dists, vol_local, base, voxel_size, trunc, eta, R, t, intr):
@@ -84,9 +95,9 @@
                                                      _f(intr[1]), _f(intr[2]), _f(intr[3]), _stream()), "tile3_integrate_depth")
 
 
-def integrate_fuse(phi_global, phi_n_psi, max_weight):
-    check(_lib.lib().sobfu_hip_integrate_fuse(_ptr(phi_global), _ptr(phi_n_psi), *_xyz(phi_global), _f(max_weight),
-                                              _stream()), "integrate_fuse")
+def integrate_fuse(phi_global, phi_n_psi, max_weight, channel=None):
+    check(_lib.lib().sobfu_hip_integrate_fuse_ch(_ptr(phi_global), _channel(channel, phi_global), _ptr(phi_n_psi), *_xyz(phi_global),
+                                                 _f(max_weight), _stream()), "integrate_fuse")
 
 
 def init_sphere(vol, voxel_size, trunc, eta, centre, radius):
@@ -296,6 +307,31 @@
 
     def set_compact(self, enable=True):
         check(_lib.lib().sobfu_hip_solver_set_compact(self._h, C.c_int(1 if enable else 0)), "set_compact")
+
+    def set_resident(self, enable=True):
+        check(_lib.lib().sobfu_hip_solver_set_resident(self._h, C.c_int(1 if enable else 0)), "set_resident")
+
+    def invalidate(self):
+        check(_lib.lib().sobfu_hip_solver_invalidate(self._h), "invalidate")
+
+    def channels(self):
+        g, n = C.c_void_p(), C.c_void_p()
+        check(_lib.lib().sobfu_hip_solver_channels(self._h, C.byref(g), C.byref(n)), "solver_channels")
+        if not g.value or not n.value:
+            return None, None
+        X, Y, Z = self.dims
+
+        def view(p):
+            class _Raw:
+                __cuda_array_interface__ = {"shape": (Z, Y, X), "typestr": "<f4", "data": (int(p), False), "version": 2}
+
+            return torch.as_tensor(_Raw(), device="cuda")
+
+        return view(g.value), view(n.value)
+
+    def channels_current(self, phi_global=None, phi_n=None):
+        check(_lib.lib().sobfu_hip_solver_channels_current(self._h, None if phi_global is None else _ptr(phi_global),
+                                                           None if phi_n is None else _ptr(phi_n)), "channels_current")
 
     def set_profiling(self, stride=1):
         check(_lib.lib().sobfu_hip_solver_set_profiling(self._h, C.c_int(int(stride))), "set_profiling")
```

Result: no change. 4433 (-0.2%).
